# cornell-zhang/HiSparse

Measured on AMD Instinct MI355X. Metric: SpMV GBPS (8 B per non-zero per SpMV, sw/benchmark.cpp:312-346), higher is better.
Workload: dtype u32 (Q8.24 fixed point, u64 row sums)

## Files before the change

hisparse_amd/csrc/gpu_tiles.h:

```cpp
#ifndef HISPARSE_GPU_TILES_H_
#define HISPARSE_GPU_TILES_H_

#include <hip/hip_runtime_api.h>

#include <cstdint>
#include <string>
#include <vector>

#include "device_buffer.h"
#include "tiles_common.h"

namespace hisparse {
namespace dev {

hipError_t warm_gpu_tiler();

class GpuTiler {
  public:
    GpuTiler(const detail::Layout& layout, const void* const channel[NUM_HBM_CHANNELS], const uint64_t n_packets[NUM_HBM_CHANNELS], hipStream_t stream);
    GpuTiler(const detail::Layout& layout, const CsrView& csr, hipStream_t stream);
    GpuTiler(const GpuTiler&) = delete;
    GpuTiler& operator=(const GpuTiler&) = delete;

    const std::string& error() const { return error_; }
    bool count_rows(std::vector<uint32_t>& row_nnz, uint64_t& nnz);
    bool count_tiles(const std::vector<uint32_t>& block_of_row, uint32_t num_ranges, std::vector<uint32_t>& cnt);
    bool sort_elements(const std::vector<uint32_t>& block_of_row, const std::vector<uint32_t>& range_row0, const std::vector<uint32_t>& unit_of,
                       const std::vector<detail::UnitPlan>& plans, bool& duplicates);
    bool delta_slots(std::vector<detail::UnitPlan>& plans);
    bool owner_shares(std::vector<detail::UnitPlan>& plans, uint32_t max_span);
    bool emit(StreamFormat format, uint64_t image_bytes, uint64_t slack_bytes, const std::vector<detail::UnitPlan>& plans,
              const std::vector<uint32_t>& block_of_unit, const std::vector<Block>& blocks, bool is_float);
    bool bitmap_slice_counts(uint32_t slices, uint32_t groups_per_row, std::vector<uint32_t>& cnt);
    struct BitmapBlock {
        uint32_t row0, nrows, gs0, GS, pieces, stride;
        uint64_t mask_word0;
        uint64_t prefix0;
        uint32_t piece_cut[kBitmapWaves + 1];
    };
    struct BitmapRun {
        uint64_t mask_word, prefix_at;
        uint32_t steps, pad;
    };
    bool bitmap_emit(uint32_t slices, uint32_t groups_per_row, const std::vector<uint32_t>& range_of_row, const std::vector<BitmapBlock>& blocks,
                     const std::vector<uint64_t>& row_value_base, uint64_t image_bytes, uint64_t slack_bytes, const std::vector<BitmapRun>& runs,
                     std::vector<uint32_t>& run_prefix, std::vector<uint64_t>& run_heads, const MfmaImage* mfma, bool& duplicates);
    uint8_t* release_mfma() { return d_mfma_.release(); }
    bool sweep_line_counts(uint32_t lines, std::vector<uint64_t>& line_nnz);
    bool sweep_sort(const std::vector<uint32_t>& range_of_row, const std::vector<uint32_t>& range_row0, const std::vector<uint32_t>& slice_col,
                    uint32_t num_blocks, std::vector<uint64_t>& block_start, bool& unsupported);
    struct SweepBlock {
        uint64_t first;
        uint64_t stream_at, table_at;
        uint64_t chunk0;
        uint32_t count, steps, nrows, pad_col;
    };
    bool sweep_emit(const std::vector<SweepBlock>& blocks, uint64_t image_bytes, uint64_t slack_bytes);
    uint8_t* release_image() { return d_image_.release(); }
    uint32_t* release_value_map() { return d_map_.release(); }
    uint32_t* release_value_map2() { return d_map2_.release(); }

  private:
    bool fail(const std::string& what);
    bool check(hipError_t e, const char* what);
    bool upload_channels();
    bool upload_csr(std::vector<uint32_t>& row_nnz);
    bool read_error(const char* copy, const char* sync);
    bool gather_values();
    void release_source();
    bool alloc_map(DeviceBuffer<uint32_t>& map, uint64_t image_bytes);
    template <typename S> S source() const;
    template <typename G> const G* groups() const { return reinterpret_cast<const G*>(d_groups_.get()); }
    uint64_t element_threads() const;

    detail::Layout L_;
    Geometry geom_;
    const void* const* channel_;
    const uint64_t* n_packets_;
    hipStream_t stream_;
    std::string error_;

    const CsrView* csr_ = nullptr;
    uint32_t indptr_rows_ = 0;
    DeviceBuffer<uint32_t> d_indptr_;
    DeviceBuffer<uint32_t> d_indices_;
// ... 27 lines not shown
```

hisparse_amd/csrc/gpu_tiles.hip:

```cpp
#include "gpu_tiles.h"

#include <hip/hip_runtime.h>
#include <hipcub/hipcub.hpp>

#include <algorithm>
#include <cstring>
#include <type_traits>

#include "value_word.h"

namespace hisparse {
namespace dev {

using detail::Layout;
using detail::UnitPlan;

namespace {

constexpr uint32_t kPosBits = 28;
constexpr uint64_t kPosMask = (1ull << kPosBits) - 1;
constexpr uint32_t kErrColumn = 1, kErrRow = 2;

struct StreamGroup {
    uint64_t byte_off;
// ... 384 lines not shown
        uint32_t d = 0;
        if (i > 0) {
            const uint32_t prev = uint32_t(keys[p.start + i - 1] & kPosMask);
            const uint64_t b = bridges[p.start + i] - bridges[p.start + i - 1];
            d = uint32_t(pos - prev - b * kBridgeAdvance);
        }
        return Slot{d, vals[p.start + i], pos, p.start + i};
    }
    const uint32_t prev = uint32_t(keys[p.start + i - 1] & kPosMask);
    const uint64_t s_prev = (i - 1) + (bridges[p.start + i - 1] - bbase);
    const uint64_t k = si - (s_prev + 1);
    return Slot{kBridgeGap, 0u, uint32_t(prev + (k + 1) * kBridgeAdvance), kNoElement};
}

template <bool kMap>
__global__ __launch_bounds__(256) void emit_delta_kernel(const DevicePlan* __restrict__ plans, const uint64_t* __restrict__ keys,
                                                        const uint32_t* __restrict__ vals, const uint64_t* __restrict__ bridges,
                                                        uint8_t* __restrict__ image, uint32_t pad_gap, const uint32_t* __restrict__ src,
                                                        uint32_t* __restrict__ map) {
    const DevicePlan& p = plans[blockIdx.x];
    if (!p.n) return;
    const uint32_t scratch_pos = p.nrows * kSubTileCols;
    const uint32_t first_pos = uint32_t(keys[p.start] & kPosMask);
    for (uint32_t w = 0; w < kConsumerWaves; ++w) {
        const uint32_t run = p.run_len[w];
        if (!run) continue;
        uint8_t* rec = image + p.wave_offset[w] + uint64_t(p.start_step[w]) * kRecordBytes;
        const uint32_t slots_in_records = (run + 2) / 2 * 2;
        for (uint32_t idx = threadIdx.x; idx < slots_in_records * kWaveLanes; idx += blockDim.x) {
            const uint32_t j = idx / kWaveLanes, l = idx % kWaveLanes;
            uint8_t* r = rec + uint64_t(j / 2) * kRecordBytes;
            uint32_t* value_word = reinterpret_cast<uint32_t*>(r) + 2 * l + j % 2;
            uint16_t* gap_word = reinterpret_cast<uint16_t*>(r + kWaveLanes * 8) + 2 * l + j % 2;
            const uint64_t s0 = p.first_slot[w] + uint64_t(l) * p.lane_stride[w];
            if (j == 0) {
                uint32_t head = scratch_pos;
                if (s0 < p.slots) head = s0 == 0 ? first_pos : delta_slot(p, keys, vals, bridges, s0 - 1).after;
                *value_word = head;
                continue;
            }
            if (j > run) { *gap_word = uint16_t(pad_gap); continue; }
            const uint64_t si = s0 + (j - 1);
            uint32_t value = 0, gap = pad_gap;
            if (si < p.slots) {
                const Slot s = delta_slot(p, keys, vals, bridges, si);
                value = s.val;
                gap = s.gap;
                if (kMap && s.e != kNoElement) map[src[s.e]] = word_index(value_word, image);
            }
            *value_word = value;
            *gap_word = uint16_t(gap);
        }
    }
}

struct ElementSource {
    const uint8_t* channels;
    const StreamGroup* groups;
    const uint64_t* advance;
    const uint32_t* indptr;
    const uint32_t* indices;
    const float* values;
    uint64_t nnz;
    uint32_t num_groups, total_slots, num_rows, num_cols, logical_vb, fixed, csr;
    uint32_t transposed;
};

template <typename Visit>
__device__ __forceinline__ void visit_elements(const ElementSource& src, uint64_t t, uint32_t* err, Visit visit) {
    if (src.csr) {
        CsrCursor c;
        if (!csr_segment(src.indptr, src.num_rows, src.nnz, t, c)) return;
        for (; c.e < c.end; ++c.e) {
            while (c.e >= src.indptr[c.row + 1]) ++c.row;
            const uint32_t idx = src.indices[c.e];
            if (idx >= src.num_cols) { report(err, kErrColumn, c.row / PACK_SIZE, c.row % PACK_SIZE); return; }
            const uint32_t row = src.transposed ? idx : c.row, col = src.transposed ? c.row : idx;
            if constexpr (std::is_invocable_v<Visit, uint32_t, uint32_t, uint32_t, uint64_t>) visit(row, col, value_word(src.values[c.e], src.fixed != 0), c.e);
            else visit(row, col, value_word(src.values[c.e], src.fixed != 0));
        }
        return;
    }
    Segment s;
    if (t >= src.total_slots || !find_segment(src.channels, src.groups, src.num_groups, src.total_slots, uint32_t(t), s)) return;
    const StreamGroup& g = src.groups[s.group];
    const uint32_t col_base = g.cp * src.logical_vb;
    if constexpr (std::is_invocable_v<Visit, uint32_t, uint32_t, uint32_t, uint64_t>)
        walk_segment(g, s, src.advance, [&](uint32_t row, uint32_t col, uint32_t val) { visit(row, col_base + col, val, ~0ull); });
    else
        walk_segment(g, s, src.advance, [&](uint32_t row, uint32_t col, uint32_t val) { visit(row, col_base + col, val); });
}

__device__ __forceinline__ uint32_t cut_at(uint32_t n, uint32_t parts, uint32_t k) { return uint32_t(uint64_t(k) * n / parts); }
__device__ __forceinline__ uint32_t part_of(uint32_t n, uint32_t parts, uint32_t x) {
    uint32_t k = min(parts - 1, uint32_t((uint64_t(x) + 1) * parts / n));
    while (cut_at(n, parts, k) > x) --k;
    while (k + 1 < parts && cut_at(n, parts, k + 1) <= x) ++k;
    return k;
}
__device__ __forceinline__ uint32_t padded_masks(uint32_t steps) { return (steps + 7u) / 8u * 8u + 16u; }
__device__ __forceinline__ uint32_t mask_offset(const GpuTiler::BitmapBlock& b, uint32_t g) {
    if (b.pieces <= 1) return g;
    uint32_t j = 0, at = 0;
    while (j + 1 < b.pieces && b.piece_cut[j + 1] <= g) {
        at += padded_masks(b.piece_cut[j + 1] - b.piece_cut[j]);
        ++j;
// ... 427 lines not shown
    DeviceBuffer<DevicePlan> d_plans;
    DeviceBuffer<uint8_t> d_temp;
    std::vector<DevicePlan> dp;
    make_device_plans(plans, {}, {}, dp);
    bool ok = check(d_in.alloc_count(n), "hipMalloc") && check(d_bridges_.alloc_count(n), "hipMalloc") && check(d_slots.alloc_count(plans.size(), 16), "hipMalloc") &&
              check(upload(d_plans, dp, stream_), "upload plans");
    if (ok && total_) {
        hipLaunchKernelGGL(bridges_kernel, dim3(uint32_t((total_ + 255) / 256)), dim3(256), 0, stream_, d_keys_.get(), total_, d_in.get());
        size_t temp_bytes = 0;
        ok = check(hipGetLastError(), "bridges_kernel") &&
             check(hipcub::DeviceScan::InclusiveSum(nullptr, temp_bytes, d_in.get(), d_bridges_.get(), total_, stream_), "scan (size)") &&
             check(d_temp.alloc_count(temp_bytes, 16), "hipMalloc(scan)") &&
             check(hipcub::DeviceScan::InclusiveSum(d_temp.get(), temp_bytes, d_in.get(), d_bridges_.get(), total_, stream_), "scan");
    }
    std::vector<uint64_t> slots(plans.size(), 0);
    if (ok && !plans.empty()) {
        hipLaunchKernelGGL(unit_slots_kernel, dim3(uint32_t((plans.size() + 255) / 256)), dim3(256), 0, stream_, d_plans.get(), uint32_t(plans.size()), d_bridges_.get(), d_slots.get());
        ok = check(hipGetLastError(), "unit_slots_kernel") &&
             check(hipMemcpyAsync(slots.data(), d_slots.get(), slots.size() * 8, hipMemcpyDeviceToHost, stream_), "read slots");
    }
    ok = ok && check(hipStreamSynchronize(stream_), "delta slots");
    if (ok)
        for (size_t u = 0; u < plans.size(); ++u) plans[u].slots = slots[u];
    return ok;
}

bool GpuTiler::owner_shares(std::vector<UnitPlan>& plans, uint32_t max_span) {
    const uint32_t nu = uint32_t(plans.size());
    if (!nu) return true;
    std::vector<uint64_t> start(nu);
    std::vector<uint32_t> count(nu);
    for (uint32_t u = 0; u < nu; ++u) { start[u] = plans[u].scratch; count[u] = plans[u].n; }
    DeviceBuffer<uint64_t> d_start;
    DeviceBuffer<uint32_t> d_n, d_own;
    std::vector<uint32_t> own(size_t(nu) * kShareWords);
    bool ok = check(upload(d_start, start, stream_), "upload") && check(upload(d_n, count, stream_), "upload") && check(d_own.alloc_count(own.size()), "hipMalloc");
    if (ok) {
        hipLaunchKernelGGL(owner_balanced_shares_kernel, dim3((nu + 255) / 256), dim3(256), 0, stream_, d_start.get(), d_n.get(), nu, d_keys_.get(), max_span, d_own.get());
        ok = check(hipGetLastError(), "owner_balanced_shares_kernel") &&
             check(hipMemcpyAsync(own.data(), d_own.get(), own.size() * 4, hipMemcpyDeviceToHost, stream_), "read shares") && check(hipStreamSynchronize(stream_), "owner shares");
    }
    if (ok)
        for (uint32_t u = 0; u < nu; ++u) {
            const uint32_t* o = own.data() + size_t(u) * kShareWords;
            for (uint32_t w = 0; w <= kConsumerWaves; ++w) plans[u].own_begin[w] = o[w];
            for (uint32_t w = 0; w < kConsumerWaves; ++w) {
                plans[u].own_row[w] = o[kConsumerWaves + 1 + w];
                plans[u].own_last[w] = o[2 * kConsumerWaves + 1 + w];
            }
        }
    return ok;
}

bool GpuTiler::emit(StreamFormat format, uint64_t image_bytes, uint64_t slack_bytes, const std::vector<UnitPlan>& plans,
                    const std::vector<uint32_t>& block_of_unit, const std::vector<Block>& blocks, bool is_float) {
    std::vector<DevicePlan> dp;
    make_device_plans(plans, block_of_unit, blocks, dp);
    DeviceBuffer<DevicePlan> d_plans;
    const size_t bytes = std::max<uint64_t>(image_bytes + slack_bytes, 256);
    bool ok = check(d_image_.alloc(bytes), "hipMalloc(image)") && check(hipMemsetAsync(d_image_.get(), 0, bytes, stream_), "hipMemset(image)") &&
              check(upload(d_plans, dp, stream_), "upload plans");
    if (ok && d_src_) ok = alloc_map(d_map_, image_bytes);
    const dim3 grid(uint32_t(plans.size())), block(256);
    if (ok && !plans.empty()) {
        const bool m = bool(d_map_);
        const DevicePlan* p = d_plans.get();
        const uint64_t* keys = d_keys_.get();
        const uint32_t *vals = d_vals_.get(), *src = d_src_.get();
        uint8_t* image = d_image_.get();
        uint32_t* map = d_map_.get();
        switch (format) {
            case kFormatPairs:
                hipLaunchKernelGGL((m ? emit_pairs_kernel<false, true> : emit_pairs_kernel<false, false>), grid, block, 0, stream_, p, keys, vals, image, src, map);
                break;
            case kFormatPairs24:
                hipLaunchKernelGGL((m ? emit_pairs_kernel<true, true> : emit_pairs_kernel<true, false>), grid, block, 0, stream_, p, keys, vals, image, src, map);
                break;
            case kFormatOwner:
                hipLaunchKernelGGL((m ? emit_owner_kernel<false, true> : emit_owner_kernel<false, false>), grid, block, 0, stream_, p, keys, vals, image, src, map);
                break;
            case kFormatOwner24:
                hipLaunchKernelGGL((m ? emit_owner_kernel<true, true> : emit_owner_kernel<true, false>), grid, block, 0, stream_, p, keys, vals, image, src, map);
                break;
            case kFormatDelta:
                hipLaunchKernelGGL(m ? emit_delta_kernel<true> : emit_delta_kernel<false>, grid, block, 0, stream_, p, keys, vals, d_bridges_.get(), image,
                                   is_float ? kBridgeGap : 0u, src, map);
                break;
            default: ok = fail("gpu re-tile: format not supported");
        }
        ok = ok && check(hipGetLastError(), "emit kernel");
    }
    ok = ok && check(hipStreamSynchronize(stream_), "emit");
    d_keys_.reset();
    d_vals_.reset();
    d_bridges_.reset();
    d_src_.reset();
    return ok;
}

bool GpuTiler::bitmap_slice_counts(uint32_t slices, uint32_t GR, std::vector<uint32_t>& cnt) {
    cnt.assign(size_t(L_.num_rows) * slices, 0);
    const uint64_t threads = element_threads();
    DeviceBuffer<uint32_t> d_cnt;
    bool ok = check(d_cnt.alloc_count(cnt.size(), 16), "hipMalloc") && check(hipMemsetAsync(d_cnt.get(), 0, cnt.size() * 4, stream_), "hipMemset");
    if (ok && threads) {
        hipLaunchKernelGGL(bitmap_slice_counts_kernel, dim3(uint32_t((threads + 255) / 256)), dim3(256), 0, stream_, source<ElementSource>(), slices, GR, d_cnt.get(), d_scalar_.get());
        ok = check(hipGetLastError(), "bitmap_slice_counts_kernel");
    }
    return ok && (cnt.empty() || check(hipMemcpyAsync(cnt.data(), d_cnt.get(), cnt.size() * 4, hipMemcpyDeviceToHost, stream_), "read slice counts")) &&
           read_error("slice counts", "slice counts");
}

bool GpuTiler::bitmap_emit(uint32_t slices, uint32_t GR, const std::vector<uint32_t>& range_of_row, const std::vector<BitmapBlock>& blocks,
                           const std::vector<uint64_t>& row_value_base, uint64_t image_bytes, uint64_t slack_bytes, const std::vector<BitmapRun>& runs,
                           std::vector<uint32_t>& run_prefix, std::vector<uint64_t>& run_heads, const MfmaImage* mfma, bool& duplicates) {
    detail::PhaseTimer timer;
    duplicates = false;
    const ElementSource src = source<ElementSource>();
    const uint64_t threads = element_threads();
    const dim3 egrid(uint32_t((threads + 255) / 256)), block(256);
    uint64_t prefix_words = 0;
    for (const BitmapBlock& b : blocks) prefix_words = std::max<uint64_t>(prefix_words, b.prefix0 + uint64_t(b.nrows) * b.stride);
    const size_t bytes = std::max<uint64_t>(image_bytes + slack_bytes, 256);
    const uint32_t num_runs = uint32_t(runs.size());
    run_prefix.assign(num_runs, 0);
    run_heads.assign(size_t(num_runs) * kBitmapMaskBatch, 0);
    DeviceBuffer<uint32_t> d_range, d_prefix, d_flags, d_run_prefix, d_cnt, d_pos;
    DeviceBuffer<BitmapBlock> d_blocks;
    DeviceBuffer<BitmapRun> d_runs;
    DeviceBuffer<uint64_t> d_row_base;
    DeviceBuffer<unsigned long long> d_heads;
    DeviceBuffer<uint8_t> d_temp;
    bool ok = check(d_image_.alloc(bytes), "hipMalloc(image)") && check(hipMemsetAsync(d_image_.get(), 0, bytes, stream_), "hipMemset(image)") &&
              check(upload(d_range, range_of_row, stream_), "upload row ranges") && check(upload(d_blocks, blocks, stream_), "upload blocks") &&
              check(upload(d_row_base, row_value_base, stream_), "upload row bases") && check(upload(d_runs, runs, stream_), "upload runs") &&
              check(d_prefix.alloc_count(prefix_words, 16), "hipMalloc(prefix)") &&
              check(d_flags.alloc(16), "hipMalloc") && check(hipMemsetAsync(d_flags.get(), 0, 16, stream_), "hipMemset") &&
              check(d_run_prefix.alloc_count(num_runs, 16), "hipMalloc") && check(d_heads.alloc_count(run_heads.size(), 16), "hipMalloc");
    unsigned long long* image64 = reinterpret_cast<unsigned long long*>(d_image_.get());
    unsigned long long* masks2 = nullptr;
    if (ok && mfma) {
        ok = check(d_mfma_.alloc_count(mfma->words_bytes, 16), "hipMalloc(second image)") &&
             check(hipMemsetAsync(d_mfma_.get(), 0, mfma->words_bytes, stream_), "hipMemset(second image)");
        masks2 = reinterpret_cast<unsigned long long*>(d_mfma_.get());
    }
// ... 232 lines not shown
```

hisparse_amd/csrc/hs_load.cpp:

```cpp
#include "hs_context.h"

#include <algorithm>
#include <chrono>
#include <cstdio>
#include <cstdlib>

#include "hisparse/channel_packets.h"

using hisparse::Geometry;
using hisparse::dev::Block;
using hisparse::dev::Unit;

namespace {

constexpr size_t kImageSlackBytes = 16384;

bool value_map_asked(const hs_context* c) {
    const char* v = ctx_option(c, "HISPARSE_VALUE_MAP");
    return v && std::atoi(v) != 0;
}

template <typename T>
hipError_t upload(DeviceBuffer<T>& dst, const void* src, size_t bytes, size_t slack) {
    const hipError_t e = dst.alloc(std::max<size_t>(bytes + slack, 256));
    if (e != hipSuccess || bytes == 0) return e;
    return hipMemcpy(dst.get(), src, bytes, hipMemcpyHostToDevice);
}

int load_matrix_once(hs_context* ctx, const void* const* channel, const uint64_t* n_packets, const hisparse::dev::CsrView* csr_in,
                     uint32_t num_rows, uint32_t num_cols, uint32_t num_row_partitions, uint32_t num_col_partitions, bool want_map) {
    const Geometry& g = ctx->geom;
    if (num_rows == 0 || num_cols == 0) return fail(ctx, HS_ERR_BAD_ARG, "empty matrix");
    if (num_rows % g.row_divisor != 0 || num_cols % hisparse::PACK_SIZE != 0)
        return fail(ctx, HS_ERR_BAD_ARG, "dimensions are not padded: rows must divide by " + std::to_string(g.row_divisor) +
                                             " and columns by 8 (util_round_csr_matrix_dim)");
    if (num_row_partitions != (num_rows + g.logical_ob - 1) / g.logical_ob || num_col_partitions != (num_cols + g.logical_vb - 1) / g.logical_vb)
        return fail(ctx, HS_ERR_BAD_ARG, "partition counts do not match the dimensions and the bank sizes of this context");
    if (int rc = enter(ctx, 0)) return rc;
    HS_HIP(ctx, hipStreamSynchronize(ctx->stream));
    free_matrix(ctx);
    MatrixData& m = ctx->mat;
    const auto t0 = std::chrono::steady_clock::now();
    const bool map_on = value_map_asked(ctx);
    hisparse::dev::CsrView csr_view;
    const hisparse::dev::CsrView* csr = nullptr;
    if (csr_in) {
        csr_view = *csr_in;
        csr_view.value_map = map_on && want_map;
        csr = &csr_view;
    }

    hisparse::dev::StreamTiles tiles;
    std::string why;
    auto adopt_device_images = [&]() {
        m.image.adopt(tiles.d_image);
        m.mfma.words.adopt(reinterpret_cast<uint32_t*>(tiles.mfma.d_words));
        m.value_map.adopt(tiles.d_value_map);
        m.mfma.value_map.adopt(tiles.d_value_map2);
        tiles.d_image = nullptr;
        tiles.mfma.d_words = nullptr;
        tiles.d_value_map = tiles.d_value_map2 = nullptr;
    };
    auto start_over_on_host = [&]() {
        adopt_device_images();
        m = MatrixData();
        tiles = hisparse::dev::StreamTiles();
    };
    const hisparse::dev::detail::OptionScope option_scope(&ctx->options);
    const char* retile = hisparse::dev::detail::env_switch("HISPARSE_RETILE");
    bool on_gpu = csr || !(retile && std::string(retile) == "host");
    int rc = HS_OK;
    try {
        bool ok = hisparse::dev::build_stream_tiles(channel, n_packets, g, num_rows, num_cols, num_row_partitions, num_col_partitions,
                                                    uint32_t(ctx->compute_units), tiles, why, ctx->stream, on_gpu, kImageSlackBytes, csr);
        if (!ok && csr && why == "gpu re-tile: duplicate entries") {
            start_over_on_host();
            const hisparse::dev::detail::HostCsr rows(csr);
            on_gpu = false;
            if (rows.ok()) {
                spmv::io::CSRMatrix<float> mat;
                mat.num_rows = rows->num_rows;
                mat.num_cols = rows->num_cols;
                const uint64_t nnz = rows->indptr[rows->num_rows];
                mat.adj_indptr.assign(rows->indptr, rows->indptr + rows->num_rows + 1);
                mat.adj_indices.assign(rows->indices, rows->indices + nnz);
                mat.adj_data.assign(rows->values, rows->values + nnz);
                const hisparse::ChannelPackets packets = hisparse::format_matrix(mat, g, true);
                const void* chan[hisparse::NUM_HBM_CHANNELS];
                uint64_t count[hisparse::NUM_HBM_CHANNELS];
                for (uint32_t c = 0; c < hisparse::NUM_HBM_CHANNELS; ++c) { chan[c] = packets.channel[c].data(); count[c] = packets.channel[c].size(); }
                ok = packets.num_rows == num_rows && packets.num_cols == num_cols &&
                     hisparse::dev::build_stream_tiles(chan, count, g, num_rows, num_cols, num_row_partitions, num_col_partitions, uint32_t(ctx->compute_units), tiles, why);
            } else {
                why = "CSR column index outside the matrix";
            }
        }
        if (!ok && !csr && on_gpu && why.rfind("gpu re-tile:", 0) == 0) {
            start_over_on_host();
            on_gpu = false;
            ok = hisparse::dev::build_stream_tiles(channel, n_packets, g, num_rows, num_cols, num_row_partitions, num_col_partitions,
                                                   uint32_t(ctx->compute_units), tiles, why);
        }
        if (!ok) rc = fail(ctx, why == hisparse::dev::detail::kBadMfmaChunk ? HS_ERR_BAD_ARG : HS_ERR_BAD_MATRIX, why);
    } catch (const std::bad_alloc&) {
        rc = fail(ctx, HS_ERR_NO_MEMORY, "out of host memory while re-tiling the matrix");
    } catch (const std::exception& e) {
        rc = fail(ctx, HS_ERR_BAD_MATRIX, std::string("re-tiling the matrix failed: ") + e.what());
    } catch (...) {
        rc = fail(ctx, HS_ERR_BAD_MATRIX, "re-tiling the matrix failed");
    }
    const bool image_on_device = tiles.d_image != nullptr, mfma_on_device = tiles.mfma.d_words != nullptr;
    adopt_device_images();
    if (rc != HS_OK) return rc;
    const bool debug = ctx_option(ctx, "HISPARSE_PLAN_DEBUG") != nullptr;
    auto since = [&]() { return std::chrono::duration<double, std::milli>(std::chrono::steady_clock::now() - t0).count(); };
    if (debug) std::fprintf(stderr, "load: image built after %.1f ms\n", since());
    const uint32_t lds_bytes = tiles.format == hisparse::dev::kFormatSweep ? hisparse::dev::spmv_sweep_lds_bytes(tiles.max_block_rows, ctx->is_float())
                               : tiles.light ? hisparse::dev::spmv_light_lds_bytes(tiles.max_block_rows)
                                           : hisparse::dev::spmv_lds_bytes(tiles.max_block_rows, tiles.ring_buffers, tiles.format) +
                                                 tiles.bitmap_x_groups * hisparse::dev::kBitmapGroupCols * 4u;
    if (lds_bytes > hisparse::dev::kMaxLdsBytes) return fail(ctx, HS_ERR_UNSUPPORTED, "row block does not fit the LDS");

    HS_HIP(ctx, hisparse::dev::configure_spmv_kernels(hisparse::dev::kMaxLdsBytes));
    if (!image_on_device)
        HS_HIP(ctx, upload(m.image, tiles.image.data(), tiles.image.size(), kImageSlackBytes));
    HS_HIP(ctx, upload(m.blocks, tiles.blocks.data(), tiles.blocks.size() * sizeof(Block), 0));
    HS_HIP(ctx, upload(m.units, tiles.units.data(), tiles.units.size() * sizeof(Unit), 0));
    HS_HIP(ctx, upload(m.part_heads, tiles.part_heads.data(), tiles.part_heads.size() * sizeof(uint32_t), 0));
    HS_HIP(ctx, m.y.alloc(size_t(num_rows) * 4));
    HS_HIP(ctx, hipMemset(m.y.get(), 0, size_t(num_rows) * 4));
    const uint64_t image_bytes = image_on_device ? tiles.image_bytes : uint64_t(tiles.image.size());
    const char* resident_opt = ctx_option(ctx, "HISPARSE_STREAM_RESIDENT");
    m.launch.stream_resident = resident_opt ? std::atoi(resident_opt) != 0
                                     : hisparse::dev::plan_stream_resident(tiles.format, tiles.light, image_bytes, tiles.units.size(), tiles.blocks.size());
    const char* carry_opt = ctx_option(ctx, "HISPARSE_CARRY_COMBINE");
    const bool carries = tiles.col_slices > 1 && (carry_opt ? std::atoi(carry_opt) != 0 : hisparse::dev::plan_carries(tiles.format, image_bytes));
    HS_HIP(ctx, ctx->carry.reset(ctx->is_float(), num_rows, num_cols, tiles.col_slices, carries));
    if (mfma_on_device || (tiles.mfma.words_bytes != 0 && !tiles.mfma.words.empty())) {
        const hisparse::dev::MfmaImage& mi = tiles.mfma;
        MatrixData::Mfma& mf = m.mfma;
        bool ok = mfma_on_device || upload(mf.words, mi.words.data(), mi.words.size(), 0) == hipSuccess;
        ok = ok && mf.x.alloc(hisparse::dev::spmm_mfma_x_words(mi.groups) * 4) == hipSuccess &&
             mf.partial.alloc(hisparse::dev::spmm_mfma_partial_words(mi.tiles, mi.chunks) * 4) == hipSuccess &&
             mf.flag.alloc(64) == hipSuccess && hipMemset(mf.flag.get(), 0, 64) == hipSuccess;
        if (ok) {
            mf.info = std::move(tiles.mfma);
            mf.info.words = {};
        } else {
            (void)hipGetLastError();
            mf = MatrixData::Mfma();
        }
    }
    if (m.value_map) {
        m.value_map_nnz = tiles.nnz;
        m.value_map_why.clear();
    } else if (!map_on) {
        m.value_map_why = "the value_map option was off when the matrix was loaded";
    } else if (!csr) {
        m.value_map_why = "the matrix came from hs_load_matrix (CPSR): only hs_load_matrix_csr and hs_load_matrix_csr_transposed keep a value map";
    } else if (!image_on_device) {
        m.value_map_why = "the image was built by the host builder (duplicate (row, column) entries, bitmap_build=host, or SWEEP chunks spanning more than 65535 "
                          "columns): it has no value map";
    } else {
        m.value_map_why = "the image is 16 GiB or larger: its word indices do not fit 32 bits";
    }
    if (debug) std::fprintf(stderr, "load: descriptors + result buffers on the device after %.1f ms\n", since());
    m.num_rows = num_rows;
    m.num_cols = num_cols;
    m.row_parts = num_row_partitions;
    m.col_slices = tiles.col_slices;
    m.spmm_vectors = tiles.spmm_vectors;
    if (tiles.spmm_vectors == 4) {
        const uint32_t need = hisparse::dev::spmm_sweep_lds_bytes(tiles.max_block_rows, ctx->is_float());
        if (need > hisparse::dev::kMaxLdsBytes) m.spmm_vectors = 1;
        else HS_HIP(ctx, hisparse::dev::configure_spmm_sweep_kernels(hisparse::dev::kMaxLdsBytes));
    }
    for (const Block& b : tiles.blocks) m.crossing_blocks = m.crossing_blocks || b.last_part != b.row_part;
    m.max_block_rows = tiles.max_block_rows;
    hisparse::dev::SpmvLaunch& a = m.launch;
    a.image = m.image.get();
    a.blocks = m.blocks.get();
    a.units = m.units.get();
    a.part_heads = m.part_heads.get();
    a.ring_buffers = tiles.ring_buffers;
    a.format = tiles.format;
    a.num_cols = num_cols;
    a.num_workgroups = tiles.num_workgroups;
    a.lds_bytes = lds_bytes;
    a.bitmap_x_groups = tiles.bitmap_x_groups;
    a.light = tiles.light;
    ctx->dense_spmv_us = 0.0;
    m.loaded = true;

    hs_stats& s = ctx->stats;
    s = hs_stats{};
    s.nnz = tiles.nnz;
    for (int c = 0; n_packets && c < HS_NUM_CHANNELS; ++c) s.cpsr_bytes += n_packets[c] * sizeof(hisparse::MatPkt);
    s.stream_bytes = tiles.image_bytes;
    s.stream_elements = tiles.elements;
    s.num_blocks = uint32_t(tiles.blocks.size());
    s.num_units = uint32_t(tiles.units.size());
    s.col_slices = tiles.col_slices;
    s.ring_buffers = tiles.ring_buffers;
    s.stream_format = tiles.format;
    s.num_workgroups = tiles.num_workgroups;
    s.lds_bytes = lds_bytes;
    s.num_compute_units = uint32_t(ctx->compute_units);
    s.load_seconds = std::chrono::duration<double>(std::chrono::steady_clock::now() - t0).count();
    s.retiled_on_gpu = image_on_device;
    s.light_kernel = tiles.light ? 1u : 0u;
    s.stream_resident = a.stream_resident && hisparse::dev::stream_policy_applies(tiles.format, tiles.light) ? 1u : 0u;
    return HS_OK;
}

double time_loaded_plan(hs_context* ctx, int runs) {
    DeviceBuffer<uint32_t> zero_x;
    if (zero_x.alloc(size_t(ctx->mat.num_cols) * 4 + 64) != hipSuccess) { (void)hipGetLastError(); return -1.0; }
    double us = -1.0;
    if (hipMemsetAsync(zero_x.get(), 0, size_t(ctx->mat.num_cols) * 4, ctx->stream) == hipSuccess)
        (void)time_steps(ctx, zero_x.get(), ctx->mat.y.get(), 3, 2, runs, &us);
    (void)hipStreamSynchronize(ctx->stream);
    return us;
}

int load_matrix_impl(hs_context* ctx, const void* const* channel, const uint64_t* n_packets, const hisparse::dev::CsrView* csr,
                     uint32_t num_rows, uint32_t num_cols, uint32_t num_row_partitions, uint32_t num_col_partitions) {
    const char* tune = ctx_option(ctx, "HISPARSE_AUTOTUNE");
    const bool tuning = tune && std::atoi(tune) != 0 && !ctx_option(ctx, "HISPARSE_STREAM_FORMAT");
    int rc = load_matrix_once(ctx, channel, n_packets, csr, num_rows, num_cols, num_row_partitions, num_col_partitions, !tuning);
    if (rc != HS_OK || !tuning) return rc;
    const bool debug = ctx_option(ctx, "HISPARSE_PLAN_DEBUG") != nullptr;
    const char* const names[] = {"pairs", "delta", "bitmap", "owner", "pairs24", "owner24", "sweep"};
    const MatrixData& m = ctx->mat;
    const std::string own = m.launch.light ? "light" : names[m.launch.format < 7 ? m.launch.format : 0];
    const uint64_t nnz = ctx->stats.nnz;
    const int runs = int(std::max<uint64_t>(5, std::min<uint64_t>(50, (uint64_t(40) << 20) / std::max<uint64_t>(1, nnz))));
    double best_us = time_loaded_plan(ctx, runs);
    if (best_us <= 0.0)
        return value_map_asked(ctx) ? load_matrix_once(ctx, channel, n_packets, csr, num_rows, num_cols, num_row_partitions, num_col_partitions, true) : HS_OK;
    std::string best = own;
    if (debug) std::fprintf(stderr, "autotune: planner's plan %s x%u: %.2f us\n", own.c_str(), m.col_slices, best_us);
    const double own_us = best_us;
    const auto light_it = ctx->options.find("HISPARSE_LIGHT");
    const bool had_light = light_it != ctx->options.end();
    const std::string caller_light = had_light ? light_it->second : std::string();
    auto restore = [&]() {
        ctx->options.erase("HISPARSE_STREAM_FORMAT");
        if (had_light) ctx->options["HISPARSE_LIGHT"] = caller_light; else ctx->options.erase("HISPARSE_LIGHT");
    };
    for (const char* fmt : {"delta", "pairs", "owner24", "sweep"}) {
        if (own == fmt) continue;
        ctx->options["HISPARSE_STREAM_FORMAT"] = fmt;
        ctx->options["HISPARSE_LIGHT"] = "0";
        const int rc2 = load_matrix_once(ctx, channel, n_packets, csr, num_rows, num_cols, num_row_partitions, num_col_partitions, false);
        double us = -1.0;
        if (rc2 == HS_OK && std::string(names[m.launch.format < 7 ? m.launch.format : 0]) == fmt) us = time_loaded_plan(ctx, runs);
        if (debug) std::fprintf(stderr, "autotune: %s x%u: %s\n", fmt, rc2 == HS_OK ? m.col_slices : 0u, us > 0.0 ? (std::to_string(us) + " us").c_str() : "not available");
        if (us > 0.0 && us < 0.97 * best_us) { best_us = us; best = fmt; }
    }
    restore();
    if (best != own) {
        ctx->options["HISPARSE_STREAM_FORMAT"] = best;
        ctx->options["HISPARSE_LIGHT"] = "0";
// ... 103 lines not shown
```

hisparse_amd/csrc/spmv_kernels.h:

```cpp
#ifndef HISPARSE_SPMV_KERNELS_H_
#define HISPARSE_SPMV_KERNELS_H_

#include <hip/hip_runtime_api.h>

#include <cstdint>

#include "stream_tiles.h"

namespace hisparse {
namespace dev {

struct SpmvLaunch {
    const uint8_t* image;
    const Block* blocks;
    const Unit* units;
    const uint32_t* part_heads;
    const uint32_t* x;
    uint32_t* out;
    int32_t row_part_filter;
    uint32_t ring_buffers;
    uint32_t format;
    uint32_t num_cols;
    uint32_t num_workgroups;
    uint32_t lds_bytes;
    uint32_t bitmap_x_groups = 0;
    const uint32_t* carry_partial = nullptr;
    uint32_t* carry_y = nullptr;
    uint32_t carry_rows = 0, carry_slices = 0;
    bool stream_resident = false;
    bool light = false;
};

bool profiling_switches(int& ablate, int& depth);
bool profiling_depth_given();
const char* profiling_switch_error();

uint32_t spmv_lds_bytes(uint32_t max_block_rows, uint32_t ring_buffers, uint32_t format = kFormatPairs);
uint32_t spmv_light_lds_bytes(uint32_t max_block_rows);
hipError_t configure_spmv_kernels(uint32_t lds_bytes);
hipError_t launch_spmv(bool is_float, const SpmvLaunch& a, hipStream_t stream);
struct SpmmLaunch {
    const uint8_t* image;
    const Block* blocks;
    const Unit* units;
    const uint32_t* x;
    uint64_t ldx;
    uint32_t* x_interleaved;
    uint32_t* y;
    uint64_t ldy;
    uint32_t vectors;
    uint32_t num_cols;
    uint32_t num_workgroups;
    uint32_t max_block_rows;
};
uint32_t spmm_bitmap_max_block_rows(bool is_float, uint32_t vectors);
hipError_t launch_spmm_bitmap(bool is_float, const SpmmLaunch& a, hipStream_t stream);
struct SpmmMfmaLaunch {
    const uint32_t* words;
    uint64_t offsets_word, values_word;
    uint32_t tiles, groups, chunk, chunks;
    const uint32_t* x;
    uint64_t ldx;
    uint32_t* x_interleaved;
    float* partial;
    uint32_t* flag;
    uint32_t call;
    uint32_t* y;
    uint64_t ldy;
    uint32_t num_rows, num_cols;
    uint32_t vectors = 16;
};
size_t spmm_mfma_x_words(uint32_t groups);
size_t spmm_mfma_partial_words(uint32_t tiles, uint32_t chunks);
hipError_t launch_spmm_mfma(const SpmmMfmaLaunch& a, hipStream_t stream);
// ... 53 lines not shown
```

hisparse_amd/csrc/spmv_kernels.hip:

```cpp
#include <hip/hip_runtime.h>

#include <cstdio>
#include <cstdlib>
#include <utility>
#include <vector>

#include "spmv_kernels.h"
#include "spmv_device.h"

namespace hisparse {
namespace dev {

namespace {

constexpr int kThreads = kWaveLanes * kWavesPerWorkgroup;
constexpr int kLightThreads = 256;
#ifndef HS_LIGHT_BATCH
#define HS_LIGHT_BATCH 4
#endif
constexpr int kLightBatch = HS_LIGHT_BATCH;
constexpr uint32_t kBufBytes = kSubTileCols * 4u;

template <int kIters, int kStride>
__device__ __forceinline__ void fill_x(uint32_t* dst, const uint32_t* __restrict__ x, uint32_t col0, uint32_t ncols, uint32_t t) {
    const uint4* src = reinterpret_cast<const uint4*>(x + col0);
    uint4* d = reinterpret_cast<uint4*>(dst);
    const uint32_t n4 = ncols / 4;
    uint4 r[kIters];
#pragma unroll
    for (int j = 0; j < kIters; ++j) r[j] = src[min(t + j * kStride, n4 - 1)];
#pragma unroll
    for (int j = 0; j < kIters; ++j) d[min(t + j * kStride, n4 - 1)] = r[j];
}

constexpr uint32_t kDmaCols = kWaveLanes * 4;
constexpr uint32_t kDmaPerFill = kSubTileCols / kDmaCols / kLoaderWaves;
__device__ __forceinline__ void dma_fill_x(uint32_t* dst, const uint32_t* __restrict__ x, uint32_t col0, uint32_t ncols, uint32_t w,
                                           uint32_t lane) {
#pragma unroll
    for (uint32_t j = 0; j < kDmaPerFill; ++j) {
        const uint32_t c = (w * kDmaPerFill + j) * kDmaCols;
        __builtin_amdgcn_global_load_lds((const __attribute__((address_space(1))) uint32_t*)(x + col0 + min(c + lane * 4, ncols - 4)),
                                         (__attribute__((address_space(3))) uint32_t*)(dst + c), 16, 0, 0);
    }
}
template <int kFills>
__device__ __forceinline__ void dma_wait() {
    asm volatile("s_waitcnt vmcnt(%0)" ::"n"(kFills * kDmaPerFill) : "memory");
}

#ifndef HS_ROWBLOCK_STREAM_POLICY
#define HS_ROWBLOCK_STREAM_POLICY "nt"
#endif
#ifndef HS_ROWBLOCK_RESIDENT_POLICY
#define HS_ROWBLOCK_RESIDENT_POLICY "sc1"
#endif
#define HS_BY_POLICY(kRes, STATEMENT)                                 \
    do {                                                              \
        if constexpr (kRes) { STATEMENT(HS_ROWBLOCK_RESIDENT_POLICY); } \
        else { STATEMENT(HS_ROWBLOCK_STREAM_POLICY); }                \
    } while (0)
#define HS_RING_AGPRS "a0", "a1", "a2", "a3", "a4", "a5", "a6", "a7", "a8", "a9", "a10", "a11", "a12", "a13", "a14", "a15", "a16", "a17", \
                      "a18", "a19", "a20", "a21", "a22", "a23", "a24", "a25", "a26", "a27", "a28", "a29", "a30", "a31"
constexpr int kMaxDepth = 16;
constexpr int kOwner24Depth = 3;

template <int kFmt, bool kRes>
struct RingT;
template <int kRing>
using Ring = RingT<(kRing & 3), (kRing & 4) != 0>;
template <bool kRes>
struct RingT<0, kRes> {
    static constexpr uint32_t kLaneBytes = 8;
    template <int K>
    static __device__ __forceinline__ void issue(const uint8_t* base, uint32_t byte_off, uint32_t lane_off) {
#define HS_ISSUE(P) asm volatile("s_nop 4\n\tglobal_load_dwordx2 a[%0:%1], %2, %3 " P ::"n"(2 * K), "n"(2 * K + 1), "v"(byte_off + lane_off), "s"(base) : "memory", HS_RING_AGPRS)
        HS_BY_POLICY(kRes, HS_ISSUE);
#undef HS_ISSUE
    }
    template <int K, int kDepth>
    static __device__ __forceinline__ void take(uint32_t& value, uint32_t& where) {
        asm volatile("s_waitcnt vmcnt(%4)\n\tv_accvgpr_read_b32 %0, a[%2]\n\tv_accvgpr_read_b32 %1, a[%3]"
                     : "=v"(value), "=v"(where) : "n"(2 * K), "n"(2 * K + 1), "n"(kDepth - 1) : "memory");
    }
    template <int K, int kDepth>
    static __device__ __forceinline__ void take2(uint32_t& value0, uint32_t& where0, uint32_t& value1, uint32_t& where1) {
        asm volatile("s_waitcnt vmcnt(%8)\n\tv_accvgpr_read_b32 %0, a[%4]\n\tv_accvgpr_read_b32 %1, a[%5]\n\tv_accvgpr_read_b32 %2, a[%6]\n\t"
                     "v_accvgpr_read_b32 %3, a[%7]"
                     : "=v"(value0), "=v"(where0), "=v"(value1), "=v"(where1)
                     : "n"(2 * K), "n"(2 * K + 1), "n"(2 * K + 2), "n"(2 * K + 3), "n"(kDepth - 2) : "memory");
    }
};
template <bool kRes>
struct RingT<1, kRes> {
    static constexpr uint32_t kLaneBytes = 8;
    template <int K>
    static __device__ __forceinline__ void issue(const uint8_t* base, uint32_t byte_off, uint32_t lane_off) {
        static_assert(2 * K + 1 < kMaxDepth && K + kMaxDepth < 2 * kMaxDepth, "values in a0..a15, gap words in a16..a23: ring depth <= 8");
#define HS_ISSUE(P)                                                                                                                                         \
    asm volatile("s_nop 4\n\tglobal_load_dwordx2 a[%0:%1], %3, %5 " P "\n\tglobal_load_dword a[%2], %4, %5 offset:512 " P ::"n"(2 * K), "n"(2 * K + 1),     \
                 "n"(K + kMaxDepth), "v"(byte_off + lane_off), "v"(byte_off + lane_off / 2), "s"(base)                                                     \
                 : "memory", HS_RING_AGPRS)
        HS_BY_POLICY(kRes, HS_ISSUE);
#undef HS_ISSUE
    }
    template <int K, int kDepth>
    static __device__ __forceinline__ void take_record(uint32_t& value_a, uint32_t& value_b, uint32_t& gaps) {
        asm volatile("s_waitcnt vmcnt(%6)\n\tv_accvgpr_read_b32 %0, a[%3]\n\tv_accvgpr_read_b32 %1, a[%4]\n\tv_accvgpr_read_b32 %2, a[%5]"
                     : "=v"(value_a), "=v"(value_b), "=v"(gaps) : "n"(2 * K), "n"(2 * K + 1), "n"(K + kMaxDepth), "n"(2 * (kDepth - 1)) : "memory");
    }
};
template <bool kRes>
struct RingT<2, kRes> {
    static constexpr uint32_t kLaneBytes = 4;
    template <int K>
    static __device__ __forceinline__ void issue(const uint8_t* base, uint32_t byte_off, uint32_t lane_off) {
#define HS_ISSUE(P)                                                                                                                       \
    asm volatile("s_nop 4\n\tglobal_load_dword a[%0], %2, %4 " P "\n\tglobal_load_dword a[%1], %3, %4 offset:256 " P ::"n"(K),           \
                 "n"(K + kMaxDepth), "v"(byte_off + lane_off), "v"(byte_off + lane_off - lane_off / 4), "s"(base)                        \
                 : "memory", HS_RING_AGPRS)
        HS_BY_POLICY(kRes, HS_ISSUE);
#undef HS_ISSUE
    }
    template <int K, int kDepth>
    static __device__ __forceinline__ void take(uint32_t& value, uint32_t& where) {
        asm volatile("s_waitcnt vmcnt(%4)\n\tv_accvgpr_read_b32 %0, a[%2]\n\tv_accvgpr_read_b32 %1, a[%3]"
                     : "=v"(value), "=v"(where) : "n"(K), "n"(K + kMaxDepth), "n"(2 * (kDepth - 1)) : "memory");
        where &= 0xffffffu;
    }
    template <int K, int kDepth>
    static __device__ __forceinline__ void take2(uint32_t& value0, uint32_t& where0, uint32_t& value1, uint32_t& where1) {
        asm volatile("s_waitcnt vmcnt(%8)\n\tv_accvgpr_read_b32 %0, a[%4]\n\tv_accvgpr_read_b32 %1, a[%5]\n\tv_accvgpr_read_b32 %2, a[%6]\n\t"
                     "v_accvgpr_read_b32 %3, a[%7]"
                     : "=v"(value0), "=v"(where0), "=v"(value1), "=v"(where1)
                     : "n"(K), "n"(K + kMaxDepth), "n"(K + 1), "n"(K + 1 + kMaxDepth), "n"(2 * (kDepth - 2)) : "memory");
        where0 &= 0xffffffu;
        where1 &= 0xffffffu;
    }
};
template <bool kRes>
struct RingT<3, kRes> {
    template <int K>
    static __device__ __forceinline__ void issue(const uint8_t* base, uint32_t byte_off, uint32_t lane16, uint32_t lane12) {
        static_assert(K < 4 && 16 + 4 * K + 2 < 2 * kMaxDepth, "a0..a15: values of four records, a16..a30: their position words");
#define HS_ISSUE(P)                                                                                                                                          \
    asm volatile("s_nop 4\n\tglobal_load_dwordx4 a[%0:%1], %4, %6 " P "\n\tglobal_load_dwordx3 a[%2:%3], %5, %6 offset:1024 " P ::"n"(4 * K), "n"(4 * K + 3), \
                 "n"(16 + 4 * K), "n"(16 + 4 * K + 2), "v"(byte_off + lane16), "v"(byte_off + lane12), "s"(base)                                            \
                 : "memory", HS_RING_AGPRS)
        HS_BY_POLICY(kRes, HS_ISSUE);
#undef HS_ISSUE
    }
    template <int K, int kDepth>
    static __device__ __forceinline__ void take(uint32_t (&v)[4], uint32_t (&w)[3]) {
        asm volatile("s_waitcnt vmcnt(%14)\n\tv_accvgpr_read_b32 %0, a[%7]\n\tv_accvgpr_read_b32 %1, a[%8]\n\tv_accvgpr_read_b32 %2, a[%9]\n\t"
                     "v_accvgpr_read_b32 %3, a[%10]\n\tv_accvgpr_read_b32 %4, a[%11]\n\tv_accvgpr_read_b32 %5, a[%12]\n\tv_accvgpr_read_b32 %6, a[%13]"
                     : "=v"(v[0]), "=v"(v[1]), "=v"(v[2]), "=v"(v[3]), "=v"(w[0]), "=v"(w[1]), "=v"(w[2])
                     : "n"(4 * K), "n"(4 * K + 1), "n"(4 * K + 2), "n"(4 * K + 3), "n"(16 + 4 * K), "n"(16 + 4 * K + 1), "n"(16 + 4 * K + 2), "n"(2 * (kDepth - 1))
                     : "memory");
    }
};
__device__ __forceinline__ const uint8_t* scalar_pointer(const uint8_t* p) {
    const uint64_t a = reinterpret_cast<uint64_t>(p);
    const uint32_t hi = __builtin_amdgcn_readfirstlane(static_cast<uint32_t>(a >> 32));
    const uint32_t lo = __builtin_amdgcn_readfirstlane(static_cast<uint32_t>(a));
    return reinterpret_cast<const uint8_t*>((static_cast<uint64_t>(hi) << 32) | lo);
}

__device__ __forceinline__ void lds_barrier() {
    __builtin_amdgcn_fence(__ATOMIC_RELEASE, "workgroup", "local");
    __builtin_amdgcn_s_barrier();
    __builtin_amdgcn_fence(__ATOMIC_ACQUIRE, "workgroup", "local");
}

template <bool kFloat> struct OwnerSum { using type = float; };
template <> struct OwnerSum<false> { using type = uint32_t; };
template <bool kFloat>
struct Consumer {
    using acc_t = typename Rows<kFloat>::acc_t;
    using prod_t = typename Rows<kFloat>::prod_t;
    static constexpr uint32_t kNoRow = 0xffffffffu;
    const uint8_t* stream;
    UnitTable unit;
    uint32_t U, wave, lane, lane_off, ring, nrows, last;
    const uint32_t* xs;
    acc_t* ys;
    uint32_t u = 0, slot = 0, end = 0, base = 0;
    uint32_t next_end = 0;
    const uint32_t* xb;
    uint32_t pos = 0;
    bool head = true;
    uint32_t run_row = kNoRow;
    typename Rows<kFloat>::sum_t run_sum = 0;
    uint32_t lane_row = 0;
    typename Rows<kFloat>::lane_t lane_sum = 0;
    typename OwnerSum<kFloat>::type own_sum = 0;
    uint32_t spare = 0;
    uint32_t row_base = 0;
    uint32_t lane_off12 = 0;
    uint64_t t_flush = 0, t_barrier = 0;
};

__device__ uint64_t* g_owner_profile = nullptr;
__device__ uint64_t* g_rowblock_timeline = nullptr;
constexpr uint32_t kTimelineBlocks = 4, kTimelineStamps = 8;
template <int kAblate>
__device__ __forceinline__ void timeline_stamp(uint32_t k, uint32_t wave, uint32_t lane, uint32_t i) {
    if (!(kAblate & 512)) return;
    if (lane != 0 || (wave != 0 && wave != kConsumerWaves) || k >= kTimelineBlocks || !g_rowblock_timeline) return;
    const uint64_t t = __builtin_amdgcn_s_memrealtime();
    g_rowblock_timeline[((static_cast<size_t>(blockIdx.x) * kTimelineBlocks + k) * 2 + (wave ? 1 : 0)) * kTimelineStamps + i] = t;
}

template <bool kFloat, int kRing, int kAblate, int kDepth, bool kDense, int K>
__device__ __forceinline__ bool consume_step(Consumer<kFloat>& c) {
    using R = Rows<kFloat>;
    constexpr bool kDelta = (kRing & 3) == 1, k24 = (kRing & 3) == 2;
    constexpr uint32_t kStride = kDelta ? kRecordBytes : k24 ? kWaveStrideBytes24 : kWaveStrideBytes;
    constexpr uint32_t kColMask = k24 ? kSubTileCols - 1u : 0xffffu, kRowShift = k24 ? kOwnerColBits : 16u;
    const uint32_t s = c.base + K;
    while (s == c.end) {
        if (!kDelta && kDense && c.u + 1 == c.U && c.run_row != Consumer<kFloat>::kNoRow) {
            const typename R::sum_t sum = wave_sum(c.run_sum);
            if (c.lane == 0) R::add_sum(c.ys, c.run_row, sum);
            c.run_row = Consumer<kFloat>::kNoRow;
        }
        if (kDelta && kDense) {
            R::add_lane(c.ys, c.lane_row, c.lane_sum);
            c.lane_row = c.nrows;
            c.lane_sum = 0;
        }
        if (!(kAblate & 8)) lds_barrier();
        if (++c.u == c.U) return false;
        c.end = c.next_end;
        c.next_end = c.unit[min(c.u + 1, c.U - 1)].end_step[c.wave];
        c.slot = c.slot + 1 == c.ring ? 0 : c.slot + 1;
        c.xb = c.xs + c.slot * kSubTileCols;
        c.head = true;
    }
    uint32_t mat, aux;
    if constexpr (kDelta) {
        uint32_t value_a, value_b, gaps;
        Ring<kRing>::template take_record<K, kDepth>(value_a, value_b, gaps);
        auto slot = [&](uint32_t value, uint32_t gap) {
            c.pos += gap;
            uint32_t row = c.pos / kSubTileCols;
            const uint32_t col = c.pos % kSubTileCols;
            if (kAblate & 1) {
                asm volatile("" ::"v"(row), "v"(value));
                return;
            }
            const uint32_t xv = (kAblate & 2) ? col : c.xb[col];
            typename R::prod_t prod = R::product(value, xv);
            if (kFloat) {
                if (gap == kBridgeGap) prod = 0;
                row = min(row, c.nrows);
            }
            if (kDense) {
                if (row != c.lane_row) {
                    R::add_lane(c.ys, c.lane_row, c.lane_sum);
                    c.lane_row = row;
                    c.lane_sum = 0;
                }
                c.lane_sum += prod;
            } else {
                R::add(c.ys, row, prod);
            }
        };
        if (c.head) {
            c.pos = value_a;
            c.head = false;
        } else {
            slot(value_a, gaps & 0xffffu);
        }
        slot(value_b, gaps >> 16);
    } else {
        Ring<kRing>::template take<K, kDepth>(mat, aux);
        const uint32_t xv = (kAblate & 2) ? aux : c.xb[aux & kColMask];
        if (kAblate & 1) {
            asm volatile("" ::"v"(xv), "v"(mat));
        } else {
            const typename R::prod_t prod = R::product(mat, xv);
            const uint32_t row = aux >> kRowShift;
            if (kDense) {
                const uint32_t row0 = __builtin_amdgcn_readfirstlane(row);
                const bool uniform = __ballot(row == row0) == ~0ull;
                if (uniform && row0 == c.run_row) {
                    c.run_sum += R::widen(prod);
                } else {
                    if (c.run_row != Consumer<kFloat>::kNoRow) {
                        const typename R::sum_t sum = wave_sum(c.run_sum);
                        if (c.lane == 0) R::add_sum(c.ys, c.run_row, sum);
                    }
                    if (uniform) { c.run_row = row0; c.run_sum = R::widen(prod); }
                    else { c.run_row = Consumer<kFloat>::kNoRow; c.run_sum = 0; R::add(c.ys, row, prod); }
                }
            } else {
                R::add(c.ys, row, prod);
            }
        }
    }
    Ring<kRing>::template issue<K>(c.stream, min(s + kDepth, c.last) * kStride, c.lane_off);
    return true;
}

template <bool kFloat>
struct OwnerOps;
template <>
struct OwnerOps<true> {
    using val_t = float;
    static __device__ __forceinline__ val_t product(uint32_t mat, uint32_t xv) { return __uint_as_float(mat) * __uint_as_float(xv); }
    static __device__ __forceinline__ val_t add(val_t a, val_t b) { return a + b; }
};
template <>
struct OwnerOps<false> {
    using val_t = uint32_t;
    static __device__ __forceinline__ val_t product(uint32_t mat, uint32_t xv) { return q8_24_mul(mat, xv); }
    static __device__ __forceinline__ val_t add(val_t a, val_t b) { return __builtin_elementwise_add_sat(a, b); }
};
template <bool kFloat>
__device__ __forceinline__ void owner_flush(typename OwnerOps<kFloat>::val_t* ys32, uint32_t row, typename OwnerOps<kFloat>::val_t sum) {
    ys32[row] = OwnerOps<kFloat>::add(ys32[row], sum);
}
template <bool kFloat>
__device__ __forceinline__ void owner_end_of_unit(Consumer<kFloat>& c) {
    using Ops = OwnerOps<kFloat>;
    using val_t = typename Ops::val_t;
    val_t* ys32 = reinterpret_cast<val_t*>(c.ys);
// ... 193 lines not shown
    const uint32_t where2 = __builtin_amdgcn_alignbit(w[2], w[1], 16) & 0xffffffu, where3 = w[2] >> 8;
    if (!owner24_pair<kFloat, kAblate>(c, 4 * r, v[0], where0, v[1], where1)) return false;
    return owner24_pair<kFloat, kAblate>(c, 4 * r + 2, v[2], where2, v[3], where3);
}
template <bool kFloat, int kAblate, int kDepth, int... Ks>
__device__ __forceinline__ bool consume_round_owner24(Consumer<kFloat>& c, std::integer_sequence<int, Ks...>) {
    return (consume_record_owner24<kFloat, kAblate, kDepth, Ks>(c) && ...);
}
template <bool kFloat, int... Ks>
__device__ __forceinline__ void prime_ring_owner24(Consumer<kFloat>& c, std::integer_sequence<int, Ks...>) {
    (Ring<3>::template issue<Ks>(c.stream, min(static_cast<uint32_t>(Ks), c.last) * kOwnerRecordBytes, c.lane_off, c.lane_off12), ...);
}
template <bool kFloat, int kDepth>
__device__ __forceinline__ void consumer_begin_owner24(Consumer<kFloat>& c, const uint8_t* stream, UnitTable unit, uint32_t U, uint32_t wave, uint32_t lane,
                                                       const uint32_t* xs, uint32_t ring, typename Rows<kFloat>::acc_t* ys, uint32_t nrows, uint32_t total_steps,
                                                       uint32_t first_end) {
    static_assert(kDepth >= 1 && kDepth <= 4, "records in flight: a0..a30");
    c.stream = scalar_pointer(stream);
    c.unit = unit; c.U = U; c.wave = wave; c.lane = lane; c.ring = ring; c.nrows = nrows;
    c.lane_off = lane * 16u;
    c.lane_off12 = lane * 12u;
    const uint32_t records = (total_steps + kOwnerRecordSteps - 1) / kOwnerRecordSteps;
    c.last = records ? records - 1 : 0;
    c.xs = xs; c.xb = xs; c.ys = ys;
    c.end = first_end & kOwnerStepMask;
    c.row_base = first_end >> 16;
    c.next_end = U > 1 ? unit[1].end_step[wave] : first_end;
    c.lane_row = nrows + wave;
    c.spare = nrows + wave;
    prime_ring_owner24<kFloat>(c, std::make_integer_sequence<int, kDepth>());
}
template <bool kFloat, int kAblate, int kDepth>
__device__ __forceinline__ void consumer_run_owner24(Consumer<kFloat>& c) {
    __builtin_amdgcn_s_waitcnt(0x0f70);
    for (;; c.base += kDepth)
        if (!consume_round_owner24<kFloat, kAblate, kDepth>(c, std::make_integer_sequence<int, kDepth>())) break;
    asm volatile("s_waitcnt vmcnt(0)" ::: "memory", HS_RING_AGPRS);
}

template <bool kFloat, int kRing, int kAblate, int kDepth, bool kDense, int... Ks>
__device__ __forceinline__ bool consume_round(Consumer<kFloat>& c, std::integer_sequence<int, Ks...>) {
    return (consume_step<kFloat, kRing, kAblate, kDepth, kDense, Ks>(c) && ...);
}
template <int kRing, int... Ks>
__device__ __forceinline__ void prime_ring(const uint8_t* stream, uint32_t last, uint32_t stride, uint32_t lane_off, std::integer_sequence<int, Ks...>) {
    (Ring<kRing>::template issue<Ks>(stream, min(static_cast<uint32_t>(Ks), last) * stride, lane_off), ...);
}

template <bool kFloat, int kRing, int kDepth, bool kOwner = false>
__device__ __forceinline__ void consumer_begin(Consumer<kFloat>& c, const uint8_t* stream, UnitTable unit, uint32_t U, uint32_t wave,
                                               uint32_t lane, const uint32_t* xs, uint32_t ring, typename Rows<kFloat>::acc_t* ys, uint32_t nrows,
                                               uint32_t total, uint32_t first_end) {
    static_assert(kDepth <= kMaxDepth, "the ring lives in a0..a31");
    constexpr bool kDelta = (kRing & 3) == 1, k24 = (kRing & 3) == 2;
    constexpr uint32_t kStride = kDelta ? kRecordBytes : kOwner ? kChunkBytes : k24 ? kWaveStrideBytes24 : kWaveStrideBytes;
    c.stream = scalar_pointer(stream);
    c.unit = unit; c.U = U; c.wave = wave; c.lane = lane; c.ring = ring; c.nrows = nrows;
    c.lane_off = lane * Ring<kRing>::kLaneBytes;
    c.last = total ? total - 1 : 0;
    c.xs = xs; c.xb = xs; c.ys = ys;
    c.end = first_end;
    c.next_end = U > 1 ? unit[1].end_step[wave] : first_end;
    c.lane_row = kOwner ? nrows + wave : nrows;
    c.spare = nrows + wave;
    prime_ring<kRing>(c.stream, c.last, kStride, c.lane_off, std::make_integer_sequence<int, kDepth>());
}

template <bool kFloat, int kRing, int kAblate, int kDepth, bool kDense, bool kOwner = false>
__device__ __forceinline__ void consumer_run(Consumer<kFloat>& c) {
    __builtin_amdgcn_s_waitcnt(0x0f70);
    if (kAblate & 64) { c.u = c.U - 1; c.end = c.last + 1; }
    const uint64_t t_begin = (kOwner && (kAblate & 256)) ? __builtin_readcyclecounter() : 0;
    for (;; c.base += kDepth) {
        if constexpr (kOwner) {
            if (!consume_round_owner<kRing, kAblate, kDepth>(c, std::make_integer_sequence<int, kDepth>())) break;
        } else {
            if (!consume_round<kFloat, kRing, kAblate, kDepth, kDense>(c, std::make_integer_sequence<int, kDepth>())) break;
        }
    }
    asm volatile("s_waitcnt vmcnt(0)" ::: "memory", HS_RING_AGPRS);
    if (kOwner && (kAblate & 256) && c.lane == 0 && g_owner_profile) {
        uint64_t* p = g_owner_profile + (static_cast<size_t>(blockIdx.x) * kWavesPerWorkgroup + c.wave) * 8;
        p[0] += __builtin_readcyclecounter() - t_begin;
        p[1] += c.t_flush;
        p[2] += c.t_barrier;
        p[3] += c.U;
        p[4] += c.last + 1;
    }
}

template <bool kFloat, int kRing, int kAblate, int kDepth, bool kOwner = false>
__global__ __launch_bounds__(kThreads) void spmv_rowblock_kernel(const uint8_t* __restrict__ image, const Block* __restrict__ blocks,
                                                                  const Unit* __restrict__ units, const uint32_t* __restrict__ x,
                                                                  uint32_t* __restrict__ out, int32_t row_part_filter, uint32_t ring,
                                                                  uint32_t x_base, const uint32_t* __restrict__ part_heads, CarriedCombine carry) {
    using acc_t = typename Rows<kFloat>::acc_t;
    extern __shared__ __attribute__((aligned(16))) uint8_t lds[];
    acc_t* ys = reinterpret_cast<acc_t*>(lds);
    uint32_t* xs = reinterpret_cast<uint32_t*>(lds + x_base);
    const uint32_t tid = threadIdx.x;
    const uint32_t lane = tid & (kWaveLanes - 1);
    const uint32_t wave = __builtin_amdgcn_readfirstlane(tid / kWaveLanes);
    const bool loader = wave >= kConsumerWaves;
    uint32_t wg = blockIdx.x;
    if ((gridDim.x & 7u) == 0) wg = (blockIdx.x & 7u) * (gridDim.x >> 3) + (blockIdx.x >> 3);

    uint32_t bi = wg;
    if (row_part_filter >= 0) {
        bi = ((const __attribute__((address_space(4))) uint32_t*)part_heads)[static_cast<uint32_t>(row_part_filter) * gridDim.x + wg];
        if (bi == kNoBlock) return;
    }
    bool first_block = true;
    uint32_t block_no = 0;
    for (uint32_t next = 0;; bi = next, ++block_no) {
        const BlockTable blk = (BlockTable)(blocks + bi);
        next = (row_part_filter >= 0 && blk->next_part > static_cast<uint32_t>(row_part_filter)) ? 0u : blk->next;
        const uint32_t nrows = blk->nrows, out0 = blk->out_offset;
        const UnitTable unit = (UnitTable)(units + blk->unit_begin);
        const uint32_t U = blk->unit_end - blk->unit_begin;

        if (!first_block) __syncthreads();
        first_block = false;
        timeline_stamp<kAblate>(block_no, wave, lane, 0);
        Consumer<kFloat> c;
        if (!loader && U > 0) {
            if constexpr (kRing == 3)
                consumer_begin_owner24<kFloat, kDepth>(c, image + blk->wave_offset[wave], unit, U, wave, lane, xs, ring, ys, nrows, blk->total_steps[wave], blk->first_end[wave]);
            else
                consumer_begin<kFloat, kRing, kDepth, kOwner>(c, image + blk->wave_offset[wave], unit, U, wave, lane, xs, ring, ys, nrows, blk->total_steps[wave],
                                                               blk->first_end[wave]);
        }
        if (carry.partial && block_no == 0) carried_combine<kFloat, kThreads>(carry, blockIdx.x, gridDim.x, tid);
        if (kOwner) {
            if (!(kAblate & 16)) for (uint32_t i = tid; i < nrows + kConsumerWaves; i += kThreads) reinterpret_cast<float*>(ys)[i] = 0.0f;
        } else
        if (!(kAblate & 16)) for (uint32_t i = tid; i <= nrows; i += kThreads) ys[i] = 0;
        if (U > 0 && !(kAblate & 16)) fill_x<kSubTileCols / 4 / kThreads, kThreads>(xs, x, blk->first_col0, blk->first_ncols, tid);
        __syncthreads();
        timeline_stamp<kAblate>(block_no, wave, lane, 1);

        if (U > 0) {
            if (loader) {
                const uint32_t lw = wave - kConsumerWaves;
                __builtin_amdgcn_s_setprio(3);
                uint32_t fill_slot = 1 == ring ? 0 : 1;
                uint32_t col0_next = U > 1 ? unit[1].col0 : 0, ncols_next = U > 1 ? unit[1].ncols : 8;
                uint32_t col0_after = U > 2 ? unit[2].col0 : col0_next, ncols_after = U > 2 ? unit[2].ncols : ncols_next;
                auto refill = [&](uint32_t v) {
                    const uint32_t col0 = col0_next, ncols = ncols_next;
                    if (kOwner) {
                        col0_next = col0_after;
                        ncols_next = ncols_after;
                        const uint32_t ahead = min(v + 2, U - 1);
                        col0_after = unit[ahead].col0;
                        ncols_after = unit[ahead].ncols;
                    } else {
                        const uint32_t ahead = min(v + 1, U - 1);
                        col0_next = unit[ahead].col0;
                        ncols_next = unit[ahead].ncols;
                    }
                    if (!(kAblate & 4)) dma_fill_x(xs + fill_slot * kSubTileCols, x, col0, ncols, lw, lane);
                    fill_slot = fill_slot + 1 == ring ? 0 : fill_slot + 1;
                };
                uint32_t issued = 1;
                while (issued < U && issued < ring - 1) refill(issued++);
                uint64_t t_wait = 0, t_bar = 0, t_issue = 0;
                const uint64_t t_begin = (kOwner && (kAblate & 256)) ? __builtin_readcyclecounter() : 0;
                for (uint32_t u = 0; u < U; ++u) {
                    const uint64_t ti = (kOwner && (kAblate & 256)) ? __builtin_readcyclecounter() : 0;
                    if (issued < U) refill(issued++);
                    if (kOwner && (kAblate & 256)) t_issue += __builtin_readcyclecounter() - ti;
                    const uint32_t younger = issued - min(issued, u + 2);
                    const uint64_t t0 = (kOwner && (kAblate & 256)) ? __builtin_readcyclecounter() : 0;
                    if (younger >= 2) dma_wait<2>(); else if (younger == 1) dma_wait<1>(); else dma_wait<0>();
                    const uint64_t t1 = (kOwner && (kAblate & 256)) ? __builtin_readcyclecounter() : 0;
                    if (!(kAblate & 8)) __builtin_amdgcn_s_barrier();
                    if (kOwner && (kAblate & 256)) { const uint64_t t2 = __builtin_readcyclecounter(); t_wait += t1 - t0; t_bar += t2 - t1; }
                }
                if (kOwner && (kAblate & 256) && lane == 0 && g_owner_profile) {
                    uint64_t* p = g_owner_profile + (static_cast<size_t>(blockIdx.x) * kWavesPerWorkgroup + wave) * 8;
                    p[0] += __builtin_readcyclecounter() - t_begin;
                    p[1] += t_wait;
                    p[2] += t_bar;
                    p[3] += U;
                    p[4] += t_issue;
                }
            } else {
                if constexpr (kRing == 3) consumer_run_owner24<kFloat, kAblate, kDepth>(c);
                else if constexpr (kOwner) consumer_run<kFloat, kRing, kAblate, kDepth, false, true>(c);
                else if (blk->flags & kBlockDenseRows) consumer_run<kFloat, kRing, kAblate, kDepth, true>(c);
                else consumer_run<kFloat, kRing, kAblate, kDepth, false>(c);
            }
        }
        timeline_stamp<kAblate>(block_no, wave, lane, 2);
        if (kOwner) {
            if (!loader) {
                const float flushed = reinterpret_cast<volatile float*>(ys)[nrows + wave];
                asm volatile("" ::"v"(flushed));
            }
            __syncthreads();
            timeline_stamp<kAblate>(block_no, wave, lane, 3);
            if (!(kAblate & 32)) for (uint32_t i = tid; i < nrows; i += kThreads) out[out0 + i] = reinterpret_cast<uint32_t*>(ys)[i];
            timeline_stamp<kAblate>(block_no, wave, lane, 4);
            if (!next) break;
            continue;
        }
        if (!loader) {
            const acc_t flushed = atomicAdd(ys + nrows, static_cast<acc_t>(0));
            asm volatile("" ::"v"(flushed));
        }
        __syncthreads();
        timeline_stamp<kAblate>(block_no, wave, lane, 3);
        if (!(kAblate & 32)) for (uint32_t i = tid; i < nrows; i += kThreads) out[out0 + i] = Rows<kFloat>::finish(ys[i]);
        timeline_stamp<kAblate>(block_no, wave, lane, 4);
        if (!next) break;
    }
}

template <bool kFloat>
__device__ __forceinline__ uint32_t feedback_word(uint32_t y, uint32_t scale, uint32_t shift) {
    if (kFloat) {
        const float p = __uint_as_float(scale) * __uint_as_float(y);
        return __float_as_uint(p + __uint_as_float(shift));
    }
    const uint64_t s = static_cast<uint64_t>(q8_24_mul(scale, y)) + shift;
    return s > 0xffffffffull ? 0xffffffffu : static_cast<uint32_t>(s);
}

template <bool kFloat, int kSlices>
__global__ __launch_bounds__(256) void combine_slices_kernel(const uint32_t* __restrict__ partial, uint32_t* __restrict__ y,
                                                             uint32_t num_rows, uint32_t row_lo, uint32_t row_hi,
                                                             uint32_t* __restrict__ x_fb, uint32_t n_fb, uint32_t scale, uint32_t shift) {
    const uint32_t r = row_lo + (blockIdx.x * blockDim.x + threadIdx.x) * 4u;
    if (r >= row_hi) return;
    uint4 p[kSlices];
#pragma unroll
    for (int k = 0; k < kSlices; ++k) p[k] = *reinterpret_cast<const uint4*>(partial + static_cast<size_t>(k) * num_rows + r);
    uint32_t word[4];
    if (kFloat) {
        float s[4] = {0.0f, 0.0f, 0.0f, 0.0f};
#pragma unroll
        for (int k = 0; k < kSlices; ++k) {
            s[0] += __uint_as_float(p[k].x); s[1] += __uint_as_float(p[k].y); s[2] += __uint_as_float(p[k].z); s[3] += __uint_as_float(p[k].w);
        }
        for (int j = 0; j < 4; ++j) word[j] = __float_as_uint(s[j]);
    } else {
        uint64_t s[4] = {0, 0, 0, 0};
#pragma unroll
        for (int k = 0; k < kSlices; ++k) {
            s[0] += p[k].x; s[1] += p[k].y; s[2] += p[k].z; s[3] += p[k].w;
        }
        for (int j = 0; j < 4; ++j) word[j] = s[j] > 0xffffffffull ? 0xffffffffu : static_cast<uint32_t>(s[j]);
    }
    *reinterpret_cast<uint4*>(y + r) = make_uint4(word[0], word[1], word[2], word[3]);
    if (x_fb && r < n_fb)
        *reinterpret_cast<uint4*>(x_fb + r) = make_uint4(feedback_word<kFloat>(word[0], scale, shift), feedback_word<kFloat>(word[1], scale, shift),
                                                         feedback_word<kFloat>(word[2], scale, shift), feedback_word<kFloat>(word[3], scale, shift));
}

template <bool kFloat>
__global__ __launch_bounds__(256) void feedback_kernel(const uint32_t* __restrict__ y, uint32_t* __restrict__ x, uint32_t n, uint32_t scale,
                                                       uint32_t shift) {
    const uint32_t i = blockIdx.x * blockDim.x + threadIdx.x;
    if (i < n) x[i] = feedback_word<kFloat>(y[i], scale, shift);
}

struct PushTargets { uint32_t* dst[kMaxPushTargets]; };
__global__ __launch_bounds__(256) void push_result_kernel(const uint32_t* __restrict__ y, PushTargets t, uint32_t n_dst, uint32_t words) {
    const uint32_t i = (blockIdx.x * blockDim.x + threadIdx.x) * 4u;
// ... 132 lines not shown
#else
    return false;
#endif
}
bool profiling_switches(int& ablate, int& depth) {
#ifdef HISPARSE_PROFILING
    ablate = env_int("HISPARSE_ABLATE", 0);
    depth = env_int("HISPARSE_DEPTH", 8);
    return true;
#else
    ablate = 0;
    depth = 8;
    return profiling_switch_error() == nullptr;
#endif
}
const char* profiling_switch_error() {
#ifdef HISPARSE_PROFILING
    return nullptr;
#else
    if (env_int("HISPARSE_ABLATE", 0) != 0)
        return "HISPARSE_ABLATE is set: the ablation builds (wrong results by design) live in libhisparse_hip_prof.so (make HISPARSE_PROFILING=1, "
               "HISPARSE_HIP_LIB=...); this library will not launch with it in the environment";
    if (env_int("HISPARSE_DEPTH", 8) != 8)
        return "HISPARSE_DEPTH is set: prefetch-depth experiments live in libhisparse_hip_prof.so (make HISPARSE_PROFILING=1); this library will "
               "not launch with it in the environment";
    return nullptr;
#endif
}

uint32_t spmv_light_lds_bytes(uint32_t max_block_rows) { return ((max_block_rows + 1) * kAccumulatorBytes + 15u) & ~15u; }
uint32_t spmv_lds_bytes(uint32_t max_block_rows, uint32_t ring_buffers, uint32_t format) {
    const uint32_t acc = (format == kFormatOwner || format == kFormatOwner24) ? (max_block_rows + kConsumerWaves) * kOwnerAccumulatorBytes : (max_block_rows + 1) * kAccumulatorBytes;
    return ((acc + 15u) & ~15u) + ring_buffers * kBufBytes;
}

#ifdef HISPARSE_PROFILING
#define HS_FOR_EACH_OWNER24_ABLATION(X) X(0) X(1) X(4) X(5) X(8) X(12) X(13) X(512)
#define HS_FOR_EACH_LIGHT_VARIANT(X) X(0) X(1) X(2) X(3) X(32) X(35)
#define HS_FOR_EACH_OWNER24_DEPTH(X) X(2) X(3) X(4)
#define HS_FOR_EACH_OWNER24_FIXED(X) X(0) X(512)
#define HS_FOR_EACH_OWNER_VARIANT(X) X(0) X(1) X(2) X(3) X(4) X(7) X(8) X(11) X(12) X(15) X(127) X(256)
#else
#define HS_FOR_EACH_OWNER24_ABLATION(X) X(0)
#define HS_FOR_EACH_LIGHT_VARIANT(X) X(0)
#define HS_FOR_EACH_OWNER24_DEPTH(X) X(3)
#define HS_FOR_EACH_OWNER24_FIXED(X) X(0)
#define HS_FOR_EACH_OWNER_VARIANT(X) X(0)
#endif

#define HS_FOR_EACH_PRODUCT_VARIANT(X)                                                                           \
    X(true, 0, 0, 8) X(true, 1, 0, 8) X(false, 0, 0, 8) X(false, 1, 0, 8) X(true, 2, 0, 8) X(false, 2, 0, 8)      \
    X(true, 4, 0, 8) X(true, 5, 0, 8) X(false, 4, 0, 8) X(false, 5, 0, 8)
#ifndef HISPARSE_PROFILING
#define HS_FOR_EACH_VARIANT(X) HS_FOR_EACH_PRODUCT_VARIANT(X)
#else
#define HS_FOR_EACH_VARIANT(X)                                                                                   \
    HS_FOR_EACH_PRODUCT_VARIANT(X)                                                                               \
    X(false, false, 0, 16) X(false, false, 3, 8) X(false, true, 3, 8)                       \
    X(false, false, 4, 8) X(false, true, 4, 8) X(false, false, 8, 8) X(false, true, 8, 8) X(false, false, 15, 8) X(false, true, 15, 8) X(false, false, 31, 8) X(false, true, 31, 8)                     \
    X(false, false, 47, 8) X(false, true, 47, 8) X(false, false, 79, 8) X(false, true, 79, 8)                     \
    X(false, false, 127, 8) X(false, true, 127, 8)                                                                 \
    X(true, false, 3, 8) X(true, false, 4, 8) X(true, false, 8, 8) X(true, false, 15, 8) X(true, false, 127, 8) \
    X(false, false, 512, 8) X(false, true, 512, 8) X(true, false, 512, 8) X(true, true, 512, 8)
#endif

hipError_t configure_spmv_kernels(uint32_t lds_bytes) {
    hipError_t e;
#define X(F, T, A, D) if ((e = configure_one<F, T, A, D>(lds_bytes)) != hipSuccess) return e;
    HS_FOR_EACH_VARIANT(X)
#undef X
#define X(A) if ((e = configure_one<true, false, A, 8, true>(lds_bytes)) != hipSuccess) return e;
    HS_FOR_EACH_OWNER_VARIANT(X)
#undef X
#define X(D) if (D != 3 && (e = configure_one<true, 3, 0, D, true>(lds_bytes)) != hipSuccess) return e;
    HS_FOR_EACH_OWNER24_DEPTH(X)
#undef X
#define X(A) if ((e = configure_one<true, 3, A, 3, true>(lds_bytes)) != hipSuccess) return e;
    HS_FOR_EACH_OWNER24_ABLATION(X)
#undef X
#define X(A) if ((e = configure_one<false, 3, A, 3, true>(lds_bytes)) != hipSuccess) return e;
    HS_FOR_EACH_OWNER24_FIXED(X)
#undef X
    if ((e = configure_sweep_kernels(lds_bytes)) != hipSuccess) return e;
    return configure_bitmap_kernels(lds_bytes);
}

hipError_t launch_spmv(bool is_float, const SpmvLaunch& a, hipStream_t stream) {
    if (a.num_workgroups == 0) return hipSuccess;
    if (a.format == kFormatBitmap) return launch_spmv_bitmap(is_float, a, stream);
    if (a.format == kFormatSweep) return launch_spmv_sweep(is_float, a, stream);
    if (a.light) {
        if (a.format != kFormatPairs) return hipErrorInvalidValue;
        int ablate = 0, depth_unused = 8;
        if (!profiling_switches(ablate, depth_unused)) return hipErrorInvalidValue;
        const dim3 grid(a.num_workgroups), block(kLightThreads);
#define X(A)                                                                                                                                  \
    if (ablate == A) {                                                                                                                        \
        if (is_float) hipLaunchKernelGGL((spmv_light_kernel<true, A>), grid, block, a.lds_bytes, stream, a.image, a.blocks, a.units, a.x, a.out, a.row_part_filter, a.part_heads); \
        else hipLaunchKernelGGL((spmv_light_kernel<false, A>), grid, block, a.lds_bytes, stream, a.image, a.blocks, a.units, a.x, a.out, a.row_part_filter, a.part_heads);       \
        return hipGetLastError();                                                                                                             \
    }
        HS_FOR_EACH_LIGHT_VARIANT(X)
#undef X
        return hipErrorInvalidValue;
    }
    int ring = a.format == kFormatDelta ? 1 : a.format == kFormatPairs24 ? 2 : 0;
    const dim3 grid(a.num_workgroups), block(kThreads);
    const uint32_t x_base = a.lds_bytes - a.ring_buffers * kBufBytes;
    const CarriedCombine carry = carried(a);
    int ablate = 0, depth = 8;
    if (!profiling_switches(ablate, depth)) return hipErrorInvalidValue;
    if (a.stream_resident && ring < 2 && ablate == 0 && depth == 8 && (a.format == kFormatPairs || a.format == kFormatDelta)) ring |= 4;
    bool launched = false;
    struct TimelineDump {
        hipStream_t stream; uint32_t workgroups; bool on;
        ~TimelineDump() {
            const char* path = std::getenv("HISPARSE_TIMELINE_OUT");
            if (!on || !path || !buffer()) return;
            (void)hipStreamSynchronize(stream);
            std::vector<uint64_t> host(size_t(workgroups) * kTimelineBlocks * 2 * kTimelineStamps);
            (void)hipMemcpy(host.data(), buffer(), host.size() * sizeof(uint64_t), hipMemcpyDeviceToHost);
            if (FILE* f = std::fopen(path, "wb")) { std::fwrite(host.data(), sizeof(uint64_t), host.size(), f); std::fclose(f); }
        }
        static uint64_t*& buffer() {
            static uint64_t* b[16] = {};
            int dev = 0;
            (void)hipGetDevice(&dev);
            return b[dev >= 0 && dev < 16 ? dev : 0];
        }
    } timeline_dump{stream, a.num_workgroups, ablate == 512 && a.num_workgroups <= 4096};
    if (timeline_dump.on) {
        const size_t bytes = size_t(4096) * kTimelineBlocks * 2 * kTimelineStamps * sizeof(uint64_t);
        if (!TimelineDump::buffer() && hipMalloc(reinterpret_cast<void**>(&TimelineDump::buffer()), bytes) == hipSuccess)
            (void)hipMemcpyToSymbol(HIP_SYMBOL(g_rowblock_timeline), &TimelineDump::buffer(), sizeof(uint64_t*));
        if (TimelineDump::buffer()) (void)hipMemsetAsync(TimelineDump::buffer(), 0, bytes, stream);
    }
    if (a.format == kFormatOwner24) {
        const int records = profiling_depth_given() ? depth : kOwner24Depth;
        if (!is_float) {
            if (records != 3) return hipErrorInvalidValue;
#define X(A)                                                                                                                       \
    if (ablate == A) {                                                                                                             \
        hipLaunchKernelGGL((spmv_rowblock_kernel<false, 3, A, 3, true>), grid, block, a.lds_bytes, stream, a.image, a.blocks, a.units, a.x, a.out, \
                           a.row_part_filter, a.ring_buffers, x_base, a.part_heads, carry);                                               \
        return hipGetLastError();                                                                                                  \
    }
            HS_FOR_EACH_OWNER24_FIXED(X)
#undef X
            return hipErrorInvalidValue;
        }
#define X(A)                                                                                                                       \
    if (ablate == A && records == 3) {                                                                                             \
        hipLaunchKernelGGL((spmv_rowblock_kernel<true, 3, A, 3, true>), grid, block, a.lds_bytes, stream, a.image, a.blocks, a.units, a.x, a.out, \
                           a.row_part_filter, a.ring_buffers, x_base, a.part_heads, carry);                                               \
        return hipGetLastError();                                                                                                  \
    }
        HS_FOR_EACH_OWNER24_ABLATION(X)
#undef X
        if (ablate != 0) return hipErrorInvalidValue;
#define X(D)                                                                                                                       \
    if (records == D) {                                                                                                            \
        hipLaunchKernelGGL((spmv_rowblock_kernel<true, 3, 0, D, true>), grid, block, a.lds_bytes, stream, a.image, a.blocks, a.units, a.x, a.out, \
                           a.row_part_filter, a.ring_buffers, x_base, a.part_heads, carry);                                               \
        return hipGetLastError();                                                                                                  \
    }
        HS_FOR_EACH_OWNER24_DEPTH(X)
#undef X
        return hipErrorInvalidValue;
    }
    if (a.format == kFormatOwner) {
        if (!is_float) return hipErrorInvalidValue;
        static uint64_t* profile = nullptr;
        if (ablate == 256 && !profile) {
            (void)hipMalloc(reinterpret_cast<void**>(&profile), size_t(4096) * kWavesPerWorkgroup * 8 * sizeof(uint64_t));
            (void)hipMemset(profile, 0, size_t(4096) * kWavesPerWorkgroup * 8 * sizeof(uint64_t));
            (void)hipMemcpyToSymbol(HIP_SYMBOL(g_owner_profile), &profile, sizeof(profile));
        }
#define X(A)                                                                                                                      \
    if (!launched && ablate == A) {                                                                                               \
        hipLaunchKernelGGL((spmv_rowblock_kernel<true, false, A, 8, true>), grid, block, a.lds_bytes, stream, a.image, a.blocks,  \
                           a.units, a.x, a.out, a.row_part_filter, a.ring_buffers, x_base, a.part_heads, carry);                        \
        launched = true;                                                                                                          \
    }
        if (depth == 8) {
        HS_FOR_EACH_OWNER_VARIANT(X)
        }
#undef X
        if (ablate == 256 && profile && a.num_workgroups <= 4096) {
            if (const char* path = std::getenv("HISPARSE_TIMELINE_OUT")) {
                (void)hipStreamSynchronize(stream);
                std::vector<uint64_t> host(size_t(a.num_workgroups) * kWavesPerWorkgroup * 8);
                (void)hipMemcpy(host.data(), profile, host.size() * sizeof(uint64_t), hipMemcpyDeviceToHost);
                if (FILE* f = std::fopen(path, "wb")) {
                    std::fwrite(host.data(), sizeof(uint64_t), host.size(), f);
                    std::fclose(f);
                }
            }
        }
        return launched ? hipGetLastError() : hipErrorInvalidValue;
    }
#define X(F, T, A, D)                                                                                                           \
    if (!launched && is_float == F && ring == int(T) && ablate == A && depth == D) {                                     \
        hipLaunchKernelGGL((spmv_rowblock_kernel<F, T, A, D>), grid, block, a.lds_bytes, stream, a.image, a.blocks, a.units,    \
                           a.x, a.out, a.row_part_filter, a.ring_buffers, x_base, a.part_heads, carry);                   \
        launched = true;                                                                                                        \
    }
    HS_FOR_EACH_VARIANT(X)
#undef X
    if (!launched) return hipErrorInvalidValue;
    return hipGetLastError();
}

hipError_t launch_combine_slices(bool is_float, const uint32_t* partial, uint32_t* y, uint32_t num_rows, uint32_t slices, uint32_t row_lo,
                                 uint32_t row_hi, hipStream_t stream, uint32_t* x_fb, uint32_t n_fb, uint32_t scale, uint32_t shift) {
    if (row_hi <= row_lo) return hipSuccess;
    const dim3 grid((row_hi - row_lo + 1023) / 1024), block(256);
    switch (slices) {
#define X(N)                                                                                                                                        \
    case N:                                                                                                                                         \
        if (is_float) hipLaunchKernelGGL((combine_slices_kernel<true, N>), grid, block, 0, stream, partial, y, num_rows, row_lo, row_hi, x_fb, n_fb, scale, shift); \
        else hipLaunchKernelGGL((combine_slices_kernel<false, N>), grid, block, 0, stream, partial, y, num_rows, row_lo, row_hi, x_fb, n_fb, scale, shift);         \
        break;
        X(2) X(3) X(4) X(5) X(6) X(7) X(8) X(9) X(10) X(11) X(12) X(13) X(14) X(15) X(16)
#undef X
        default: return hipErrorInvalidValue;
    }
    static_assert(kMaxColSlices <= 16 && kMaxSweepSlices == 16, "combine_slices_kernel is instantiated for 2 .. 16 slices");
    return hipGetLastError();
}

hipError_t launch_push_result(const uint32_t* y, void* const* dst, uint32_t n_dst, uint32_t words, hipStream_t stream) {
    if (n_dst == 0 || words == 0) return hipSuccess;
    if (n_dst > kMaxPushTargets || (words & 3u)) return hipErrorInvalidValue;
    PushTargets t{};
    for (uint32_t k = 0; k < n_dst; ++k) t.dst[k] = static_cast<uint32_t*>(dst[k]);
    hipLaunchKernelGGL(push_result_kernel, dim3((words / 4 + 255) / 256), dim3(256), 0, stream, y, t, n_dst, words);
    return hipGetLastError();
}

hipError_t launch_feedback(bool is_float, const uint32_t* y, uint32_t* x, uint32_t n, uint32_t scale, uint32_t shift, hipStream_t stream) {
    if (n == 0) return hipSuccess;
    const dim3 grid((n + 255) / 256), block(256);
    if (is_float) hipLaunchKernelGGL(feedback_kernel<true>, grid, block, 0, stream, y, x, n, scale, shift);
    else hipLaunchKernelGGL(feedback_kernel<false>, grid, block, 0, stream, y, x, n, scale, shift);
    return hipGetLastError();
}

}
}
```

hisparse_amd/csrc/stream_plan.h:

```cpp
#ifndef HISPARSE_STREAM_PLAN_H_
#define HISPARSE_STREAM_PLAN_H_

#include <algorithm>
#include <cmath>
#include <cstdint>
#include <cstdio>
#include <cstdlib>
#include <functional>
#include <map>
#include <numeric>
#include <string>
#include <vector>

#include "stream_tiles.h"
#include "tiles_common.h"

namespace hisparse {
namespace dev {
namespace detail {

enum class ForcedFormat { kNone, kPairs, kDelta, kOwner, kOwner24, kSweep, kBitmap, kInvalid };
struct IntSwitch {
    bool set = false;
    int value = 0;
};
struct PlanSwitches {
    ForcedFormat format = ForcedFormat::kNone;
    IntSwitch col_slices, max_rows, light, light_wgs, sweep, row_runs;
    bool spmm4 = false;
    bool pow2_slices = false;
    bool aux24 = false;
    bool delta_spread = true;
    bool xcd_affinity = false;
    bool census = true;
    bool bitmap_on_host = false;
    bool cross_parts = true;
    bool debug = false;
    bool format_set() const { return format != ForcedFormat::kNone; }

    static PlanSwitches read() {
        PlanSwitches sw;
        auto number = [](const char* name) {
            IntSwitch s;
            if (const char* v = env_switch(name)) { s.set = true; s.value = std::atoi(v); }
            return s;
        };
        if (const char* force = env_switch("HISPARSE_STREAM_FORMAT")) {
            const std::string f(force);
            sw.format = f == "pairs" ? ForcedFormat::kPairs : f == "delta" ? ForcedFormat::kDelta : f == "owner" ? ForcedFormat::kOwner :
                        f == "owner24" ? ForcedFormat::kOwner24 : f == "sweep" ? ForcedFormat::kSweep : f == "bitmap" ? ForcedFormat::kBitmap : ForcedFormat::kInvalid;
        }
        sw.col_slices = number("HISPARSE_COL_SLICES");
        sw.max_rows = number("HISPARSE_MAX_ROWS");
        sw.light = number("HISPARSE_LIGHT");
        sw.light_wgs = number("HISPARSE_LIGHT_WGS");
        sw.sweep = number("HISPARSE_SWEEP");
        sw.row_runs = number("HISPARSE_ROW_RUNS");
        sw.spmm4 = number("HISPARSE_SPMM_VECTORS").value == 4;
        sw.pow2_slices = env_switch("HISPARSE_POW2_SLICES") != nullptr;
        sw.aux24 = number("HISPARSE_AUX_BITS").value == 24;
        if (const char* deal = env_switch("HISPARSE_DELTA_DEAL")) sw.delta_spread = std::string(deal) != "wave";
        sw.xcd_affinity = number("HISPARSE_XCD_AFFINITY").value != 0;
        const IntSwitch census = number("HISPARSE_PLAN_CENSUS");
        sw.census = !(census.set && census.value == 0);
        if (const char* where = env_switch("HISPARSE_BITMAP_BUILD")) sw.bitmap_on_host = std::string(where) == "host";
        const IntSwitch cross = number("HISPARSE_CROSS_PARTITIONS");
        if (cross.set) sw.cross_parts = cross.value != 0;
        sw.debug = env_switch("HISPARSE_PLAN_DEBUG") != nullptr;
        return sw;
    }
};
inline const char* const kBadStreamFormat = "HISPARSE_STREAM_FORMAT must be pairs, delta, owner, owner24, sweep or bitmap";


template <typename Load>
inline void deal_tiles_to_slices(const std::vector<Load>& tile_load, uint32_t slices, std::vector<uint32_t>& by_weight, Load* slice_load,
                                 uint32_t* slice_tiles, uint32_t* slice_of) {
    std::iota(by_weight.begin(), by_weight.end(), 0u);
    std::stable_sort(by_weight.begin(), by_weight.end(), [&](uint32_t x, uint32_t y) { return tile_load[x] > tile_load[y]; });
    for (uint32_t k : by_weight) {
        uint32_t best = 0;
        for (uint32_t c = 1; c < slices; ++c)
            if (slice_load[c] < slice_load[best] || (slice_load[c] == slice_load[best] && slice_tiles[c] < slice_tiles[best])) best = c;
        if (slice_of) slice_of[k] = best;
        slice_load[best] += tile_load[k];
        slice_tiles[best] += 1;
    }
}

inline bool pairs_block_is_dense(const RowRange& range, uint64_t range_nnz) {
    return range.nrows <= kDenseBlockRows && range_nnz >= 64ull * range.nrows;
}

struct TileCensus {
    uint32_t fine = 0, tiles = 0;
    std::vector<uint32_t> cnt;
    double populated = 1.0;
    struct Eval { double nonempty_units, max_wg_load; };
    Eval evaluate(uint64_t plan_ranges, uint32_t cs, uint32_t G, uint64_t nnz) const {
        plan_ranges = std::max<uint64_t>(1, plan_ranges);
        if (cnt.empty() || !fine) {
            const double blocks = double(plan_ranges) * cs, per_wg = std::ceil(blocks / G);
            return {double(plan_ranges) * tiles, double(nnz) / blocks * per_wg};
        }
        const uint64_t split = plan_ranges > fine ? (plan_ranges + fine - 1) / fine : 1;
        const uint64_t groups = plan_ranges > fine ? fine : plan_ranges;
        std::vector<double> t(tiles), block_load;
        std::vector<uint32_t> order(tiles);
        block_load.reserve(size_t(groups * split) * cs);
        double nonempty = 0.0;
        std::vector<double> slice_load(cs);
        std::vector<uint32_t> slice_tiles(cs);
        for (uint64_t j = 0; j < groups; ++j) {
            const uint64_t lo = j * fine / groups, hi = (j + 1) * fine / groups;
            std::fill(t.begin(), t.end(), 0.0);
            for (uint64_t f = lo; f < hi; ++f)
                for (uint32_t k = 0; k < tiles; ++k) t[k] += cnt[f * tiles + k];
            uint32_t live = 0;
            for (uint32_t k = 0; k < tiles; ++k) live += t[k] > 0.0;
            nonempty += double(live) * double(split);
            std::fill(slice_load.begin(), slice_load.end(), 0.0);
            if (cs == 1) {
                for (uint32_t k = 0; k < tiles; ++k) slice_load[0] += t[k];
            } else {
                std::fill(slice_tiles.begin(), slice_tiles.end(), 0u);
// ... 313 lines not shown
```

hisparse_amd/csrc/stream_tiles.cpp:

```cpp
#include "stream_tiles.h"
#include "tiles_common.h"
#include "gpu_tiles.h"
#include "stream_plan.h"

#include <algorithm>
#include <atomic>
#include <chrono>
#include <cmath>
#include <cstdint>
#include <cstdio>
#include <cstdlib>
#include <cstring>
#include <functional>
#include <map>
#include <memory>
#include <numeric>
#include <string>
#include <thread>

namespace hisparse {
namespace dev {

namespace {

using namespace detail;

struct TileBuild {
    const void* const* const channel;
    const uint64_t* const n_packets;
    const CsrView* const csr;
    const uint32_t max_workgroups;
    const uint64_t image_slack;
    const bool is_float;
    const PlanSwitches& sw;
    StreamTiles& out;
    std::string& error;
    Layout L;
    uint32_t num_rows, num_cols, CP, RP, S;
    PhaseTimer timer;
    std::unique_ptr<GpuTiler> gpu;
    std::vector<uint32_t> row_nnz;
    TileCensus census;
    TilePlan plan;
    std::vector<RowRange> ranges;
    std::vector<uint64_t> range_nnz;
    std::vector<uint32_t> block_of_row;
    size_t slots_per_range = 0;
    std::vector<uint32_t> cnt;
    std::vector<uint32_t> unit_of;
    std::vector<UnitPlan> plans;
    std::vector<uint64_t> scratch;
    uint64_t scratch_elems = 0;
    std::vector<uint32_t> block_of_unit;
    std::vector<uint64_t> block_nnz;
    uint64_t image_bytes = 0;
    std::vector<std::vector<uint32_t>> mine;

    TileBuild(const void* const channel_[NUM_HBM_CHANNELS], const uint64_t n_packets_[NUM_HBM_CHANNELS], const Geometry& geom, uint32_t num_rows_,
              uint32_t num_cols_, uint32_t num_row_partitions, uint32_t num_col_partitions, uint32_t max_workgroups_, StreamTiles& out_,
              std::string& error_, uint64_t image_slack_, const CsrView* csr_, const PlanSwitches& sw_)
        : channel(channel_), n_packets(n_packets_), csr(csr_), max_workgroups(max_workgroups_), image_slack(image_slack_),
          is_float(geom.impl != IMPL_FIXED), sw(sw_), out(out_), error(error_), num_rows(num_rows_), num_cols(num_cols_), timer{sw_.debug} {
        L.g = &geom;
        L.num_rows = num_rows;
        L.num_cols = num_cols;
        L.row_parts = num_row_partitions;
        L.col_parts = num_col_partitions;
        L.F = geom.interleave;
        L.sub_width = uint32_t(std::min<uint64_t>(kSubTileCols, geom.logical_vb));
        L.subs_per_cp = uint32_t((geom.logical_vb + L.sub_width - 1) / L.sub_width);
        L.cross_parts = sw.cross_parts;
        CP = num_col_partitions, RP = num_row_partitions, S = L.subs_per_cp;
    }

    const MatPkt* chan(uint32_t pc) const { return static_cast<const MatPkt*>(channel[pc]); }
    size_t slot(uint32_t b, uint32_t cp, uint32_t s, uint32_t pc) const { return size_t(b) * slots_per_range + (size_t(cp) * S + s) * NUM_HBM_CHANNELS + pc; }
    size_t walk_tasks() const { return L.cross_parts ? size_t(CP) * NUM_HBM_CHANNELS : size_t(RP) * CP * NUM_HBM_CHANNELS; }
    PlanInputs plan_inputs() const { return PlanInputs{L, row_nnz, out.nnz, census, max_workgroups, is_float, sw}; }
    bool gpu_failed() { error = gpu->error(); return false; }
    void set_format(StreamFormat format) { plan.format = out.format = format; }
    uint32_t chunk_bytes() const { return plan.aux24() ? kChunkBytes24 : kChunkBytes; }
    uint32_t wave_stride() const { return chunk_bytes() * kConsumerWaves; }
    static void put(bool aux24, uint8_t* chunk, uint32_t lane, uint32_t value, uint32_t where) {
        if (aux24) {
            reinterpret_cast<uint32_t*>(chunk)[lane] = value;
            uint8_t* a = chunk + kWaveLanes * 4 + lane * 3;
            a[0] = uint8_t(where); a[1] = uint8_t(where >> 8); a[2] = uint8_t(where >> 16);
        } else {
            reinterpret_cast<uint32_t*>(chunk)[2 * lane] = value;
            reinterpret_cast<uint32_t*>(chunk)[2 * lane + 1] = where;
        }
    }

    bool count_rows(void* gpu_stream, bool use_gpu);
    bool take_census();
    void cut_row_ranges();
    bool count_units();
    uint32_t block_flags(uint32_t b) const;
    bool enumerate_blocks();
    bool collect_and_sort();
    void fall_back_to_pairs();
    bool owner_shares(uint32_t max_span);
    bool lay_out_streams();
    void assign_to_workgroups();
    void finish_blocks();
    bool emit_on_gpu();
    void emit_owner();
    void emit_pairs();
    void emit_delta();
};

void reset_keeping_nnz(StreamTiles& out) {
    const uint64_t nnz_keep = out.nnz;
    out = StreamTiles();
    out.nnz = nnz_keep;
}

bool TileBuild::count_rows(void* gpu_stream, bool use_gpu) {
    row_nnz.assign(num_rows, 0);
    if (use_gpu) {
        if (csr) gpu.reset(new GpuTiler(L, *csr, static_cast<hipStream_t>(gpu_stream)));
        else gpu.reset(new GpuTiler(L, channel, n_packets, static_cast<hipStream_t>(gpu_stream)));
        if (!gpu->count_rows(row_nnz, out.nnz)) return gpu_failed();
    } else {
    std::vector<WalkResult> res0(size_t(RP) * NUM_HBM_CHANNELS);
    parallel_for(res0.size(), [&](size_t w) {
        const uint32_t rp = uint32_t(w / NUM_HBM_CHANNELS), pc = uint32_t(w % NUM_HBM_CHANNELS);
        for (uint32_t cp = 0; cp < CP && res0[w].ok; ++cp) {
            WalkResult r = walk_channel_partition(L, chan(pc), n_packets[pc], pc, rp, cp,
                                                  [&](uint32_t row, uint32_t, uint32_t) { row_nnz[row]++; });
            if (!r.ok) res0[w] = r; else res0[w].nnz += r.nnz;
        }
    });
    for (const auto& r : res0) {
        if (!r.ok) { error = r.error; return false; }
        out.nnz += r.nnz;
    }
    }
    timer.lap("pass 0 (row counts)");
    return true;
}

bool TileBuild::take_census() {
    census.tiles = CP * S;
    if (out.nnz && sw.census) {
        census.fine = uint32_t(std::max<uint64_t>(1, std::min<uint64_t>({512, (uint64_t(4) << 20) / std::max<uint32_t>(1, census.tiles), num_rows})));
        std::vector<uint32_t> fine_of_row(num_rows);
        uint64_t seen = 0;
        for (uint32_t r = 0; r < num_rows; ++r) {
            fine_of_row[r] = uint32_t(std::min<uint64_t>(census.fine - 1, seen * census.fine / out.nnz));
            seen += row_nnz[r];
        }
        if (gpu) {
            if (!gpu->count_tiles(fine_of_row, census.fine, census.cnt)) { error = gpu->error(); return false; }
        } else {
            const size_t cells = size_t(census.fine) * census.tiles;
// ... 174 lines not shown
            });
    });
    std::vector<uint32_t>().swap(cnt);

    timer.lap("pass 2 (scatter)");
    parallel_for(NU, [&](size_t u) {
        UnitPlan& up = plans[u];
        uint64_t* e = scratch.data() + up.scratch;
        std::sort(e, e + up.n);
        uint64_t slots = up.n;
        for (uint32_t i = 1; delta && i < up.n; ++i) {
            const uint64_t d = (e[i] >> 32) - (e[i - 1] >> 32);
            if (d > kMaxGap) slots += (d - kMaxGap + kBridgeAdvance - 1) / kBridgeAdvance;
        }
        up.slots = slots;
    });
    return true;
}

void TileBuild::fall_back_to_pairs() {
    set_format(kFormatPairs);
    for (UnitPlan& up : plans) up.slots = up.n;
    for (uint32_t bi = 0; bi < out.blocks.size(); ++bi) {
        const uint32_t b = bi / plan.slices;
        out.blocks[bi].flags = pairs_block_is_dense(ranges[b], range_nnz[b]) ? kBlockDenseRows : 0u;
    }
}

bool TileBuild::owner_shares(uint32_t max_span) {
    if (gpu) {
        if (!gpu->owner_shares(plans, max_span)) return gpu_failed();
        return true;
    }
    parallel_for(out.units.size(), [&](size_t u) {
        UnitPlan& up = plans[u];
        const uint64_t* e = scratch.data() + up.scratch;
        auto row_of = [&](uint32_t i) { return uint32_t(e[i] >> (32 + kOwnerColBits)); };
        balanced_owner_shares(up.n, row_of, up.own_begin, max_span);
        for (uint32_t w = 0; w < kConsumerWaves; ++w) {
            const bool any = up.own_begin[w + 1] > up.own_begin[w];
            up.own_row[w] = any ? row_of(up.own_begin[w]) : 0u;
            up.own_last[w] = any ? row_of(up.own_begin[w + 1] - 1) : 0u;
        }
    });
    return true;
}

bool TileBuild::lay_out_streams() {
    const bool delta = plan.delta(), owner = plan.owner(), owner24 = plan.owner24();
    const uint32_t NB = uint32_t(out.blocks.size()), chunk_bytes = this->chunk_bytes(), wave_stride = this->wave_stride();
    const bool delta_spread = sw.delta_spread;
    block_nnz.assign(NB, 0);
    image_bytes = 0;
    for (uint32_t bi = 0; bi < NB; ++bi) {
        Block& blk = out.blocks[bi];
        uint32_t pos[kConsumerWaves] = {0};
        uint32_t chunk_counter = 0;
        for (uint32_t u = blk.unit_begin; u < blk.unit_end; ++u) {
            UnitPlan& up = plans[u];
            if (up.slots > 0x7fffffffull) { error = "unit too large"; return false; }
            if (owner) {
                for (uint32_t w = 0; w < kConsumerWaves; ++w) {
                    const uint32_t steps = (up.own_begin[w + 1] - up.own_begin[w] + kWaveLanes - 1) / kWaveLanes;
                    up.run_len[w] = steps;
                    up.start_step[w] = up.start_record[w] = pos[w];
                    pos[w] += steps;
                    out.units[u].end_step[w] = owner24 ? (pos[w] | up.own_row[w] << 16) : pos[w];
                    out.elements += uint64_t(steps) * kWaveLanes;
                }
                continue;
            }
            const uint32_t chunks = uint32_t((up.slots + kWaveLanes - 1) / kWaveLanes);
            uint32_t run[kConsumerWaves] = {0};
            for (uint32_t c = 0; c < chunks; ++c) run[(chunk_counter + c) % kConsumerWaves]++;
            up.chunks = chunks;
            up.base = chunk_counter;
            chunk_counter += chunks;
            uint64_t first = 0;
            for (uint32_t w = 0; w < kConsumerWaves; ++w) {
                up.run_len[w] = run[w];
                up.first_slot[w] = delta_spread ? first / kWaveLanes : first;
                up.lane_stride[w] = delta_spread ? chunks : run[w];
                first += uint64_t(run[w]) * kWaveLanes;
                up.start_step[w] = up.start_record[w] = pos[w];
                pos[w] += delta ? (run[w] ? (run[w] + 2) / 2 : 0) : run[w];
                out.units[u].end_step[w] = pos[w];
            }
            out.elements += uint64_t(chunks) * kWaveLanes;
        }
        for (uint32_t w = 0; w < kConsumerWaves; ++w) block_nnz[bi] += pos[w];
        for (uint32_t w = 0; w < kConsumerWaves; ++w)
            if (uint64_t(pos[w]) * (delta ? kRecordBytes : owner ? chunk_bytes : wave_stride) >= (1ull << 32)) { error = "row block stream exceeds 4 GiB"; return false; }
        if (delta || owner) {
            for (uint32_t w = 0; w < kConsumerWaves; ++w) {
                blk.wave_offset[w] = image_bytes;
                image_bytes += owner24 ? uint64_t((pos[w] + kOwnerRecordSteps - 1) / kOwnerRecordSteps) * kOwnerRecordBytes
                                       : uint64_t(pos[w]) * (delta ? kRecordBytes : chunk_bytes);
            }
        } else {
            for (uint32_t w = 0; w < kConsumerWaves; ++w) blk.wave_offset[w] = image_bytes + uint64_t(w) * chunk_bytes;
            image_bytes += uint64_t(chunk_counter) * chunk_bytes;
        }
    }
    return true;
}

void TileBuild::assign_to_workgroups() {
    const uint32_t NB = uint32_t(out.blocks.size()), G = plan.G, slices = plan.slices;
    if (sw.xcd_affinity && slices > 1 && G % 8 == 0 && NB >= G) {
        std::vector<uint32_t> slice_of_block(NB);
        for (uint32_t bi = 0; bi < NB; ++bi) slice_of_block[bi] = bi % slices;
        assign_workgroups_by_slice(out, block_nnz, G, RP, slice_of_block, mine);
    } else {
        assign_workgroups(out, block_nnz, G, RP, mine);
    }
    timer.lap("stream layout + workgroups");
}

void TileBuild::finish_blocks() {
    const bool owner24 = plan.owner24();
    for (Block& blk : out.blocks) {
        if (blk.unit_end > blk.unit_begin) {
            for (uint32_t w = 0; w < kConsumerWaves; ++w) {
                blk.total_steps[w] = out.units[blk.unit_end - 1].end_step[w] & (owner24 ? kOwnerStepMask : 0xffffffffu);
                blk.first_end[w] = out.units[blk.unit_begin].end_step[w];
            }
            blk.first_col0 = out.units[blk.unit_begin].col0;
            blk.first_ncols = out.units[blk.unit_begin].ncols;
        }
    }
    chain_blocks(out, mine, RP);
}

bool TileBuild::emit_on_gpu() {
    if (!gpu->emit(out.format, image_bytes, image_slack, plans, block_of_unit, out.blocks, is_float)) return gpu_failed();
    out.d_image = gpu->release_image();
    out.d_value_map = gpu->release_value_map();
    out.image_bytes = image_bytes;
    finish_blocks();
    timer.lap("gpu: emit");
    return true;
}

void TileBuild::emit_owner() {
    uint8_t* image = out.image.data();
    const bool owner24 = plan.owner24();
    const uint32_t chunk_bytes = kChunkBytes;
    parallel_for(out.units.size(), [&](size_t u) {
        const UnitPlan& up = plans[u];
        const Block& blk = out.blocks[block_of_unit[u]];
        const uint64_t* e = scratch.data() + up.scratch;
        for (uint32_t w = 0; w < kConsumerWaves; ++w) {
            const uint32_t steps = up.run_len[w], n = up.own_begin[w + 1] - up.own_begin[w];
            const uint64_t* mine = e + up.own_begin[w];
            uint8_t* stream = image + blk.wave_offset[w];
            for (uint32_t st = 0; st < steps; ++st) {
                const uint32_t S = up.start_step[w] + st;
                for (uint32_t l = 0; l < kWaveLanes; ++l) {
                    const uint64_t i = uint64_t(l) * steps + st;
                    const uint32_t value = i < n ? uint32_t(mine[i]) : 0u, pos = i < n ? uint32_t(mine[i] >> 32) : 0u;
                    if (owner24) {
                        uint8_t* rec = stream + uint64_t(S / kOwnerRecordSteps) * kOwnerRecordBytes;
                        const uint32_t j = S % kOwnerRecordSteps;
                        const uint32_t where = i < n ? pos - (up.own_row[w] << kOwnerColBits) : kOwnerSpareField << kOwnerColBits;
                        reinterpret_cast<uint32_t*>(rec)[l * kOwnerRecordSteps + j] = value;
                        uint8_t* a = rec + kOwnerRecordValueBytes + (l * kOwnerRecordSteps + j) * 3;
                        a[0] = uint8_t(where); a[1] = uint8_t(where >> 8); a[2] = uint8_t(where >> 16);
                    } else {
                        put(false, stream + uint64_t(S) * chunk_bytes, l, value, i < n ? pos : (blk.nrows + w) << kOwnerColBits);
                    }
                }
            }
        }
    });
    finish_blocks();
    timer.lap("emit OWNER");
}

void TileBuild::emit_pairs() {
    uint8_t* image = out.image.data();
    const bool aux24 = plan.aux24();
    const uint32_t wave_stride = this->wave_stride();
    parallel_for(out.units.size(), [&](size_t u) {
        const UnitPlan& up = plans[u];
        const Block& blk = out.blocks[block_of_unit[u]];
        const bool dense = blk.flags & kBlockDenseRows;
        const uint64_t* e = scratch.data() + up.scratch;
        const uint64_t total = uint64_t(up.chunks) * kWaveLanes;
        for (uint64_t i = 0; i < total; ++i) {
            const uint32_t lane = dense ? uint32_t(i % kWaveLanes) : uint32_t(i / up.chunks);
            const uint32_t c = dense ? uint32_t(i / kWaveLanes) : uint32_t(i % up.chunks);
            const uint32_t g = up.base + c, w = g % kConsumerWaves;
            const uint32_t first = up.base + (w + kConsumerWaves - up.base % kConsumerWaves) % kConsumerWaves;
            const uint32_t step = up.start_step[w] + (g - first) / kConsumerWaves;
            uint8_t* chunk = image + blk.wave_offset[w] + uint64_t(step) * wave_stride;
            const uint32_t row_shift = aux24 ? kOwnerColBits : 16u;
            if (i < up.n) {
                const uint32_t pos = uint32_t(e[i] >> 32);
                put(aux24, chunk, lane, uint32_t(e[i]), ((pos / kSubTileCols) << row_shift) | (pos % kSubTileCols));
            } else {
                put(aux24, chunk, lane, 0u, blk.nrows << row_shift);
            }
        }
    });
    finish_blocks();
    timer.lap("emit PAIRS");
}

void TileBuild::emit_delta() {
    uint8_t* image = out.image.data();
    parallel_for(out.units.size(), [&](size_t u) {
        const UnitPlan& up = plans[u];
        const Block& blk = out.blocks[block_of_unit[u]];
        const uint64_t* e = scratch.data() + up.scratch;
        std::vector<uint16_t> gap(up.slots);
        std::vector<uint32_t> val(up.slots), after(up.slots);
        uint64_t k = 0;
        uint32_t at = uint32_t(e[0] >> 32);
        for (uint32_t i = 0; i < up.n; ++i) {
            uint64_t d = (e[i] >> 32) - at;
            while (d > kMaxGap) { at += kBridgeAdvance; d -= kBridgeAdvance; gap[k] = kBridgeGap; val[k] = 0; after[k] = at; ++k; }
            at += uint32_t(d);
            gap[k] = uint16_t(d); val[k] = uint32_t(e[i]); after[k] = at; ++k;
        }
        const uint16_t pad_gap = is_float ? kBridgeGap : 0;
        const uint32_t scratch_pos = blk.nrows * kSubTileCols;
        for (uint32_t w = 0; w < kConsumerWaves; ++w) {
            if (!up.run_len[w]) continue;
            uint8_t* rec = image + blk.wave_offset[w] + uint64_t(up.start_record[w]) * kRecordBytes;
            auto value_at = [&](uint32_t q, uint32_t l) -> uint32_t& { return reinterpret_cast<uint32_t*>(rec + uint64_t(q / 2) * kRecordBytes)[2 * l + q % 2]; };
            auto gap_at = [&](uint32_t q, uint32_t l) -> uint16_t& { return reinterpret_cast<uint16_t*>(rec + uint64_t(q / 2) * kRecordBytes + kWaveLanes * 8)[2 * l + q % 2]; };
            const uint32_t slots_in_records = (up.run_len[w] + 2) / 2 * 2;
            for (uint32_t l = 0; l < kWaveLanes; ++l) {
                const uint64_t s0 = up.first_slot[w] + uint64_t(l) * up.lane_stride[w];
                value_at(0, l) = s0 >= up.slots ? scratch_pos : (s0 == 0 ? uint32_t(e[0] >> 32) : after[s0 - 1]);
                for (uint32_t j = 0; j < up.run_len[w]; ++j) {
                    const uint64_t si = s0 + j;
                    value_at(j + 1, l) = si < up.slots ? val[si] : 0u;
                    gap_at(j + 1, l) = si < up.slots ? gap[si] : pad_gap;
                }
                for (uint32_t q = up.run_len[w] + 1; q < slots_in_records; ++q) gap_at(q, l) = pad_gap;
            }
        }
    });
    finish_blocks();
    timer.lap("emit DELTA");
}

enum class Attempt { kDone, kFailed, kOwner24DoesNotFit };

Attempt build_stream_tiles_attempt(const void* const channel[NUM_HBM_CHANNELS], const uint64_t n_packets[NUM_HBM_CHANNELS], const Geometry& geom,
                                   uint32_t num_rows, uint32_t num_cols, uint32_t num_row_partitions, uint32_t num_col_partitions,
                                   uint32_t max_workgroups, StreamTiles& out, std::string& error, void* gpu_stream, bool use_gpu,
                                   uint64_t image_slack, const CsrView* csr, bool owner_allowed) {
    const PlanSwitches sw = PlanSwitches::read();
    const uint64_t header_pkts = uint64_t(num_row_partitions) * num_col_partitions * (1 + geom.interleave);
    if (csr && !use_gpu) { error = "the CSR source needs the GPU re-tile"; return Attempt::kFailed; }
    for (uint32_t c = 0; !csr && c < NUM_HBM_CHANNELS; ++c) {
        if (!channel[c] && n_packets[c]) { error = "null channel buffer"; return Attempt::kFailed; }
        if (n_packets[c] < header_pkts) { error = "channel " + std::to_string(c) + " is shorter than its partition headers"; return Attempt::kFailed; }
    }
    out = StreamTiles();
    TileBuild b(channel, n_packets, geom, num_rows, num_cols, num_row_partitions, num_col_partitions, max_workgroups, out, error, image_slack, csr, sw);
    if (!b.count_rows(gpu_stream, use_gpu) || !b.take_census()) return Attempt::kFailed;
    const PlanInputs in = b.plan_inputs();
    const double hubs = hub_share(in);

    const DenseRowChoice dense = choose_dense_rows(in);
    if (sw.format == ForcedFormat::kInvalid) { error = kBadStreamFormat; return Attempt::kFailed; }
    if (dense.bitmap) {
        const bool on_host = !b.gpu || sw.bitmap_on_host;
        if (on_host && !csr) b.gpu.reset();
        if (build_bitmap_tiles(b.L, channel, n_packets, b.row_nnz, max_workgroups, out, error, csr, on_host ? nullptr : b.gpu.get(), image_slack)) return Attempt::kDone;
        if (error.rfind("bitmap:", 0) != 0) return Attempt::kFailed;
        error.clear();
        reset_keeping_nnz(out);
    }
    const SweepChoice sweep = choose_sweep(in);
    if (sweep.sweep) {
        reset_keeping_nnz(out);
        if (!build_sweep_tiles(b.L, channel, n_packets, b.row_nnz, max_workgroups, out, error, csr, b.gpu.get(), image_slack)) return Attempt::kFailed;
        out.spmm_vectors = sweep.for_spmm ? 4u : 1u;
        return Attempt::kDone;
    }
    b.plan = plan_row_blocks(in, hubs, dense, owner_allowed);
    if (b.plan.tiny_unit_sweep) {
        reset_keeping_nnz(out);
        return build_sweep_tiles(b.L, channel, n_packets, b.row_nnz, max_workgroups, out, error, csr, b.gpu.get(), image_slack) ? Attempt::kDone : Attempt::kFailed;
    }
    out.format = b.plan.format;
    out.light = b.plan.light;
    out.col_slices = b.plan.slices;

    b.cut_row_ranges();
    if (!b.count_units() || !b.enumerate_blocks() || !b.collect_and_sort()) return Attempt::kFailed;
    if (b.plan.delta() && !b.plan.format_forced && delta_or_pairs(b.plans, uint32_t(out.blocks.size()), out.nnz, b.is_float) == kFormatPairs) b.fall_back_to_pairs();
    b.timer.lap("sort units");
    if (b.plan.owner()) {
        if (!b.owner_shares(b.plan.owner24() ? kOwnerShareRows : 0xffffffffu)) return Attempt::kFailed;
        if (b.plan.owner24()) {
            const Owner24Fit fit = owner24_fit(out.blocks, b.plans);
            if (!b.is_float && !fit.fits) return Attempt::kOwner24DoesNotFit;
            if (b.is_float && (!fit.fits || (!b.plan.format_forced && !fit.smaller))) {
                b.set_format(kFormatOwner);
                if (!b.owner_shares(0xffffffffu)) return Attempt::kFailed;
            }
        }
        b.timer.lap("owner shares");
    }
    if (wants_pairs24(b.plan, sw, out.max_block_rows)) b.set_format(kFormatPairs24);
    if (!b.lay_out_streams()) return Attempt::kFailed;
    b.assign_to_workgroups();
    if (b.gpu) return b.emit_on_gpu() ? Attempt::kDone : Attempt::kFailed;
    resize_zeroed(out.image, b.image_bytes);
    out.image_bytes = b.image_bytes;
    if (b.plan.owner()) b.emit_owner();
    else if (b.plan.delta()) b.emit_delta();
    else b.emit_pairs();
    return Attempt::kDone;
}

}

bool build_stream_tiles(const void* const channel[NUM_HBM_CHANNELS], const uint64_t n_packets[NUM_HBM_CHANNELS],
                        const Geometry& geom, uint32_t num_rows, uint32_t num_cols, uint32_t num_row_partitions,
                        uint32_t num_col_partitions, uint32_t max_workgroups, StreamTiles& out, std::string& error,
                        void* gpu_stream, bool use_gpu, uint64_t image_slack, const CsrView* csr) {
    Attempt a = build_stream_tiles_attempt(channel, n_packets, geom, num_rows, num_cols, num_row_partitions, num_col_partitions, max_workgroups, out, error,
                                           gpu_stream, use_gpu, image_slack, csr, true);
    if (a == Attempt::kOwner24DoesNotFit)
        a = build_stream_tiles_attempt(channel, n_packets, geom, num_rows, num_cols, num_row_partitions, num_col_partitions, max_workgroups, out, error,
                                       gpu_stream, use_gpu, image_slack, csr, false);
    return a == Attempt::kDone;
}

}
}
```

hisparse_amd/csrc/stream_tiles.h:

```cpp
#ifndef HISPARSE_STREAM_TILES_H_
#define HISPARSE_STREAM_TILES_H_

#include <cstdint>
#include <string>
#include <memory>
#include <utility>
#include <vector>

#include "hisparse/common.h"

namespace hisparse {
namespace dev {

constexpr uint32_t kWaveLanes = 64;
constexpr uint32_t kWavesPerWorkgroup = 16;
constexpr uint32_t kConsumerWaves = 14;
constexpr uint32_t kLoaderWaves = kWavesPerWorkgroup - kConsumerWaves;
constexpr uint32_t kSubTileCols = 8192;
constexpr uint32_t kMaxXBuffers = 4;
constexpr uint32_t kMinXBuffers = 2;
constexpr uint32_t kAccumulatorBytes = 8;
constexpr uint32_t max_block_rows(bool sliced) { return (sliced ? 96u : 32u) * 1024u / kAccumulatorBytes - 1u; }
constexpr uint32_t kMaxColSlices = 8;
constexpr uint32_t kMaxForcedColSlices = 16;
constexpr uint32_t kMaxSweepSlices = 16;
constexpr uint64_t kCarryMaxImageBytes = 160ull << 20;
constexpr uint64_t kSlicedDeltaMaxImageBytes = 48ull << 20;
constexpr uint64_t kResidentMaxImageBytes = 256ull << 20;
constexpr uint64_t kRowblockResidentMaxImageBytes = 256ull << 20;
constexpr uint64_t kRowblockResidentSmallImageBytes = 32ull << 20;
constexpr uint32_t kMaxLdsBytes = 160 * 1024;
constexpr uint32_t kChunkBytes = kWaveLanes * 8;
constexpr uint32_t kWaveStrideBytes = kChunkBytes * kConsumerWaves;
constexpr uint32_t kRecordBytes = kWaveLanes * 2 * (4 + 2);
constexpr uint32_t kMaxGap = 0xfffeu;
constexpr uint32_t kBridgeGap = 0xffffu;
constexpr uint32_t kBridgeAdvance = 0xffffu;
constexpr double kDeltaMinMeanGap = 8.0;
constexpr double kDeltaMaxMeanGap = 20000.0;
constexpr uint64_t kDeltaMinSavedBytes = 23u << 20;
constexpr uint64_t kDeltaMinSavedBytesFloat = 40u << 20;
constexpr double kDenseMeanGap = 320.0;
enum StreamFormat : uint32_t { kFormatPairs = 0, kFormatDelta = 1, kFormatBitmap = 2, kFormatOwner = 3, kFormatPairs24 = 4, kFormatOwner24 = 5, kFormatSweep = 6 };
constexpr bool rowblock_stream(uint32_t format, bool light) { return (format == kFormatPairs || format == kFormatDelta) && !light; }
constexpr bool stream_policy_applies(uint32_t format, bool light) { return format == kFormatSweep || rowblock_stream(format, light); }
constexpr bool plan_stream_resident(uint32_t format, bool light, uint64_t image_bytes, uint64_t num_units, uint64_t num_blocks) {
    return rowblock_stream(format, light)
               ? image_bytes <= kRowblockResidentMaxImageBytes && (num_units > num_blocks || image_bytes <= kRowblockResidentSmallImageBytes)
               : image_bytes <= kResidentMaxImageBytes;
}
constexpr bool plan_carries(uint32_t format, uint64_t image_bytes) {
    return image_bytes < kCarryMaxImageBytes || format == kFormatOwner || format == kFormatOwner24;
}
constexpr uint32_t kChunkBytes24 = kWaveLanes * 7;
constexpr uint32_t kWaveStrideBytes24 = kChunkBytes24 * kConsumerWaves;
constexpr uint32_t kAux24MaxRows = 2046;
constexpr uint32_t kOwnerRecordSteps = 4;
constexpr uint32_t kOwnerRecordValueBytes = kWaveLanes * 4 * kOwnerRecordSteps;
constexpr uint32_t kOwnerRecordBytes = kOwnerRecordValueBytes + kWaveLanes * 3 * kOwnerRecordSteps;
constexpr uint32_t kOwnerSpareField = 2047;
constexpr uint32_t kOwnerShareRows = 2047;
constexpr uint32_t kOwnerStepMask = 0xffffu;
constexpr uint32_t kOwnerAccumulatorBytes = 4;
constexpr uint32_t kOwnerColBits = 13;
constexpr uint32_t owner_max_block_rows(uint32_t ring) { return (kMaxLdsBytes - ring * kSubTileCols * 4u) / kOwnerAccumulatorBytes - kConsumerWaves - 1u; }
constexpr double kOwnerMinMeanGap = 20000.0;
constexpr double kBitmapMinDensity = 0.125;
constexpr uint32_t kBitmapMinCols = 2048;
constexpr uint32_t kBitmapGroupCols = 64;
#ifndef HS_BITMAP_WAVES
#define HS_BITMAP_WAVES 16
#endif
constexpr uint32_t kBitmapWaves = HS_BITMAP_WAVES;
constexpr uint32_t kBitmapMaxBlockRows = 8191;
constexpr uint32_t kBitmapMaxXLdsGroups = 576;
constexpr uint32_t kBitmapSkew[4] = {170, 140, 65, 25};
constexpr uint32_t kBitmapMaskBatch = 32;
constexpr uint32_t kBitmapRunSlots = 5;
constexpr uint64_t kLightMaxNnz = 2u << 20;
constexpr uint32_t kLightMaxUnits = 16;
constexpr uint32_t kLightWorkgroupsPerCu = 4;
constexpr uint32_t kLightMaxBlockRows = 3071;
constexpr uint32_t kLightMinBlockNnz = 1024;
#ifndef HS_SWEEP_WAVES
#define HS_SWEEP_WAVES 8
#endif
constexpr uint32_t kSweepWaves = HS_SWEEP_WAVES;
constexpr uint32_t kSweepMaxBlockRowsFloat = kMaxLdsBytes / kAccumulatorBytes - 1;
constexpr uint32_t kSweepMaxBlockRowsFixed = (kMaxLdsBytes / 4 - 2) * 32 / 33 - 1;
constexpr uint32_t kSweepColAlign = 32;
constexpr double kSweepSlabMinMeanGap = 8000.0;
constexpr uint64_t kSweepMinNnz = (2u << 20) + 1;
constexpr uint64_t kFloatOneSliceOwnerMinNnz = 8u << 20;
constexpr uint64_t kSweepMinNnzWide = 256u << 10;
constexpr uint32_t kDenseBlockRows = 32;
constexpr uint32_t kBlockDenseRows = 1u;
constexpr uint32_t kBlockLastOfPartition = 2u;
constexpr uint32_t kNoBlock = 0xffffffffu;

struct Block {
    uint32_t row0;
    uint32_t nrows;
    uint32_t row_part;
    uint32_t unit_begin;
    uint32_t unit_end;
    uint32_t flags;
    uint32_t out_offset;
    uint32_t next;
    uint64_t wave_offset[kConsumerWaves];
    uint32_t total_steps[kConsumerWaves];
    uint32_t first_end[kConsumerWaves];
    uint32_t first_col0, first_ncols;
    uint32_t last_part;
    uint32_t next_part;
    uint32_t pad[12];
};
struct Unit {
    uint32_t col0;
    uint32_t ncols;
    uint32_t end_step[kConsumerWaves];
};
struct WaveSeg {
    uint32_t row_begin, row_end;
    uint32_t g_begin, g_end;
    uint32_t value_lo, value_hi;
    uint32_t mask_lo, mask_hi;
    uint32_t pad[8];
};
static_assert(sizeof(WaveSeg) == 64, "WaveSeg overlays Unit");
static_assert(sizeof(Block) == 320, "Block layout is shared with the device code");
static_assert(sizeof(Unit) == 8 + 4 * kConsumerWaves, "Unit layout is shared with the device code");

class GpuTiler;

template <typename T>
struct DefaultInitAllocator : std::allocator<T> {
    template <typename U> struct rebind { using other = DefaultInitAllocator<U>; };
    using std::allocator<T>::allocator;
    template <typename U> void construct(U* p) { ::new (static_cast<void*>(p)) U; }
    template <typename U, typename... A> void construct(U* p, A&&... a) { ::new (static_cast<void*>(p)) U(std::forward<A>(a)...); }
};
using ImageBytes = std::vector<uint8_t, DefaultInitAllocator<uint8_t>>;

struct MfmaImage {
    ImageBytes words;
    uint32_t tiles = 0;
    uint32_t groups = 0;
    uint32_t chunk = 0;
    uint32_t chunks = 0;
    uint64_t offsets_word = 0, values_word = 0;
    uint64_t words_bytes = 0;
    uint8_t* d_words = nullptr;
    bool present() const { return words_bytes != 0 && (d_words != nullptr || !words.empty()); }
};
constexpr uint32_t kMfmaTileRows = 16;

struct StreamTiles {
    ImageBytes image;
    MfmaImage mfma;
    uint32_t bitmap_x_groups = 0;
    uint8_t* d_image = nullptr;
    uint32_t* d_value_map = nullptr;
    uint32_t* d_value_map2 = nullptr;
    uint64_t image_bytes = 0;
    std::vector<Block> blocks;
    std::vector<Unit> units;
    std::vector<uint32_t> wg_first;
    std::vector<uint32_t> block_order;
    std::vector<uint32_t> part_heads;
    uint32_t num_workgroups = 0;
    uint32_t max_block_rows = 0;
    uint64_t sweep_table_bytes = 0;
    uint32_t spmm_vectors = 1;
    bool light = false;
    uint32_t col_slices = 1;
    uint32_t ring_buffers = kMaxXBuffers;
    StreamFormat format = kFormatPairs;
    uint64_t nnz = 0;
    uint64_t elements = 0;
};

struct CsrView {
    uint32_t num_rows = 0, num_cols = 0;
    const uint32_t* indptr = nullptr;
    const uint32_t* indices = nullptr;
    const float* values = nullptr;
    bool value_map = false;
    bool transposed = false;
    uint32_t out_rows() const { return transposed ? num_cols : num_rows; }
    uint32_t out_cols() const { return transposed ? num_rows : num_cols; }
};

bool build_stream_tiles(const void* const channel[NUM_HBM_CHANNELS], const uint64_t n_packets[NUM_HBM_CHANNELS],
                        const Geometry& geom, uint32_t num_rows, uint32_t num_cols, uint32_t num_row_partitions,
                        uint32_t num_col_partitions, uint32_t max_workgroups, StreamTiles& out, std::string& error,
                        void* gpu_stream = nullptr, bool use_gpu = false, uint64_t image_slack = 0, const CsrView* csr = nullptr);

}
}

#endif
```

hisparse_amd/device.py:

```python
import ctypes as C
import os

import numpy as np

from . import host

_LIB_PATH = os.environ.get("HISPARSE_HIP_LIB") or os.path.join(os.path.dirname(os.path.abspath(__file__)), "lib", "libhisparse_hip.so")
_lib = None

EXPORTS = [
    "hs_strerror", "hs_last_error", "hs_create", "hs_destroy", "hs_load_matrix", "hs_load_vector", "hs_run",
    "hs_load_matrix_csr", "hs_load_matrix_csr_transposed", "hs_run_batch", "hs_run_partition", "hs_sync", "hs_read_result", "hs_set_stream", "hs_get_stream", "hs_device_vector", "hs_device_result",
    "hs_bind_device_vector", "hs_bind_device_result", "hs_push_result", "hs_set_option", "hs_feedback", "hs_iterate", "hs_load_matrix_csc", "hs_spmspv", "hs_spmspv_device", "hs_read_spmspv_result", "hs_spmspv_status", "hs_spmm", "hs_spmm_device", "hs_get_stats", "hs_time_runs", "hs_time_kernel", "hs_debug_read_tiles", "hs_debug_read_mfma_image", "hs_update_values", "hs_update_values_device", "hs_tiles_build", "hs_tiles_info",
    "hs_tiles_copy", "hs_tiles_mfma", "hs_tiles_free", "hs_tiles_last_error",
]


class DeviceError(RuntimeError):
    def __init__(self, code, message):
        super().__init__(f"hisparse_hip error {code}: {message}")
        self.code = code


class Stats(C.Structure):
    _fields_ = [("nnz", C.c_uint64), ("cpsr_bytes", C.c_uint64), ("stream_bytes", C.c_uint64), ("stream_elements", C.c_uint64),
                ("num_blocks", C.c_uint32), ("num_units", C.c_uint32), ("num_workgroups", C.c_uint32), ("lds_bytes", C.c_uint32),
                ("num_compute_units", C.c_uint32), ("col_slices", C.c_uint32), ("ring_buffers", C.c_uint32), ("stream_format", C.c_uint32),
                ("load_seconds", C.c_double), ("retiled_on_gpu", C.c_uint32), ("light_kernel", C.c_uint32), ("stream_resident", C.c_uint32), ("reserved0", C.c_uint32)]

    def as_dict(self):
        return {name: getattr(self, name) for name, _ in self._fields_}


STREAM_FORMATS = ("pairs", "delta", "bitmap", "owner", "pairs24", "owner24", "sweep")
CONSUMER_WAVES = 14
BLOCK_DTYPE = np.dtype([("row0", "<u4"), ("nrows", "<u4"), ("row_part", "<u4"), ("unit_begin", "<u4"), ("unit_end", "<u4"),
                        ("flags", "<u4"), ("out_offset", "<u4"), ("next", "<u4"), ("wave_offset", "<u8", (CONSUMER_WAVES,)),
                        ("total_steps", "<u4", (CONSUMER_WAVES,)), ("first_end", "<u4", (CONSUMER_WAVES,)), ("first_col0", "<u4"),
                        ("first_ncols", "<u4"), ("last_part", "<u4"), ("next_part", "<u4"), ("pad", "<u4", (12,))])
UNIT_DTYPE = np.dtype([("col0", "<u4"), ("ncols", "<u4"), ("end_step", "<u4", (CONSUMER_WAVES,))])


def lib():
    global _lib
    if _lib is None:
        if not os.path.exists(_LIB_PATH):
            raise DeviceError(-3, f"{_LIB_PATH} is missing: run `make hip` (or __graft_entry__.build()); there is no fallback path")
        l = C.CDLL(_LIB_PATH)
        vp, u32, u64 = C.c_void_p, C.c_uint32, C.c_uint64
        l.hs_strerror.restype = C.c_char_p
        l.hs_strerror.argtypes = [C.c_int]
        l.hs_last_error.restype = C.c_char_p
        l.hs_last_error.argtypes = [vp]
        l.hs_create.argtypes = [C.POINTER(vp), C.c_int, C.c_int, u32, u32]
        l.hs_destroy.argtypes = [vp]
        l.hs_load_matrix.argtypes = [vp, C.POINTER(vp), C.POINTER(u64), u32, u32, u32, u32]
        l.hs_load_vector.argtypes = [vp, vp, u32]
        l.hs_run.argtypes = [vp]
        l.hs_run_partition.argtypes = [vp, u32, u32]
        l.hs_sync.argtypes = [vp]
        l.hs_read_result.argtypes = [vp, vp, u32]
        l.hs_set_stream.argtypes = [vp, vp]
        l.hs_get_stream.argtypes = [vp, C.POINTER(vp)]
        l.hs_device_vector.argtypes = [vp, C.POINTER(vp)]
        l.hs_device_result.argtypes = [vp, C.POINTER(vp)]
        l.hs_bind_device_vector.argtypes = [vp, vp]
        l.hs_bind_device_result.argtypes = [vp, vp]
        l.hs_push_result.argtypes = [vp, C.POINTER(vp), u32, u32]
        l.hs_set_option.argtypes = [vp, C.c_char_p, C.c_char_p]
        l.hs_feedback.argtypes = [vp, u32, u32]
        l.hs_iterate.argtypes = [vp, u32, u32, u32]
        l.hs_load_matrix_csc.argtypes = [vp, vp, vp, vp, u32, u32]
        l.hs_spmspv.argtypes = [vp, vp, u32]
        l.hs_spmspv_device.argtypes = [vp, vp, u32]
        l.hs_read_spmspv_result.argtypes = [vp, vp, u32]
        l.hs_spmspv_status.argtypes = [vp, C.POINTER(u32), C.POINTER(vp)]
        l.hs_get_stats.argtypes = [vp, C.POINTER(Stats)]
        l.hs_time_runs.argtypes = [vp, C.c_int, C.c_int, C.POINTER(C.c_float), C.POINTER(C.c_float)]
        l.hs_run_batch.argtypes = [vp, u32]
        l.hs_time_kernel.argtypes = [vp, C.c_int, C.c_int, C.POINTER(C.c_float)]
        l.hs_debug_read_tiles.argtypes = [vp, vp, u64, vp, vp]
        l.hs_debug_read_mfma_image.argtypes = [vp, vp, u64, C.POINTER(u64)]
        l.hs_load_matrix_csr.argtypes = [vp, u32, u32, vp, vp, vp, C.POINTER(u32), C.POINTER(u32)]
        l.hs_load_matrix_csr_transposed.argtypes = l.hs_load_matrix_csr.argtypes
        l.hs_spmm.argtypes = [vp, vp, u32, u32, vp, u32]
        l.hs_spmm_device.argtypes = [vp, vp, u64, vp, u64, u32]
        l.hs_update_values.argtypes = [vp, vp, u64]
        l.hs_update_values_device.argtypes = [vp, vp, u64]
        if hasattr(l, "hs_tiles_build") or os.path.basename(_LIB_PATH) == "libhisparse_hip.so":
            l.hs_tiles_build.argtypes = [C.POINTER(vp), C.POINTER(u64), C.c_int, u32, u32, u32, u32, u32, u32, u32, C.POINTER(vp)]
            l.hs_tiles_info.argtypes = [vp, C.POINTER(u64), C.POINTER(u32), C.POINTER(u32), C.POINTER(u32), C.POINTER(u32), C.POINTER(u64),
                                        C.POINTER(u64), C.POINTER(u32), C.POINTER(u32), C.POINTER(u32)]
# ... 79 lines not shown
        pr, pc = C.c_uint32(), C.c_uint32()
        load = lib().hs_load_matrix_csr_transposed if transpose else lib().hs_load_matrix_csr
        self._check(load(self._h, rows, cols, indptr.ctypes.data, indices.ctypes.data if indices.size else None,
                         data.ctypes.data if data.size else None, C.byref(pr), C.byref(pc)))
        self.num_rows, self.num_cols = pr.value, pc.value
        self.row_parts, self.col_parts = -(-pr.value // (128 * self.ob_bank)), -(-pc.value // (8 * self.vb_bank))
        self.csr_nnz = int(indptr[rows]) if indptr.size > rows else 0

    def update_values(self, values):
        values = np.ascontiguousarray(values, dtype=np.float32).ravel()
        if self.csr_nnz is not None and values.size != self.csr_nnz:
            raise DeviceError(-1, f"update_values: {values.size} values for a matrix of {self.csr_nnz} non-zeros")
        self._check(lib().hs_update_values(self._h, values.ctypes.data if values.size else None, values.size))

    def update_values_device(self, ptr, nnz=None):
        if hasattr(ptr, "data_ptr"):
            import torch
            if ptr.dtype != torch.float32 or not ptr.is_cuda or not ptr.is_contiguous():
                raise DeviceError(-1, "update_values_device: a contiguous float32 tensor on the GPU")
            nnz = ptr.numel() if nnz is None else nnz
            ptr = ptr.data_ptr()
        if nnz is None:
            raise DeviceError(-1, "update_values_device: the count of values is needed with a raw pointer")
        self._check(lib().hs_update_values_device(self._h, C.c_void_p(ptr or None), int(nnz)))

    def load_vector(self, x_words):
        x_words = np.ascontiguousarray(x_words, dtype=np.uint32)
        self._check(lib().hs_load_vector(self._h, x_words.ctypes.data, x_words.size))

    def run(self):
        self._check(lib().hs_run(self._h))

    def run_batch(self, steps):
        self._check(lib().hs_run_batch(self._h, int(steps)))

    def run_partition(self, row_part_id, part_len):
        self._check(lib().hs_run_partition(self._h, row_part_id, part_len))

    def sync(self):
        self._check(lib().hs_sync(self._h))

    def read_result(self):
        y = np.empty(self.num_rows, dtype=np.uint32)
        self._check(lib().hs_read_result(self._h, y.ctypes.data, y.size))
        return y

    def read_tiles(self):
        st = self.stats()
        nbytes, nblocks, nunits = st["stream_bytes"], st["num_blocks"], st["num_units"]
        image = np.zeros(max(nbytes, 1), dtype=np.uint8)
        blocks = np.zeros(max(nblocks, 1), dtype=BLOCK_DTYPE)
        units = np.zeros(max(nunits, 1), dtype=UNIT_DTYPE)
        self._check(lib().hs_debug_read_tiles(self._h, image.ctypes.data, image.size, blocks.ctypes.data, units.ctypes.data))
        return dict(image=image[:nbytes], blocks=blocks[:nblocks], units=units[:nunits])

    def read_mfma_image(self):
        n = C.c_uint64()
        self._check(lib().hs_debug_read_mfma_image(self._h, None, 0, C.byref(n)))
        words = np.zeros(max(n.value, 1), dtype=np.uint8)
        if n.value:
            self._check(lib().hs_debug_read_mfma_image(self._h, words.ctypes.data, words.size, C.byref(n)))
        return words[:n.value]

    def set_option(self, key, value=None):
        self._check(lib().hs_set_option(self._h, str(key).encode(), None if value is None else str(value).encode()))

    def set_stream(self, hip_stream):
        self._check(lib().hs_set_stream(self._h, C.c_void_p(hip_stream or None)))

    def get_stream(self):
        p = C.c_void_p()
        self._check(lib().hs_get_stream(self._h, C.byref(p)))
        return p.value

    def device_vector(self):
        p = C.c_void_p()
        self._check(lib().hs_device_vector(self._h, C.byref(p)))
        return p.value

    def device_result(self):
        p = C.c_void_p()
        self._check(lib().hs_device_result(self._h, C.byref(p)))
        return p.value

    def bind_device_vector(self, ptr):
        self._check(lib().hs_bind_device_vector(self._h, C.c_void_p(ptr or None)))

    def bind_device_result(self, ptr):
        self._check(lib().hs_bind_device_result(self._h, C.c_void_p(ptr or None)))

    def load_matrix_csc(self, indptr, row_indices, value_words, num_rows):
        indptr, row_indices, value_words = (np.ascontiguousarray(a, dtype=np.uint32) for a in (indptr, row_indices, value_words))
        self._check(lib().hs_load_matrix_csc(self._h, indptr.ctypes.data, row_indices.ctypes.data if row_indices.size else None,
                                            value_words.ctypes.data if value_words.size else None, num_rows, indptr.size - 1))
        self.csc_rows = num_rows

    def spmspv(self, x_index, x_words):
        pairs = np.empty((len(x_index), 2), dtype=np.uint32)
        pairs[:, 0] = x_index
        pairs[:, 1] = x_words
        self._check(lib().hs_spmspv(self._h, pairs.ctypes.data if pairs.size else None, len(x_index)))
        y = np.empty(self.csc_rows, dtype=np.uint32)
        self._check(lib().hs_read_spmspv_result(self._h, y.ctypes.data, y.size))
        return y

    def spmspv_async(self, x_index, x_words):
        pairs = np.empty((len(x_index), 2), dtype=np.uint32)
# ... 20 lines not shown
        self._check(lib().hs_spmm_device(self._h, C.c_void_p(x_dev), ldx, C.c_void_p(y_dev), ldy, k))

    def stats(self):
        s = Stats()
        self._check(lib().hs_get_stats(self._h, C.byref(s)))
        return s.as_dict()

    def feedback(self, scale_word, shift_word):
        self._check(lib().hs_feedback(self._h, int(scale_word), int(shift_word)))

    def iterate(self, iterations, scale_word, shift_word):
        self._check(lib().hs_iterate(self._h, int(iterations), int(scale_word), int(shift_word)))

    def push_result(self, dst_ptrs, num_words):
        arr = (C.c_void_p * len(dst_ptrs))(*dst_ptrs)
        self._check(lib().hs_push_result(self._h, arr, len(dst_ptrs), num_words))

    def time_runs(self, warmup, runs, kernel=True):
        total, kern = C.c_float(), C.c_float()
        self._check(lib().hs_time_runs(self._h, warmup, runs, C.byref(total), C.byref(kern) if kernel else None))
        return total.value, (kern.value if kernel else None)

    def time_kernel(self, warmup, runs):
        kern = C.c_float()
        self._check(lib().hs_time_kernel(self._h, warmup, runs, C.byref(kern)))
        return kern.value


def build_tiles(packets, impl, ob_bank, vb_bank, num_rows, num_cols, num_row_partitions, num_col_partitions, max_workgroups):
    l = lib()
    ptrs, counts, keep = _channel_arrays(packets)
    h = C.c_void_p()
    rc = l.hs_tiles_build(ptrs, counts, host.impl_id(impl), ob_bank, vb_bank, num_rows, num_cols, num_row_partitions,
                          num_col_partitions, max_workgroups, C.byref(h))
    del keep
    if rc != 0:
        raise DeviceError(rc, l.hs_tiles_last_error().decode())
    try:
        nbytes, nnz, elems = C.c_uint64(), C.c_uint64(), C.c_uint64()
        nblocks, nunits, nwg, maxrows, slices, ring, fmt = (C.c_uint32() for _ in range(7))
        l.hs_tiles_info(h, C.byref(nbytes), C.byref(nblocks), C.byref(nunits), C.byref(nwg), C.byref(maxrows), C.byref(nnz), C.byref(elems),
                        C.byref(slices), C.byref(ring), C.byref(fmt))
        image = np.zeros(max(nbytes.value, 1), dtype=np.uint8)
        blocks = np.zeros(max(nblocks.value, 1), dtype=BLOCK_DTYPE)
        units = np.zeros(max(nunits.value, 1), dtype=UNIT_DTYPE)
        wg_first = np.zeros(nwg.value + 1, dtype=np.uint32)
        order = np.zeros(max(nblocks.value, 1), dtype=np.uint32)
        l.hs_tiles_copy(h, image.ctypes.data, blocks.ctypes.data, units.ctypes.data, wg_first.ctypes.data, order.ctypes.data)
        mbytes, chunk, chunks = C.c_uint64(), C.c_uint32(), C.c_uint32()
        l.hs_tiles_mfma(h, None, 0, C.byref(mbytes), C.byref(chunk), C.byref(chunks))
        mfma = np.zeros(max(mbytes.value, 1), dtype=np.uint8)
        if mbytes.value:
            l.hs_tiles_mfma(h, mfma.ctypes.data, mfma.size, None, None, None)
        return dict(image=image[:nbytes.value], blocks=blocks[:nblocks.value], units=units[:nunits.value], wg_first=wg_first,
                    block_order=order[:nblocks.value], num_workgroups=nwg.value, max_block_rows=maxrows.value, nnz=nnz.value,
                    elements=elems.value, col_slices=slices.value, ring_buffers=ring.value,
                    format=STREAM_FORMATS[fmt.value], mfma=mfma[:mbytes.value], mfma_chunk=chunk.value, mfma_chunks=chunks.value)
    finally:
        l.hs_tiles_free(h)
```

include/hisparse_hip.h:

```cpp
#ifndef HISPARSE_HIP_H_
#define HISPARSE_HIP_H_

#include <stdint.h>

#ifdef __cplusplus
extern "C" {
#endif

#define HS_NUM_CHANNELS 16

enum {
    HS_OK = 0,
    HS_ERR_BAD_ARG = -1,
    HS_ERR_NO_DEVICE = -2,
    HS_ERR_HIP = -3,
    HS_ERR_BAD_MATRIX = -4,
    HS_ERR_NOT_LOADED = -5,
    HS_ERR_UNSUPPORTED = -6,
    HS_ERR_NO_MEMORY = -7,
};

enum { HS_IMPL_FIXED = 0, HS_IMPL_FLOAT_POB = 1, HS_IMPL_FLOAT_STALL = 2 };

enum { HS_STREAM_PAIRS = 0, HS_STREAM_DELTA = 1, HS_STREAM_BITMAP = 2, HS_STREAM_OWNER = 3, HS_STREAM_PAIRS24 = 4, HS_STREAM_OWNER24 = 5, HS_STREAM_SWEEP = 6 };

typedef struct hs_context hs_context;

typedef struct {
    uint64_t nnz;
    uint64_t cpsr_bytes;
    uint64_t stream_bytes;
    uint64_t stream_elements;
    uint32_t num_blocks;
    uint32_t num_units;
    uint32_t num_workgroups;
    uint32_t lds_bytes;
    uint32_t num_compute_units;
    uint32_t col_slices;
    uint32_t ring_buffers;
    uint32_t stream_format;
    double load_seconds;
    uint32_t retiled_on_gpu;
    uint32_t light_kernel;
    uint32_t stream_resident;
    uint32_t reserved0;
} hs_stats;

const char* hs_strerror(int code);
const char* hs_last_error(const hs_context* ctx);

int hs_create(hs_context** ctx, int device_id, int impl, uint32_t ob_bank, uint32_t vb_bank);
int hs_destroy(hs_context* ctx);

int hs_load_matrix(hs_context* ctx, const void* const channel[HS_NUM_CHANNELS], const uint64_t n_packets[HS_NUM_CHANNELS],
                   uint32_t num_rows, uint32_t num_cols, uint32_t num_row_partitions, uint32_t num_col_partitions);

int hs_load_vector(hs_context* ctx, const void* packed_x, uint32_t num_cols);


int hs_run(hs_context* ctx);
int hs_run_batch(hs_context* ctx, uint32_t steps);
int hs_run_partition(hs_context* ctx, uint32_t row_part_id, uint32_t part_len);
int hs_sync(hs_context* ctx);
int hs_read_result(hs_context* ctx, void* packed_y, uint32_t num_rows);

int hs_set_stream(hs_context* ctx, void* hip_stream);
int hs_get_stream(hs_context* ctx, void** hip_stream);
int hs_device_vector(hs_context* ctx, void** x_dev);
int hs_device_result(hs_context* ctx, void** y_dev);
int hs_bind_device_vector(hs_context* ctx, const void* x_dev);
int hs_bind_device_result(hs_context* ctx, void* y_dev);
int hs_push_result(hs_context* ctx, void* const* dst, uint32_t n_dst, uint32_t num_words);

int hs_set_option(hs_context* ctx, const char* key, const char* value);

int hs_feedback(hs_context* ctx, uint32_t scale_word, uint32_t shift_word);
int hs_iterate(hs_context* ctx, uint32_t iterations, uint32_t scale_word, uint32_t shift_word);

typedef struct { uint32_t index; uint32_t val; } hs_idx_val;
int hs_load_matrix_csc(hs_context* ctx, const uint32_t* indptr, const uint32_t* row_indices, const uint32_t* value_words, uint32_t num_rows,
                       uint32_t num_cols);
int hs_spmspv(hs_context* ctx, const hs_idx_val* x_entries, uint32_t count);
int hs_spmspv_device(hs_context* ctx, const hs_idx_val* x_entries_dev, uint32_t count);
int hs_read_spmspv_result(hs_context* ctx, void* packed_y, uint32_t num_rows);
int hs_spmspv_status(hs_context* ctx, uint32_t* overflowed, void** overflow_word_dev);

int hs_load_matrix_csr(hs_context* ctx, uint32_t num_rows, uint32_t num_cols, const uint32_t* indptr, const uint32_t* indices, const float* values,
                       uint32_t* padded_rows, uint32_t* padded_cols);

int hs_load_matrix_csr_transposed(hs_context* ctx, uint32_t num_rows, uint32_t num_cols, const uint32_t* indptr, const uint32_t* indices, const float* values,
                                  uint32_t* padded_rows, uint32_t* padded_cols);

int hs_update_values(hs_context* ctx, const float* values, uint64_t nnz);
int hs_update_values_device(hs_context* ctx, const float* values_dev, uint64_t nnz);

int hs_spmm_device(hs_context* ctx, const void* x_dev, uint64_t ldx, void* y_dev, uint64_t ldy, uint32_t k);
int hs_spmm(hs_context* ctx, const void* packed_x, uint32_t num_cols, uint32_t k, void* packed_y, uint32_t num_rows);

// ... 25 lines not shown
```

Before: 6188.

## Pack DELTA stream values into 24-bit fields with shifted scale and outlier side list

Adds a packed DELTA record format in which each value is stored as a 24-bit field, optionally right-shifted by a common shift, alongside 16-bit gaps. This shrinks each record from 12 to 10 bytes per lane-pair. Values that do not fit are sent to an outlier list that is patched separately. A counting kernel chooses the shift. The SpMV consumer gets a new ring variant that unpacks the fields with alignbit, and the residency and carry heuristics are rescaled to the equivalent unpacked size. The cost is extra unpack ALU work, outlier handling and more build-time complexity, all aimed at cutting HBM bytes read per nonzero in this bandwidth-bound kernel.

```diff
diff --git a/hisparse_amd/csrc/gpu_tiles.h b/hisparse_amd/csrc/gpu_tiles.h
--- a/hisparse_amd/csrc/gpu_tiles.h
+++ b/hisparse_amd/csrc/gpu_tiles.h
@@ -30,7 +30,9 @@
     bool delta_slots(std::vector<detail::UnitPlan>& plans);
     bool owner_shares(std::vector<detail::UnitPlan>& plans, uint32_t max_span);
     bool emit(StreamFormat format, uint64_t image_bytes, uint64_t slack_bytes, const std::vector<detail::UnitPlan>& plans,
-              const std::vector<uint32_t>& block_of_unit, const std::vector<Block>& blocks, bool is_float);
+              const std::vector<uint32_t>& block_of_unit, const std::vector<Block>& blocks, bool is_float, uint32_t value_bits, uint32_t value_shift,
+              uint64_t outliers, const std::vector<Unit>& units, std::vector<uint32_t>& outlier_unit, std::vector<Outlier>& outlier_entry);
+    bool count_value_misfits(uint64_t (&misfits)[kMaxValueShift + 1]);
     bool bitmap_slice_counts(uint32_t slices, uint32_t groups_per_row, std::vector<uint32_t>& cnt);
     struct BitmapBlock {
         uint32_t row0, nrows, gs0, GS, pieces, stride;
diff --git a/hisparse_amd/csrc/gpu_tiles.hip b/hisparse_amd/csrc/gpu_tiles.hip
--- a/hisparse_amd/csrc/gpu_tiles.hip
+++ b/hisparse_amd/csrc/gpu_tiles.hip
@@ -460,6 +460,68 @@
             *gap_word = uint16_t(gap);
         }
     }
+}
+
+struct DeviceOutlier { uint64_t element; uint32_t pos, value; };
+__global__ __launch_bounds__(256) void emit_delta24_kernel(const DevicePlan* __restrict__ plans, const uint64_t* __restrict__ keys,
+                                                          const uint32_t* __restrict__ vals, const uint64_t* __restrict__ bridges,
+                                                          uint8_t* __restrict__ image, uint32_t shift, DeviceOutlier* __restrict__ outliers,
+                                                          uint32_t* __restrict__ outlier_count, uint32_t outlier_capacity) {
+    const DevicePlan& p = plans[blockIdx.x];
+    if (!p.n) return;
+    const uint32_t scratch_pos = p.nrows * kSubTileCols;
+    const uint32_t first_pos = uint32_t(keys[p.start] & kPosMask);
+    for (uint32_t w = 0; w < kConsumerWaves; ++w) {
+        const uint32_t run = p.run_len[w];
+        if (!run) continue;
+        uint8_t* rec = image + p.wave_offset[w] + uint64_t(p.start_step[w]) * kRecordBytes24;
+        const uint32_t records = (run + 2) / 2;
+        for (uint32_t idx = threadIdx.x; idx < records * kWaveLanes; idx += blockDim.x) {
+            const uint32_t r = idx / kWaveLanes, l = idx % kWaveLanes;
+            const uint64_t s0 = p.first_slot[w] + uint64_t(l) * p.lane_stride[w];
+            uint32_t field[2] = {0, 0}, gap[2] = {0, 0};
+            for (uint32_t h = 0; h < 2; ++h) {
+                const uint32_t j = 2 * r + h;
+                if (j == 0) {
+                    uint32_t head = scratch_pos;
+                    if (s0 < p.slots) head = s0 == 0 ? first_pos : delta_slot(p, keys, vals, bridges, s0 - 1).after;
+                    field[0] = head & 0xffffffu;
+                    gap[0] = head >> 24;
+                    continue;
+                }
+                const uint64_t si = s0 + (j - 1);
+                if (j > run || si >= p.slots) continue;
+                const Slot s = delta_slot(p, keys, vals, bridges, si);
+                gap[h] = s.gap;
+                if (value_fits24(s.val, shift)) {
+                    field[h] = s.val >> shift;
+                } else {
+                    const uint32_t k = atomicAdd(outlier_count, 1u);
+                    if (k < outlier_capacity) outliers[k] = DeviceOutlier{s.e, s.after, s.val};
+                }
+            }
+            uint8_t* at = rec + uint64_t(r) * kRecordBytes24;
+            reinterpret_cast<uint64_t*>(at)[l] = uint64_t(field[0]) | uint64_t(field[1]) << 24 | uint64_t(gap[0]) << 48;
+            reinterpret_cast<uint16_t*>(at + kWaveLanes * 8)[l] = uint16_t(gap[1]);
+        }
+    }
+}
+
+__global__ __launch_bounds__(256) void value_misfits_kernel(const uint32_t* __restrict__ vals, uint64_t n, unsigned long long* __restrict__ misfits) {
+    __shared__ uint32_t local[kMaxValueShift + 1];
+    if (threadIdx.x <= kMaxValueShift) local[threadIdx.x] = 0;
+    __syncthreads();
+    uint32_t mine[kMaxValueShift + 1] = {0};
+    for (uint64_t i = uint64_t(blockIdx.x) * blockDim.x + threadIdx.x; i < n; i += uint64_t(gridDim.x) * blockDim.x) {
+        const uint32_t v = vals[i];
+#pragma unroll
+        for (uint32_t sh = 0; sh <= kMaxValueShift; ++sh) mine[sh] += !value_fits24(v, sh);
+    }
+#pragma unroll
+    for (uint32_t sh = 0; sh <= kMaxValueShift; ++sh)
+        if (mine[sh]) atomicAdd(&local[sh], mine[sh]);
+    __syncthreads();
+    if (threadIdx.x <= kMaxValueShift && local[threadIdx.x]) atomicAdd(&misfits[threadIdx.x], static_cast<unsigned long long>(local[threadIdx.x]));
 }
 
 struct ElementSource {
@@ -993,8 +1055,31 @@
     return ok;
 }
 
+bool GpuTiler::count_value_misfits(uint64_t (&misfits)[kMaxValueShift + 1]) {
+    for (uint64_t& m : misfits) m = 0;
+    if (!total_) return true;
+    DeviceBuffer<unsigned long long> d_misfits;
+    unsigned long long host[kMaxValueShift + 1] = {0};
+    bool ok = check(d_misfits.alloc_count(kMaxValueShift + 1, 16), "hipMalloc") && check(hipMemsetAsync(d_misfits.get(), 0, sizeof(host), stream_), "hipMemset");
+    if (ok) {
+        const uint32_t grid = uint32_t(std::min<uint64_t>((total_ + 255) / 256, 4096));
+        hipLaunchKernelGGL(value_misfits_kernel, dim3(grid), dim3(256), 0, stream_, d_vals_.get(), total_, d_misfits.get());
+        ok = check(hipGetLastError(), "value_misfits_kernel") && check(hipMemcpyAsync(host, d_misfits.get(), sizeof(host), hipMemcpyDeviceToHost, stream_), "read misfits") &&
+             check(hipStreamSynchronize(stream_), "value misfits");
+    }
+    for (uint32_t sh = 0; ok && sh <= kMaxValueShift; ++sh) misfits[sh] = host[sh];
+    return ok;
+}
+
 bool GpuTiler::emit(StreamFormat format, uint64_t image_bytes, uint64_t slack_bytes, const std::vector<UnitPlan>& plans,
-                    const std::vector<uint32_t>& block_of_unit, const std::vector<Block>& blocks, bool is_float) {
+                    const std::vector<uint32_t>& block_of_unit, const std::vector<Block>& blocks, bool is_float, uint32_t value_bits, uint32_t value_shift,
+                    uint64_t outliers, const std::vector<Unit>& units, std::vector<uint32_t>& outlier_unit, std::vector<Outlier>& outlier_entry) {
+    outlier_unit.clear();
+    outlier_entry.clear();
+    const bool packed = format == kFormatDelta && value_bits == 24;
+    if (packed && (is_float || d_src_ || outliers > 0xffffffffull)) return fail("gpu re-tile: the packed DELTA record is fixed-point only and keeps no value map");
+    DeviceBuffer<DeviceOutlier> d_outliers;
+    DeviceBuffer<uint32_t> d_outlier_count;
     std::vector<DevicePlan> dp;
     make_device_plans(plans, block_of_unit, blocks, dp);
     DeviceBuffer<DevicePlan> d_plans;
@@ -1024,6 +1109,14 @@
                 hipLaunchKernelGGL((m ? emit_owner_kernel<true, true> : emit_owner_kernel<true, false>), grid, block, 0, stream_, p, keys, vals, image, src, map);
                 break;
             case kFormatDelta:
+                if (packed) {
+                    ok = check(d_outliers.alloc_count(std::max<uint64_t>(outliers, 1), 16), "hipMalloc(outliers)") && check(d_outlier_count.alloc_count(1, 16), "hipMalloc") &&
+                         check(hipMemsetAsync(d_outlier_count.get(), 0, 4, stream_), "hipMemset");
+                    if (ok)
+                        hipLaunchKernelGGL(emit_delta24_kernel, grid, block, 0, stream_, p, keys, vals, d_bridges_.get(), image, value_shift, d_outliers.get(),
+                                           d_outlier_count.get(), uint32_t(outliers));
+                    break;
+                }
                 hipLaunchKernelGGL(m ? emit_delta_kernel<true> : emit_delta_kernel<false>, grid, block, 0, stream_, p, keys, vals, d_bridges_.get(), image,
                                    is_float ? kBridgeGap : 0u, src, map);
                 break;
@@ -1032,6 +1125,24 @@
         ok = ok && check(hipGetLastError(), "emit kernel");
     }
     ok = ok && check(hipStreamSynchronize(stream_), "emit");
+    if (ok && packed && !plans.empty()) {
+        uint32_t found = 0;
+        ok = check(hipMemcpy(&found, d_outlier_count.get(), 4, hipMemcpyDeviceToHost), "read outlier count");
+        if (ok && found != outliers) ok = fail("gpu re-tile: the emit pass found another number of outliers than the counting pass");
+        std::vector<DeviceOutlier> list(found);
+        if (ok && found) ok = check(hipMemcpy(list.data(), d_outliers.get(), size_t(found) * sizeof(DeviceOutlier), hipMemcpyDeviceToHost), "read outliers");
+        if (ok && found) {
+            std::sort(list.begin(), list.end(), [](const DeviceOutlier& a, const DeviceOutlier& b) { return a.element < b.element; });
+            for (const DeviceOutlier& o : list) {
+                size_t lo = 0, hi = plans.size();
+                while (hi - lo > 1) { const size_t mid = (lo + hi) / 2; if (plans[mid].scratch <= o.element) lo = mid; else hi = mid; }
+                outlier_unit.push_back(uint32_t(lo));
+                outlier_entry.push_back(Outlier{o.pos / kSubTileCols, units[lo].col0 + o.pos % kSubTileCols, o.value});
+            }
+            const uint64_t tail = (uint64_t(found) * sizeof(Outlier) + 15u) & ~uint64_t(15);
+            ok = check(hipMemcpy(d_image_.get() + image_bytes - tail, outlier_entry.data(), size_t(found) * sizeof(Outlier), hipMemcpyHostToDevice), "write outliers");
+        }
+    }
     d_keys_.reset();
     d_vals_.reset();
     d_bridges_.reset();
diff --git a/hisparse_amd/csrc/hs_load.cpp b/hisparse_amd/csrc/hs_load.cpp
--- a/hisparse_amd/csrc/hs_load.cpp
+++ b/hisparse_amd/csrc/hs_load.cpp
@@ -47,6 +47,7 @@
     if (csr_in) {
         csr_view = *csr_in;
         csr_view.value_map = map_on && want_map;
+        csr_view.plain_values = map_on;
         csr = &csr_view;
     }
 
@@ -132,9 +133,11 @@
     const uint64_t image_bytes = image_on_device ? tiles.image_bytes : uint64_t(tiles.image.size());
     const char* resident_opt = ctx_option(ctx, "HISPARSE_STREAM_RESIDENT");
     m.launch.stream_resident = resident_opt ? std::atoi(resident_opt) != 0
-                                     : hisparse::dev::plan_stream_resident(tiles.format, tiles.light, image_bytes, tiles.units.size(), tiles.blocks.size());
+                                     : hisparse::dev::plan_stream_resident(tiles.format, tiles.light, image_bytes, tiles.units.size(), tiles.blocks.size(), tiles.value_bits);
     const char* carry_opt = ctx_option(ctx, "HISPARSE_CARRY_COMBINE");
-    const bool carries = tiles.col_slices > 1 && (carry_opt ? std::atoi(carry_opt) != 0 : hisparse::dev::plan_carries(tiles.format, image_bytes));
+    const uint64_t carry_bytes = tiles.format == hisparse::dev::kFormatDelta && tiles.value_bits == 24
+                                     ? image_bytes / hisparse::dev::kRecordBytes24 * hisparse::dev::kRecordBytes : image_bytes;
+    const bool carries = tiles.col_slices > 1 && (carry_opt ? std::atoi(carry_opt) != 0 : hisparse::dev::plan_carries(tiles.format, carry_bytes));
     HS_HIP(ctx, ctx->carry.reset(ctx->is_float(), num_rows, num_cols, tiles.col_slices, carries));
     if (mfma_on_device || (tiles.mfma.words_bytes != 0 && !tiles.mfma.words.empty())) {
         const hisparse::dev::MfmaImage& mi = tiles.mfma;
@@ -184,6 +187,7 @@
     a.part_heads = m.part_heads.get();
     a.ring_buffers = tiles.ring_buffers;
     a.format = tiles.format;
+    a.value_bits = tiles.value_bits;
     a.num_cols = num_cols;
     a.num_workgroups = tiles.num_workgroups;
     a.lds_bytes = lds_bytes;
@@ -209,6 +213,7 @@
     s.load_seconds = std::chrono::duration<double>(std::chrono::steady_clock::now() - t0).count();
     s.retiled_on_gpu = image_on_device;
     s.light_kernel = tiles.light ? 1u : 0u;
+    s.value_bits = tiles.value_bits;
     s.stream_resident = a.stream_resident && hisparse::dev::stream_policy_applies(tiles.format, tiles.light) ? 1u : 0u;
     return HS_OK;
 }
diff --git a/hisparse_amd/csrc/spmv_kernels.h b/hisparse_amd/csrc/spmv_kernels.h
--- a/hisparse_amd/csrc/spmv_kernels.h
+++ b/hisparse_amd/csrc/spmv_kernels.h
@@ -20,6 +20,7 @@
     int32_t row_part_filter;
     uint32_t ring_buffers;
     uint32_t format;
+    uint32_t value_bits = 0;
     uint32_t num_cols;
     uint32_t num_workgroups;
     uint32_t lds_bytes;
diff --git a/hisparse_amd/csrc/spmv_kernels.hip b/hisparse_amd/csrc/spmv_kernels.hip
--- a/hisparse_amd/csrc/spmv_kernels.hip
+++ b/hisparse_amd/csrc/spmv_kernels.hip
@@ -65,10 +65,12 @@
 constexpr int kMaxDepth = 16;
 constexpr int kOwner24Depth = 3;
 
+constexpr int ring_format(int kRing) { return (kRing & 8) ? 4 : (kRing & 3); }
+constexpr bool ring_is_delta(int kRing) { return ring_format(kRing) == 1 || ring_format(kRing) == 4; }
 template <int kFmt, bool kRes>
 struct RingT;
 template <int kRing>
-using Ring = RingT<(kRing & 3), (kRing & 4) != 0>;
+using Ring = RingT<ring_format(kRing), (kRing & 4) != 0>;
 template <bool kRes>
 struct RingT<0, kRes> {
     static constexpr uint32_t kLaneBytes = 8;
@@ -108,6 +110,29 @@
     static __device__ __forceinline__ void take_record(uint32_t& value_a, uint32_t& value_b, uint32_t& gaps) {
         asm volatile("s_waitcnt vmcnt(%6)\n\tv_accvgpr_read_b32 %0, a[%3]\n\tv_accvgpr_read_b32 %1, a[%4]\n\tv_accvgpr_read_b32 %2, a[%5]"
                      : "=v"(value_a), "=v"(value_b), "=v"(gaps) : "n"(2 * K), "n"(2 * K + 1), "n"(K + kMaxDepth), "n"(2 * (kDepth - 1)) : "memory");
+    }
+};
+template <bool kRes>
+struct RingT<4, kRes> {
+    static constexpr uint32_t kLaneBytes = 8;
+    template <int K>
+    static __device__ __forceinline__ void issue(const uint8_t* base, uint32_t byte_off, uint32_t lane_off) {
+        static_assert(2 * K + 1 < kMaxDepth && K + kMaxDepth < 2 * kMaxDepth, "dwordx2 in a0..a15, gap B in a16..a23: ring depth <= 8");
+#define HS_ISSUE(P)                                                                                                                                         \
+    asm volatile("s_nop 4\n\tglobal_load_dwordx2 a[%0:%1], %3, %5 " P "\n\tglobal_load_ushort a[%2], %4, %5 offset:512 " P ::"n"(2 * K), "n"(2 * K + 1),    \
+                 "n"(K + kMaxDepth), "v"(byte_off + lane_off), "v"(byte_off + lane_off / 4), "s"(base)                                                     \
+                 : "memory", HS_RING_AGPRS)
+        HS_BY_POLICY(kRes, HS_ISSUE);
+#undef HS_ISSUE
+    }
+    template <int K, int kDepth>
+    static __device__ __forceinline__ void take_record(uint32_t& field_a, uint32_t& field_b, uint32_t& gaps) {
+        uint32_t lo, hi, gap_b;
+        asm volatile("s_waitcnt vmcnt(%6)\n\tv_accvgpr_read_b32 %0, a[%3]\n\tv_accvgpr_read_b32 %1, a[%4]\n\tv_accvgpr_read_b32 %2, a[%5]"
+                     : "=v"(lo), "=v"(hi), "=v"(gap_b) : "n"(2 * K), "n"(2 * K + 1), "n"(K + kMaxDepth), "n"(2 * (kDepth - 1)) : "memory");
+        field_a = lo & 0xffffffu;
+        field_b = __builtin_amdgcn_alignbit(hi, lo, 24) & 0xffffffu;
+        gaps = (hi >> 16) | (gap_b << 16);
     }
 };
 template <bool kRes>
@@ -188,6 +213,7 @@
     uint32_t next_end = 0;
     const uint32_t* xb;
     uint32_t pos = 0;
+    uint32_t value_shift = 0;
     bool head = true;
     uint32_t run_row = kNoRow;
     typename Rows<kFloat>::sum_t run_sum = 0;
@@ -214,8 +240,8 @@
 template <bool kFloat, int kRing, int kAblate, int kDepth, bool kDense, int K>
 __device__ __forceinline__ bool consume_step(Consumer<kFloat>& c) {
     using R = Rows<kFloat>;
-    constexpr bool kDelta = (kRing & 3) == 1, k24 = (kRing & 3) == 2;
-    constexpr uint32_t kStride = kDelta ? kRecordBytes : k24 ? kWaveStrideBytes24 : kWaveStrideBytes;
+    constexpr bool kDelta = ring_is_delta(kRing), kPacked = ring_format(kRing) == 4, k24 = ring_format(kRing) == 2;
+    constexpr uint32_t kStride = kPacked ? kRecordBytes24 : kDelta ? kRecordBytes : k24 ? kWaveStrideBytes24 : kWaveStrideBytes;
     constexpr uint32_t kColMask = k24 ? kSubTileCols - 1u : 0xffffu, kRowShift = k24 ? kOwnerColBits : 16u;
     const uint32_t s = c.base + K;
     while (s == c.end) {
@@ -267,12 +293,12 @@
             }
         };
         if (c.head) {
-            c.pos = value_a;
+            c.pos = kPacked ? (value_a | (gaps << 24)) : value_a;
             c.head = false;
         } else {
-            slot(value_a, gaps & 0xffffu);
-        }
-        slot(value_b, gaps >> 16);
+            slot(kPacked ? value_a << c.value_shift : value_a, gaps & 0xffffu);
+        }
+        slot(kPacked ? value_b << c.value_shift : value_b, gaps >> 16);
     } else {
         Ring<kRing>::template take<K, kDepth>(mat, aux);
         const uint32_t xv = (kAblate & 2) ? aux : c.xb[aux & kColMask];
@@ -572,8 +598,8 @@
                                                uint32_t lane, const uint32_t* xs, uint32_t ring, typename Rows<kFloat>::acc_t* ys, uint32_t nrows,
                                                uint32_t total, uint32_t first_end) {
     static_assert(kDepth <= kMaxDepth, "the ring lives in a0..a31");
-    constexpr bool kDelta = (kRing & 3) == 1, k24 = (kRing & 3) == 2;
-    constexpr uint32_t kStride = kDelta ? kRecordBytes : kOwner ? kChunkBytes : k24 ? kWaveStrideBytes24 : kWaveStrideBytes;
+    constexpr bool kDelta = ring_is_delta(kRing), kPacked = ring_format(kRing) == 4, k24 = ring_format(kRing) == 2;
+    constexpr uint32_t kStride = kPacked ? kRecordBytes24 : kDelta ? kRecordBytes : kOwner ? kChunkBytes : k24 ? kWaveStrideBytes24 : kWaveStrideBytes;
     c.stream = scalar_pointer(stream);
     c.unit = unit; c.U = U; c.wave = wave; c.lane = lane; c.ring = ring; c.nrows = nrows;
     c.lane_off = lane * Ring<kRing>::kLaneBytes;
@@ -610,10 +636,10 @@
 }
 
 template <bool kFloat, int kRing, int kAblate, int kDepth, bool kOwner = false>
-__global__ __launch_bounds__(kThreads) void spmv_rowblock_kernel(const uint8_t* __restrict__ image, const Block* __restrict__ blocks,
-                                                                  const Unit* __restrict__ units, const uint32_t* __restrict__ x,
-                                                                  uint32_t* __restrict__ out, int32_t row_part_filter, uint32_t ring,
-                                                                  uint32_t x_base, const uint32_t* __restrict__ part_heads, CarriedCombine carry) {
+__device__ __forceinline__ void rowblock_workgroup(const uint8_t* __restrict__ image, const Block* __restrict__ blocks,
+                                                   const Unit* __restrict__ units, const uint32_t* __restrict__ x,
+                                                   uint32_t* __restrict__ out, int32_t row_part_filter, uint32_t ring,
+                                                   uint32_t x_base, const uint32_t* __restrict__ part_heads, const CarriedCombine& carry) {
     using acc_t = typename Rows<kFloat>::acc_t;
     extern __shared__ __attribute__((aligned(16))) uint8_t lds[];
     acc_t* ys = reinterpret_cast<acc_t*>(lds);
@@ -649,6 +675,7 @@
             else
                 consumer_begin<kFloat, kRing, kDepth, kOwner>(c, image + blk->wave_offset[wave], unit, U, wave, lane, xs, ring, ys, nrows, blk->total_steps[wave],
                                                                blk->first_end[wave]);
+            if constexpr (ring_format(kRing) == 4) c.value_shift = blk->value_shift;
         }
         if (carry.partial && block_no == 0) carried_combine<kFloat, kThreads>(carry, blockIdx.x, gridDim.x, tid);
         if (kOwner) {
@@ -725,6 +752,16 @@
             if (!next) break;
             continue;
         }
+        if constexpr (ring_format(kRing) == 4) {
+            const uint32_t n_out = blk->outlier_count;
+            if (!loader && n_out) {
+                const Outlier* list = reinterpret_cast<const Outlier*>(image + ((static_cast<uint64_t>(blk->outlier_hi) << 32) | blk->outlier_lo));
+                for (uint32_t i = tid; i < n_out; i += kConsumerWaves * kWaveLanes) {
+                    const Outlier o = list[i];
+                    Rows<kFloat>::add(ys, o.row, Rows<kFloat>::product(o.value, x[o.col]));
+                }
+            }
+        }
         if (!loader) {
             const acc_t flushed = atomicAdd(ys + nrows, static_cast<acc_t>(0));
             asm volatile("" ::"v"(flushed));
@@ -735,6 +772,23 @@
         timeline_stamp<kAblate>(block_no, wave, lane, 4);
         if (!next) break;
     }
+}
+
+template <bool kFloat, int kRing, int kAblate, int kDepth, bool kOwner = false>
+__global__ __launch_bounds__(kThreads) void spmv_rowblock_kernel(const uint8_t* __restrict__ image, const Block* __restrict__ blocks,
+                                                                  const Unit* __restrict__ units, const uint32_t* __restrict__ x,
+                                                                  uint32_t* __restrict__ out, int32_t row_part_filter, uint32_t ring,
+                                                                  uint32_t x_base, const uint32_t* __restrict__ part_heads, CarriedCombine carry) {
+    static_assert(!(kRing & 8), "DELTA with 24-bit value fields is spmv_rowblock_kernel_delta24");
+    rowblock_workgroup<kFloat, kRing, kAblate, kDepth, kOwner>(image, blocks, units, x, out, row_part_filter, ring, x_base, part_heads, carry);
+}
+
+template <bool kRes, int kAblate>
+__global__ __launch_bounds__(kThreads) void spmv_rowblock_kernel_delta24(const uint8_t* __restrict__ image, const Block* __restrict__ blocks,
+                                                                 const Unit* __restrict__ units, const uint32_t* __restrict__ x,
+                                                                 uint32_t* __restrict__ out, int32_t row_part_filter, uint32_t ring,
+                                                                 uint32_t x_base, const uint32_t* __restrict__ part_heads, CarriedCombine carry) {
+    rowblock_workgroup<false, kRes ? 12 : 8, kAblate, 8>(image, blocks, units, x, out, row_part_filter, ring, x_base, part_heads, carry);
 }
 
 template <bool kFloat>
@@ -973,6 +1027,11 @@
     X(true, 0, 0, 8) X(true, 1, 0, 8) X(false, 0, 0, 8) X(false, 1, 0, 8) X(true, 2, 0, 8) X(false, 2, 0, 8)      \
     X(true, 4, 0, 8) X(true, 5, 0, 8) X(false, 4, 0, 8) X(false, 5, 0, 8)
 #ifndef HISPARSE_PROFILING
+#define HS_FOR_EACH_DELTA24_VARIANT(X) X(false, 0) X(true, 0)
+#else
+#define HS_FOR_EACH_DELTA24_VARIANT(X) X(false, 0) X(true, 0) X(false, 1) X(false, 2) X(false, 3)
+#endif
+#ifndef HISPARSE_PROFILING
 #define HS_FOR_EACH_VARIANT(X) HS_FOR_EACH_PRODUCT_VARIANT(X)
 #else
 #define HS_FOR_EACH_VARIANT(X)                                                                                   \
@@ -989,6 +1048,12 @@
     hipError_t e;
 #define X(F, T, A, D) if ((e = configure_one<F, T, A, D>(lds_bytes)) != hipSuccess) return e;
     HS_FOR_EACH_VARIANT(X)
+#undef X
+#define X(R, A)                                                                                                                               \
+    if ((e = hipFuncSetAttribute(reinterpret_cast<const void*>(&spmv_rowblock_kernel_delta24<R, A>), hipFuncAttributeMaxDynamicSharedMemorySize, \
+                                 static_cast<int>(lds_bytes))) != hipSuccess)                                                                \
+        return e;
+    HS_FOR_EACH_DELTA24_VARIANT(X)
 #undef X
 #define X(A) if ((e = configure_one<true, false, A, 8, true>(lds_bytes)) != hipSuccess) return e;
     HS_FOR_EACH_OWNER_VARIANT(X)
@@ -1026,6 +1091,8 @@
         return hipErrorInvalidValue;
     }
     int ring = a.format == kFormatDelta ? 1 : a.format == kFormatPairs24 ? 2 : 0;
+    const bool delta24 = a.format == kFormatDelta && a.value_bits == 24;
+    if (delta24 && is_float) return hipErrorInvalidValue;
     const dim3 grid(a.num_workgroups), block(kThreads);
     const uint32_t x_base = a.lds_bytes - a.ring_buffers * kBufBytes;
     const CarriedCombine carry = carried(a);
@@ -1120,6 +1187,18 @@
         }
         return launched ? hipGetLastError() : hipErrorInvalidValue;
     }
+    if (delta24) {
+        const bool resident = (ring & 4) != 0;
+#define X(R, A)                                                                                                                      \
+    if (!launched && resident == R && ablate == A && depth == 8) {                                                                    \
+        hipLaunchKernelGGL((spmv_rowblock_kernel_delta24<R, A>), grid, block, a.lds_bytes, stream, a.image, a.blocks, a.units, a.x, a.out,      \
+                           a.row_part_filter, a.ring_buffers, x_base, a.part_heads, carry);                                          \
+        launched = true;                                                                                                             \
+    }
+        HS_FOR_EACH_DELTA24_VARIANT(X)
+#undef X
+        return launched ? hipGetLastError() : hipErrorInvalidValue;
+    }
 #define X(F, T, A, D)                                                                                                           \
     if (!launched && is_float == F && ring == int(T) && ablate == A && depth == D) {                                     \
         hipLaunchKernelGGL((spmv_rowblock_kernel<F, T, A, D>), grid, block, a.lds_bytes, stream, a.image, a.blocks, a.units,    \
diff --git a/hisparse_amd/csrc/stream_plan.h b/hisparse_amd/csrc/stream_plan.h
--- a/hisparse_amd/csrc/stream_plan.h
+++ b/hisparse_amd/csrc/stream_plan.h
@@ -26,6 +26,7 @@
 };
 struct PlanSwitches {
     ForcedFormat format = ForcedFormat::kNone;
+    DeltaValueBits delta_bits = DeltaValueBits::kByRule;
     IntSwitch col_slices, max_rows, light, light_wgs, sweep, row_runs;
     bool spmm4 = false;
     bool pow2_slices = false;
@@ -47,7 +48,9 @@
         };
         if (const char* force = env_switch("HISPARSE_STREAM_FORMAT")) {
             const std::string f(force);
-            sw.format = f == "pairs" ? ForcedFormat::kPairs : f == "delta" ? ForcedFormat::kDelta : f == "owner" ? ForcedFormat::kOwner :
+            if (f == "delta24") sw.delta_bits = DeltaValueBits::kPacked;
+            if (f == "delta32") sw.delta_bits = DeltaValueBits::kPlain;
+            sw.format = f == "pairs" ? ForcedFormat::kPairs : (f == "delta" || f == "delta24" || f == "delta32") ? ForcedFormat::kDelta : f == "owner" ? ForcedFormat::kOwner :
                         f == "owner24" ? ForcedFormat::kOwner24 : f == "sweep" ? ForcedFormat::kSweep : f == "bitmap" ? ForcedFormat::kBitmap : ForcedFormat::kInvalid;
         }
         sw.col_slices = number("HISPARSE_COL_SLICES");
@@ -70,7 +73,7 @@
         return sw;
     }
 };
-inline const char* const kBadStreamFormat = "HISPARSE_STREAM_FORMAT must be pairs, delta, owner, owner24, sweep or bitmap";
+inline const char* const kBadStreamFormat = "HISPARSE_STREAM_FORMAT must be pairs, delta, delta24, delta32, owner, owner24, sweep or bitmap";
 
 
 template <typename Load>
diff --git a/hisparse_amd/csrc/stream_tiles.cpp b/hisparse_amd/csrc/stream_tiles.cpp
--- a/hisparse_amd/csrc/stream_tiles.cpp
+++ b/hisparse_amd/csrc/stream_tiles.cpp
@@ -4,6 +4,7 @@
 #include "stream_plan.h"
 
 #include <algorithm>
+#include <array>
 #include <atomic>
 #include <chrono>
 #include <cmath>
@@ -54,6 +55,8 @@
     std::vector<uint32_t> block_of_unit;
     std::vector<uint64_t> block_nnz;
     uint64_t image_bytes = 0;
+    uint32_t record_bytes = kRecordBytes;
+    uint64_t outlier_count = 0;
     std::vector<std::vector<uint32_t>> mine;
 
     TileBuild(const void* const channel_[NUM_HBM_CHANNELS], const uint64_t n_packets_[NUM_HBM_CHANNELS], const Geometry& geom, uint32_t num_rows_,
@@ -102,6 +105,8 @@
     void fall_back_to_pairs();
     bool owner_shares(uint32_t max_span);
     bool lay_out_streams();
+    bool choose_value_bits();
+    void place_outliers(const std::vector<uint32_t>& unit, const std::vector<Outlier>& entry);
     void assign_to_workgroups();
     void finish_blocks();
     bool emit_on_gpu();
@@ -382,6 +387,7 @@
     const bool delta_spread = sw.delta_spread;
     block_nnz.assign(NB, 0);
     image_bytes = 0;
+    out.elements = 0;
     for (uint32_t bi = 0; bi < NB; ++bi) {
         Block& blk = out.blocks[bi];
         uint32_t pos[kConsumerWaves] = {0};
@@ -420,12 +426,12 @@
         }
         for (uint32_t w = 0; w < kConsumerWaves; ++w) block_nnz[bi] += pos[w];
         for (uint32_t w = 0; w < kConsumerWaves; ++w)
-            if (uint64_t(pos[w]) * (delta ? kRecordBytes : owner ? chunk_bytes : wave_stride) >= (1ull << 32)) { error = "row block stream exceeds 4 GiB"; return false; }
+            if (uint64_t(pos[w]) * (delta ? record_bytes : owner ? chunk_bytes : wave_stride) >= (1ull << 32)) { error = "row block stream exceeds 4 GiB"; return false; }
         if (delta || owner) {
             for (uint32_t w = 0; w < kConsumerWaves; ++w) {
                 blk.wave_offset[w] = image_bytes;
                 image_bytes += owner24 ? uint64_t((pos[w] + kOwnerRecordSteps - 1) / kOwnerRecordSteps) * kOwnerRecordBytes
-                                       : uint64_t(pos[w]) * (delta ? kRecordBytes : chunk_bytes);
+                                       : uint64_t(pos[w]) * (delta ? record_bytes : chunk_bytes);
             }
         } else {
             for (uint32_t w = 0; w < kConsumerWaves; ++w) blk.wave_offset[w] = image_bytes + uint64_t(w) * chunk_bytes;
@@ -433,6 +439,59 @@
         }
     }
     return true;
+}
+
+bool TileBuild::choose_value_bits() {
+    out.value_bits = 32;
+    out.value_shift = 0;
+    if (is_float || sw.delta_bits == DeltaValueBits::kPlain || (csr && (csr->value_map || csr->plain_values))) return true;
+    uint64_t misfits[kMaxValueShift + 1] = {0};
+    if (gpu) {
+        if (!gpu->count_value_misfits(misfits)) return gpu_failed();
+    } else {
+        std::vector<std::array<uint64_t, kMaxValueShift + 1>> part(out.units.size());
+        parallel_for(out.units.size(), [&](size_t u) {
+            part[u].fill(0);
+            const uint64_t* e = scratch.data() + plans[u].scratch;
+            for (uint32_t i = 0; i < plans[u].n; ++i)
+                for (uint32_t sh = 0; sh <= kMaxValueShift; ++sh) part[u][sh] += !value_fits24(uint32_t(e[i]), sh);
+        });
+        for (const auto& p : part)
+            for (uint32_t sh = 0; sh <= kMaxValueShift; ++sh) misfits[sh] += p[sh];
+    }
+    uint32_t shift = 0;
+    for (uint32_t sh = 1; sh <= kMaxValueShift; ++sh)
+        if (misfits[sh] < misfits[shift]) shift = sh;
+    const uint64_t plain_bytes = image_bytes, outliers = misfits[shift];
+    const uint64_t packed_bytes = plain_bytes / kRecordBytes * kRecordBytes24 + ((outliers * sizeof(Outlier) + 15u) & ~uint64_t(15));
+    const bool within_cap = outliers * kDelta24OutlierShare <= out.elements;
+    const bool wanted = sw.delta_bits == DeltaValueBits::kPacked || plain_bytes >= packed_bytes + kDelta24MinSavedBytes;
+    if (sw.debug)
+        std::fprintf(stderr, "delta value bits: shift %u leaves %llu outliers among %llu element slots, %llu -> %llu bytes: %s\n", shift, (unsigned long long)outliers,
+                     (unsigned long long)out.elements, (unsigned long long)plain_bytes, (unsigned long long)packed_bytes, within_cap && wanted ? "packed" : "plain");
+    if (!within_cap || !wanted) return true;
+    out.value_bits = 24;
+    out.value_shift = shift;
+    outlier_count = outliers;
+    record_bytes = kRecordBytes24;
+    if (!lay_out_streams()) return false;
+    image_bytes += (outliers * sizeof(Outlier) + 15u) & ~uint64_t(15);
+    for (Block& blk : out.blocks) { blk.value_shift = shift; blk.value_bits = 24; }
+    return true;
+}
+
+void TileBuild::place_outliers(const std::vector<uint32_t>& unit, const std::vector<Outlier>& entry) {
+    const uint64_t lists = image_bytes - ((outlier_count * sizeof(Outlier) + 15u) & ~uint64_t(15));
+    for (size_t k = 0; k < entry.size(); ++k) {
+        Block& blk = out.blocks[block_of_unit[unit[k]]];
+        if (!blk.outlier_count) {
+            const uint64_t at = lists + k * sizeof(Outlier);
+            blk.outlier_lo = uint32_t(at);
+            blk.outlier_hi = uint32_t(at >> 32);
+        }
+        blk.outlier_count++;
+    }
+    out.outliers = entry.size();
 }
 
 void TileBuild::assign_to_workgroups() {
@@ -463,7 +522,12 @@
 }
 
 bool TileBuild::emit_on_gpu() {
-    if (!gpu->emit(out.format, image_bytes, image_slack, plans, block_of_unit, out.blocks, is_float)) return gpu_failed();
+    std::vector<uint32_t> outlier_unit;
+    std::vector<Outlier> outlier_entry;
+    if (!gpu->emit(out.format, image_bytes, image_slack, plans, block_of_unit, out.blocks, is_float, out.value_bits, out.value_shift, outlier_count, out.units, outlier_unit,
+                   outlier_entry))
+        return gpu_failed();
+    if (out.value_bits == 24) place_outliers(outlier_unit, outlier_entry);
     out.d_image = gpu->release_image();
     out.d_value_map = gpu->release_value_map();
     out.image_bytes = image_bytes;
@@ -539,6 +603,9 @@
 
 void TileBuild::emit_delta() {
     uint8_t* image = out.image.data();
+    const bool packed = out.value_bits == 24;
+    const uint32_t shift = out.value_shift;
+    std::vector<std::vector<Outlier>> unit_outliers(packed ? out.units.size() : 0);
     parallel_for(out.units.size(), [&](size_t u) {
         const UnitPlan& up = plans[u];
         const Block& blk = out.blocks[block_of_unit[u]];
@@ -552,15 +619,38 @@
             while (d > kMaxGap) { at += kBridgeAdvance; d -= kBridgeAdvance; gap[k] = kBridgeGap; val[k] = 0; after[k] = at; ++k; }
             at += uint32_t(d);
             gap[k] = uint16_t(d); val[k] = uint32_t(e[i]); after[k] = at; ++k;
+            if (packed && !value_fits24(val[k - 1], shift)) {
+                unit_outliers[u].push_back(Outlier{at / kSubTileCols, out.units[u].col0 + at % kSubTileCols, val[k - 1]});
+                val[k - 1] = 0;
+            }
         }
         const uint16_t pad_gap = is_float ? kBridgeGap : 0;
         const uint32_t scratch_pos = blk.nrows * kSubTileCols;
         for (uint32_t w = 0; w < kConsumerWaves; ++w) {
             if (!up.run_len[w]) continue;
-            uint8_t* rec = image + blk.wave_offset[w] + uint64_t(up.start_record[w]) * kRecordBytes;
+            uint8_t* rec = image + blk.wave_offset[w] + uint64_t(up.start_record[w]) * record_bytes;
+            const uint32_t slots_in_records = (up.run_len[w] + 2) / 2 * 2;
+            if (packed) {
+                auto put_slot = [&](uint32_t q, uint32_t l, uint32_t field, uint32_t gap16) {
+                    uint8_t* r = rec + uint64_t(q / 2) * kRecordBytes24;
+                    uint64_t& word = reinterpret_cast<uint64_t*>(r)[l];
+                    if (q % 2 == 0) word |= uint64_t(field) | uint64_t(gap16) << 48;
+                    else { word |= uint64_t(field) << 24; reinterpret_cast<uint16_t*>(r + kWaveLanes * 8)[l] = uint16_t(gap16); }
+                };
+                for (uint32_t l = 0; l < kWaveLanes; ++l) {
+                    const uint64_t s0 = up.first_slot[w] + uint64_t(l) * up.lane_stride[w];
+                    const uint32_t head = s0 >= up.slots ? scratch_pos : (s0 == 0 ? uint32_t(e[0] >> 32) : after[s0 - 1]);
+                    put_slot(0, l, head & 0xffffffu, head >> 24);
+                    for (uint32_t j = 0; j < up.run_len[w]; ++j) {
+                        const uint64_t si = s0 + j;
+                        put_slot(j + 1, l, si < up.slots ? val[si] >> shift : 0u, si < up.slots ? gap[si] : pad_gap);
+                    }
+                    for (uint32_t q = up.run_len[w] + 1; q < slots_in_records; ++q) put_slot(q, l, 0u, pad_gap);
+                }
+                continue;
+            }
             auto value_at = [&](uint32_t q, uint32_t l) -> uint32_t& { return reinterpret_cast<uint32_t*>(rec + uint64_t(q / 2) * kRecordBytes)[2 * l + q % 2]; };
             auto gap_at = [&](uint32_t q, uint32_t l) -> uint16_t& { return reinterpret_cast<uint16_t*>(rec + uint64_t(q / 2) * kRecordBytes + kWaveLanes * 8)[2 * l + q % 2]; };
-            const uint32_t slots_in_records = (up.run_len[w] + 2) / 2 * 2;
             for (uint32_t l = 0; l < kWaveLanes; ++l) {
                 const uint64_t s0 = up.first_slot[w] + uint64_t(l) * up.lane_stride[w];
                 value_at(0, l) = s0 >= up.slots ? scratch_pos : (s0 == 0 ? uint32_t(e[0] >> 32) : after[s0 - 1]);
@@ -573,6 +663,14 @@
             }
         }
     });
+    if (packed) {
+        std::vector<uint32_t> unit;
+        std::vector<Outlier> entry;
+        for (size_t u = 0; u < unit_outliers.size(); ++u)
+            for (const Outlier& o : unit_outliers[u]) { unit.push_back(uint32_t(u)); entry.push_back(o); }
+        place_outliers(unit, entry);
+        if (!entry.empty()) std::memcpy(image + image_bytes - ((outlier_count * sizeof(Outlier) + 15u) & ~uint64_t(15)), entry.data(), entry.size() * sizeof(Outlier));
+    }
     finish_blocks();
     timer.lap("emit DELTA");
 }
@@ -640,6 +738,7 @@
     }
     if (wants_pairs24(b.plan, sw, out.max_block_rows)) b.set_format(kFormatPairs24);
     if (!b.lay_out_streams()) return Attempt::kFailed;
+    if (out.format == kFormatDelta && !b.choose_value_bits()) return Attempt::kFailed;
     b.assign_to_workgroups();
     if (b.gpu) return b.emit_on_gpu() ? Attempt::kDone : Attempt::kFailed;
     resize_zeroed(out.image, b.image_bytes);
diff --git a/hisparse_amd/csrc/stream_tiles.h b/hisparse_amd/csrc/stream_tiles.h
--- a/hisparse_amd/csrc/stream_tiles.h
+++ b/hisparse_amd/csrc/stream_tiles.h
@@ -33,6 +33,14 @@
 constexpr uint32_t kChunkBytes = kWaveLanes * 8;
 constexpr uint32_t kWaveStrideBytes = kChunkBytes * kConsumerWaves;
 constexpr uint32_t kRecordBytes = kWaveLanes * 2 * (4 + 2);
+constexpr uint32_t kRecordBytes24 = kWaveLanes * (3 + 3 + 2 + 2);
+constexpr uint32_t kMaxValueShift = 8;
+constexpr uint64_t kDelta24OutlierShare = 4096;
+constexpr uint64_t kDelta24MinSavedBytes = 23u << 20;
+constexpr uint32_t delta_record_bytes(uint32_t value_bits) { return value_bits == 24 ? kRecordBytes24 : kRecordBytes; }
+constexpr bool value_fits24(uint32_t word, uint32_t shift) { return (word >> shift) < (1u << 24) && (word & ((1u << shift) - 1u)) == 0; }
+struct Outlier { uint32_t row, col, value; };
+enum class DeltaValueBits : uint32_t { kByRule = 0, kPacked = 24, kPlain = 32 };
 constexpr uint32_t kMaxGap = 0xfffeu;
 constexpr uint32_t kBridgeGap = 0xffffu;
 constexpr uint32_t kBridgeAdvance = 0xffffu;
@@ -44,9 +52,10 @@
 enum StreamFormat : uint32_t { kFormatPairs = 0, kFormatDelta = 1, kFormatBitmap = 2, kFormatOwner = 3, kFormatPairs24 = 4, kFormatOwner24 = 5, kFormatSweep = 6 };
 constexpr bool rowblock_stream(uint32_t format, bool light) { return (format == kFormatPairs || format == kFormatDelta) && !light; }
 constexpr bool stream_policy_applies(uint32_t format, bool light) { return format == kFormatSweep || rowblock_stream(format, light); }
-constexpr bool plan_stream_resident(uint32_t format, bool light, uint64_t image_bytes, uint64_t num_units, uint64_t num_blocks) {
+constexpr bool plan_stream_resident(uint32_t format, bool light, uint64_t image_bytes, uint64_t num_units, uint64_t num_blocks, uint32_t value_bits = 0) {
+    const uint64_t judged_bytes = format == kFormatDelta && value_bits == 24 ? image_bytes / kRecordBytes24 * kRecordBytes : image_bytes;
     return rowblock_stream(format, light)
-               ? image_bytes <= kRowblockResidentMaxImageBytes && (num_units > num_blocks || image_bytes <= kRowblockResidentSmallImageBytes)
+               ? judged_bytes <= kRowblockResidentMaxImageBytes && (num_units > num_blocks || judged_bytes <= kRowblockResidentSmallImageBytes)
                : image_bytes <= kResidentMaxImageBytes;
 }
 constexpr bool plan_carries(uint32_t format, uint64_t image_bytes) {
@@ -113,7 +122,11 @@
     uint32_t first_col0, first_ncols;
     uint32_t last_part;
     uint32_t next_part;
-    uint32_t pad[12];
+    uint32_t outlier_lo, outlier_hi;
+    uint32_t outlier_count;
+    uint32_t value_shift;
+    uint32_t value_bits;
+    uint32_t pad[7];
 };
 struct Unit {
     uint32_t col0;
@@ -176,6 +189,9 @@
     uint32_t col_slices = 1;
     uint32_t ring_buffers = kMaxXBuffers;
     StreamFormat format = kFormatPairs;
+    uint32_t value_bits = 0;
+    uint32_t value_shift = 0;
+    uint64_t outliers = 0;
     uint64_t nnz = 0;
     uint64_t elements = 0;
 };
@@ -186,6 +202,7 @@
     const uint32_t* indices = nullptr;
     const float* values = nullptr;
     bool value_map = false;
+    bool plain_values = false;
     bool transposed = false;
     uint32_t out_rows() const { return transposed ? num_cols : num_rows; }
     uint32_t out_cols() const { return transposed ? num_rows : num_cols; }
diff --git a/hisparse_amd/device.py b/hisparse_amd/device.py
--- a/hisparse_amd/device.py
+++ b/hisparse_amd/device.py
@@ -26,7 +26,7 @@
     _fields_ = [("nnz", C.c_uint64), ("cpsr_bytes", C.c_uint64), ("stream_bytes", C.c_uint64), ("stream_elements", C.c_uint64),
                 ("num_blocks", C.c_uint32), ("num_units", C.c_uint32), ("num_workgroups", C.c_uint32), ("lds_bytes", C.c_uint32),
                 ("num_compute_units", C.c_uint32), ("col_slices", C.c_uint32), ("ring_buffers", C.c_uint32), ("stream_format", C.c_uint32),
-                ("load_seconds", C.c_double), ("retiled_on_gpu", C.c_uint32), ("light_kernel", C.c_uint32), ("stream_resident", C.c_uint32), ("reserved0", C.c_uint32)]
+                ("load_seconds", C.c_double), ("retiled_on_gpu", C.c_uint32), ("light_kernel", C.c_uint32), ("stream_resident", C.c_uint32), ("value_bits", C.c_uint32)]
 
     def as_dict(self):
         return {name: getattr(self, name) for name, _ in self._fields_}
@@ -37,7 +37,16 @@
 BLOCK_DTYPE = np.dtype([("row0", "<u4"), ("nrows", "<u4"), ("row_part", "<u4"), ("unit_begin", "<u4"), ("unit_end", "<u4"),
                         ("flags", "<u4"), ("out_offset", "<u4"), ("next", "<u4"), ("wave_offset", "<u8", (CONSUMER_WAVES,)),
                         ("total_steps", "<u4", (CONSUMER_WAVES,)), ("first_end", "<u4", (CONSUMER_WAVES,)), ("first_col0", "<u4"),
-                        ("first_ncols", "<u4"), ("last_part", "<u4"), ("next_part", "<u4"), ("pad", "<u4", (12,))])
+                        ("first_ncols", "<u4"), ("last_part", "<u4"), ("next_part", "<u4"),
+                        ("outlier_lo", "<u4"), ("outlier_hi", "<u4"), ("outlier_count", "<u4"), ("value_shift", "<u4"), ("value_bits", "<u4"), ("pad", "<u4", (7,))])
+OUTLIER_DTYPE = np.dtype([("row", "<u4"), ("col", "<u4"), ("value", "<u4")])
+
+
+def _delta_value_bits(fmt, blocks):
+    if fmt != "delta":
+        return 0, 0
+    packed = len(blocks) > 0 and int(blocks["value_bits"][0]) == 24
+    return (24, int(blocks["value_shift"][0])) if packed else (32, 0)
 UNIT_DTYPE = np.dtype([("col0", "<u4"), ("ncols", "<u4"), ("end_step", "<u4", (CONSUMER_WAVES,))])
 
 
@@ -223,7 +232,8 @@
         blocks = np.zeros(max(nblocks, 1), dtype=BLOCK_DTYPE)
         units = np.zeros(max(nunits, 1), dtype=UNIT_DTYPE)
         self._check(lib().hs_debug_read_tiles(self._h, image.ctypes.data, image.size, blocks.ctypes.data, units.ctypes.data))
-        return dict(image=image[:nbytes], blocks=blocks[:nblocks], units=units[:nunits])
+        bits, shift = _delta_value_bits(STREAM_FORMATS[st["stream_format"]], blocks[:nblocks])
+        return dict(image=image[:nbytes], blocks=blocks[:nblocks], units=units[:nunits], value_bits=bits, value_shift=shift)
 
     def read_mfma_image(self):
         n = C.c_uint64()
@@ -350,7 +360,8 @@
         mfma = np.zeros(max(mbytes.value, 1), dtype=np.uint8)
         if mbytes.value:
             l.hs_tiles_mfma(h, mfma.ctypes.data, mfma.size, None, None, None)
-        return dict(image=image[:nbytes.value], blocks=blocks[:nblocks.value], units=units[:nunits.value], wg_first=wg_first,
+        bits, shift = _delta_value_bits(STREAM_FORMATS[fmt.value], blocks[:nblocks.value])
+        return dict(image=image[:nbytes.value], blocks=blocks[:nblocks.value], units=units[:nunits.value], wg_first=wg_first, value_bits=bits, value_shift=shift,
                     block_order=order[:nblocks.value], num_workgroups=nwg.value, max_block_rows=maxrows.value, nnz=nnz.value,
                     elements=elems.value, col_slices=slices.value, ring_buffers=ring.value,
                     format=STREAM_FORMATS[fmt.value], mfma=mfma[:mbytes.value], mfma_chunk=chunk.value, mfma_chunks=chunks.value)
diff --git a/include/hisparse_hip.h b/include/hisparse_hip.h
--- a/include/hisparse_hip.h
+++ b/include/hisparse_hip.h
@@ -43,7 +43,7 @@
     uint32_t retiled_on_gpu;
     uint32_t light_kernel;
     uint32_t stream_resident;
-    uint32_t reserved0;
+    uint32_t value_bits;
 } hs_stats;
 
 const char* hs_strerror(int code);
```

Measured after the change: 6598, median of 6. 1.07x the previous value.
